# burchim/AVEC

Measured on AMD Instinct MI355X. Metric: AV utterances/sec fwd+bwd (audio T=400, video 100x88x88), higher is better.
Workload: dtype bf16

## Files before the change

avec_amd/csrc/norm.hip:

```cpp
#include "common.h"
#include "avec_hip.h"

#include "vec.h"

__global__ __launch_bounds__(256) void col_finalize_kernel(ColFin f) {
  __shared__ float red[16][17];
  const int cw = threadIdx.x & 15, sl = threadIdx.x >> 4;
  const int ncols = f.NV * f.W;
  const int o = blockIdx.x * 16 + cw;
  const unsigned cb = blockIdx.y;
  const int s0 = blockIdx.z * 128;
  float s = 0.f;
  if (o < ncols) {
    const float* p = f.partial + ((size_t)cb * f.nslots) * ncols + o;
#pragma unroll
    for (int k = 0; k < 8; ++k) {
      const int si = s0 + sl + 16 * k; const int sc = si < f.nslots ? si : f.nslots - 1;
      const float v = p[(size_t)sc * ncols];
      s += si < f.nslots ? v : 0.f;
    }
  }
  red[sl][cw] = s;
  __syncthreads();
  if (sl == 0 && o < ncols) {
// ... 241 lines not shown
  t1 = wave_sum(t1) / D; t2 = wave_sum(t2) / D;
#pragma unroll
  for (int i = 0; i < 2; ++i) {
    const int c = lane * 4 + i * 256; if (c >= D) break;
    float r[4];
#pragma unroll
    for (int e = 0; e < 4; ++e) r[e] = rs1 * (o[i][e] * gg1[i][e] - t1 - w1[i][e] * t2);
    st4<float>(dx1 + row * D + c, r);
    if (pr.out) {
      float q[4], ds[4]; drop4(dk, (unsigned long long)row * D + c, ds);
#pragma unroll
      for (int e = 0; e < 4; ++e) q[e] = r[e] * (pr.alpha * ds[e]);
      if (pr.f32) st4<float>((float*)pr.out + row * D + c, q); else st4<bf16>((bf16*)pr.out + row * D + c, q);
    }
  }
}
extern "C" int avec_layernorm_bwd2(int dtype, const void* dy2, const float* x2, const float* mean2, const float* rstd2, const float* gamma2, const float* dres2, float* dx2,
                                   const float* x1, const float* mean1, const float* rstd1, const float* gamma1, float* dx1,
                                   void* prep, float prep_alpha, float prep_drop_p, const unsigned long long* rng, unsigned rng_stream, long long M, int D, hipStream_t st) {
  AVEC_CHECK_ARG(dy2 && x2 && mean2 && rstd2 && gamma2 && dx2 && x1 && mean1 && rstd1 && gamma1 && dx1, "layernorm_bwd2: null pointer");
  AVEC_CHECK_ARG(M > 0 && D > 0 && D % 4 == 0 && D <= 512 && (!prep || prep_drop_p <= 0.f || rng), "layernorm_bwd2: D=%d must be a multiple of 4 in [4, 512]; dropout needs rng", D);
  LnPrep pr; pr.out = prep; pr.alpha = prep_alpha; pr.p = prep ? prep_drop_p : 0.f; pr.rng = rng; pr.stream = rng_stream; pr.f32 = dtype == AVEC_F32;
  dim3 grid((unsigned)((M + 3) / 4));
  if (dtype == AVEC_F32) hipLaunchKernelGGL(ln_bwd_rows2_kernel<float>, grid, dim3(256), 0, st, (const float*)dy2, x2, mean2, rstd2, gamma2, dres2, dx2, x1, mean1, rstd1, gamma1, dx1, M, D, pr);
  else hipLaunchKernelGGL(ln_bwd_rows2_kernel<bf16>, grid, dim3(256), 0, st, (const bf16*)dy2, x2, mean2, rstd2, gamma2, dres2, dx2, x1, mean1, rstd1, gamma1, dx1, M, D, pr);
  AVEC_LAUNCH_CHECK(); return 0;
}

struct LnItem { const void* dy; const float* x; const float* mean; const float* rstd; float* dg; float* db; int M, D, dy_f32, first; };
struct LnGroup { LnItem it[AVEC_LN_GROUP_MAX]; int n; };
static constexpr int LNG_ROWS = 128;
__global__ __launch_bounds__(256) void ln_param_grads_grouped_kernel(LnGroup grp) {
  __shared__ float red[2][256][4];
  const int w = blockIdx.x;
  int lo = 0, hi = grp.n - 1;
  while (lo < hi) { const int mid = (lo + hi + 1) >> 1; if (grp.it[mid].first <= w) lo = mid; else hi = mid - 1; }
  const LnItem& t = grp.it[lo];
  const int D = t.D, L = D >> 2, R = 256 / L;
  const int r = threadIdx.x / L, l = threadIdx.x - r * L;
  const int m0 = (w - t.first) * LNG_ROWS; int m1 = m0 + LNG_ROWS; if (m1 > t.M) m1 = t.M;
  float pg[4] = {0.f, 0.f, 0.f, 0.f}, pb[4] = {0.f, 0.f, 0.f, 0.f};
  if (r < R) {
    constexpr int U = 8;
    for (int m = m0 + r; m < m1; m += R * U) {
      float d[U][4], v[U][4], mu[U], rs[U];
#pragma unroll
      for (int u = 0; u < U; ++u) {
        const int mm = m + u * R; const bool ok = mm < m1; const long long mi = ok ? mm : m;
        if (t.dy_f32) ld4<float>((const float*)t.dy + mi * D + l * 4, d[u]); else ld4<bf16>((const bf16*)t.dy + mi * D + l * 4, d[u]);
        ld4<float>(t.x + mi * D + l * 4, v[u]); mu[u] = t.mean[mi]; rs[u] = ok ? t.rstd[mi] : 0.f;
        if (!ok) d[u][0] = d[u][1] = d[u][2] = d[u][3] = 0.f;
      }
#pragma unroll
      for (int u = 0; u < U; ++u)
#pragma unroll
        for (int e = 0; e < 4; ++e) { pg[e] += d[u][e] * (v[u][e] - mu[u]) * rs[u]; pb[e] += d[u][e]; }
    }
  }
#pragma unroll
  for (int e = 0; e < 4; ++e) { red[0][threadIdx.x][e] = pg[e]; red[1][threadIdx.x][e] = pb[e]; }
  __syncthreads();
  for (int o = threadIdx.x; o < 2 * D; o += 256) {
    const int which = o >= D, c = o - which * D; float s = 0.f;
    for (int rr = 0; rr < R; ++rr) s += red[which][rr * L + (c >> 2)][c & 3];
    atomicAdd((which ? t.db : t.dg) + c, s);
  }
}
extern "C" int avec_layernorm_param_grads_grouped(int dtype, const avec_ln_item_t* items, int n, hipStream_t st) {
  AVEC_CHECK_ARG(items && n > 0 && n <= AVEC_LN_GROUP_MAX, "layernorm_param_grads_grouped: need 1..%d items (got %d)", AVEC_LN_GROUP_MAX, n);
  LnGroup grp; grp.n = n; int first = 0;
  for (int k = 0; k < n; ++k) {
    const avec_ln_item_t& s = items[k];
    AVEC_CHECK_ARG(s.dy && s.x && s.mean && s.rstd && s.dgamma && s.dbeta && s.M > 0 && s.M < (1ll << 31) && s.D >= 4 && s.D % 4 == 0 && s.D <= 1024,
                   "layernorm_param_grads_grouped: item %d: null pointer or D=%d not a multiple of 4 in [4, 1024]", k, s.D);
    LnItem& t = grp.it[k];
    t.dy = s.dy; t.x = s.x; t.mean = s.mean; t.rstd = s.rstd; t.dg = s.dgamma; t.db = s.dbeta; t.M = (int)s.M; t.D = s.D;
    t.dy_f32 = (s.dy_f32 || dtype == AVEC_F32) ? 1 : 0; t.first = first;
    first += (int)((s.M + LNG_ROWS - 1) / LNG_ROWS);
  }
  hipLaunchKernelGGL(ln_param_grads_grouped_kernel, dim3((unsigned)first), dim3(256), 0, st, grp);
  AVEC_LAUNCH_CHECK(); return 0;
}

static int layernorm_bwd_impl(int dtype, const void* dy, int dy_f32, const float* x, const float* mean, const float* rstd, const float* gamma,
                              float* dx, const float* dres, float* dgamma, float* dbeta, long long M, int D, const LnPrep& pr, hipStream_t st) {
  AVEC_CHECK_ARG(dy && x && mean && rstd && gamma && dx && (!dgamma == !dbeta), "layernorm_bwd: null pointer");
  AVEC_CHECK_ARG(M > 0 && D > 0 && D % 4 == 0 && D <= 1536, "layernorm_bwd: D=%d must be a multiple of 4 and <= 1536", D);
  AVEC_CHECK_ARG(!pr.out || (!dgamma && (pr.p <= 0.f || pr.rng)), "layernorm_bwd_prep: the second output comes with the dx-only kernel (dgamma == NULL); dropout needs rng");
  if (!dgamma) {
    const dim3 grid((unsigned)((M + 3) / 4)); const bool f32in = dy_f32 || dtype == AVEC_F32;
#define AVEC_LN_ROWS(TG, NG) hipLaunchKernelGGL((ln_bwd_rows_kernel<TG, NG>), grid, dim3(256), 0, st, (const TG*)dy, x, mean, rstd, gamma, dx, dres, M, D, pr)
    if (D <= 512) { if (f32in) AVEC_LN_ROWS(float, 2); else AVEC_LN_ROWS(bf16, 2); }
    else { if (f32in) AVEC_LN_ROWS(float, 6); else AVEC_LN_ROWS(bf16, 6); }
#undef AVEC_LN_ROWS
    AVEC_LAUNCH_CHECK(); return 0;
  }
  long long nb = (M + 15) / 16; if (nb > 256) nb = 256; if (nb < 1) nb = 1;
  ColWs ws = avec_reduce_ws((size_t)nb * 2 * D, st);
  if (!ws.partial && nb > 128) nb = 128;
  const size_t lds = (size_t)2 * D * sizeof(float);
#define AVEC_LN_BWD(TG, NG) hipLaunchKernelGGL((ln_bwd_kernel<TG, NG>), dim3((unsigned)nb), dim3(256), lds, st, (const TG*)dy, x, mean, rstd, gamma, dx, dres, dgamma, dbeta, M, D, ws)
  const bool f32in = dy_f32 || dtype == AVEC_F32;
  if (D <= 512) { if (f32in) AVEC_LN_BWD(float, 2); else AVEC_LN_BWD(bf16, 2); }
  else { if (f32in) AVEC_LN_BWD(float, 6); else AVEC_LN_BWD(bf16, 6); }
#undef AVEC_LN_BWD
  AVEC_LAUNCH_CHECK();
  if (ws.partial) { float* const dst[2] = {dgamma, dbeta}; return col_finalize(ws, 1, (unsigned)nb, 2, D, dst, D, st); }
  return 0;
}
extern "C" int avec_layernorm_bwd(int dtype, const void* dy, int dy_f32, const float* x, const float* mean, const float* rstd, const float* gamma,
                                  float* dx, const float* dres, float* dgamma, float* dbeta, long long M, int D, hipStream_t st) {
  LnPrep pr; pr.out = nullptr; pr.alpha = 1.f; pr.p = 0.f; pr.rng = nullptr; pr.stream = 0; pr.f32 = 0;
  return layernorm_bwd_impl(dtype, dy, dy_f32, x, mean, rstd, gamma, dx, dres, dgamma, dbeta, M, D, pr, st);
}
extern "C" int avec_layernorm_bwd_prep(int dtype, const void* dy, int dy_f32, const float* x, const float* mean, const float* rstd, const float* gamma,
                                       float* dx, const float* dres, void* prep, float prep_alpha, float prep_drop_p, const unsigned long long* rng, unsigned rng_stream,
                                       long long M, int D, hipStream_t st) {
  AVEC_CHECK_ARG(prep, "layernorm_bwd_prep: null prep buffer");
  LnPrep pr; pr.out = prep; pr.alpha = prep_alpha; pr.p = prep_drop_p; pr.rng = rng; pr.stream = rng_stream; pr.f32 = dtype == AVEC_F32;
  return layernorm_bwd_impl(dtype, dy, dy_f32, x, mean, rstd, gamma, dx, dres, nullptr, nullptr, M, D, pr, st);
}

template <typename T>
__global__ __launch_bounds__(256) void grad_prep_kernel(const float* __restrict__ dout, long long ldd, T* __restrict__ dacc, float alpha, float p,
                                                        const unsigned long long* rng, unsigned stream, float* dbias, long long M, int N, ColWs ws) {
  const int tx = threadIdx.x & 31, ty = threadIdx.x >> 5;
  const int col = (blockIdx.x * 32 + tx) * 4;
  float part[1][4] = {{0.f, 0.f, 0.f, 0.f}};
  const DropKey dk = drop_key(rng, stream, p);
  if (col < N) {
    for (long long row = (long long)blockIdx.y * 8 + ty; row < M; row += (long long)gridDim.y * 8) {
      float v[4]; ld4<float>(dout + row * ldd + col, v);
      float ds[4]; drop4(dk, (unsigned long long)row * N + col, ds);
      for (int e = 0; e < 4; ++e) { v[e] *= alpha * ds[e]; part[0][e] += v[e]; }
      st4<T>(dacc + row * N + col, v);
    }
  }
  float* const dst[1] = {dbias};
  if (dbias) colreduce_atomic<1>(part, dst, col, N, ws);
}

template <typename T>
__global__ __launch_bounds__(256) void grad_prep_flat_kernel(const float* __restrict__ dout, long long ldd, T* __restrict__ dacc, float alpha, float p,
                                                             const unsigned long long* rng, unsigned stream, long long M, int N) {
  const int N4 = N >> 2; const long long n4 = M * N4;
  const DropKey dk = drop_key(rng, stream, p);
  for (long long i = (long long)blockIdx.x * 256 + threadIdx.x; i < n4; i += (long long)gridDim.x * 256) {
    const long long row = n4 < (1ll << 31) ? (long long)((unsigned)i / (unsigned)N4) : i / N4; const int col = (int)(i - row * N4) * 4;
    float v[4]; ld4<float>(dout + row * ldd + col, v);
    float ds[4]; drop4(dk, (unsigned long long)row * N + col, ds);
    for (int e = 0; e < 4; ++e) v[e] *= alpha * ds[e];
    st4<T>(dacc + row * N + col, v);
  }
}
extern "C" int avec_grad_prep(int dtype, const float* dout, long long ld, void* dacc, float alpha, float drop_p, const unsigned long long* rng,
                              unsigned rng_stream, float* dbias, long long M, int N, hipStream_t st) {
  AVEC_CHECK_ARG(dout && dacc && M > 0 && N > 0 && N % 4 == 0 && ld % 4 == 0, "grad_prep: bad arguments (N=%d ld=%lld)", N, ld);
  AVEC_CHECK_ARG(!(drop_p > 0.f) || rng, "grad_prep: dropout without rng");
  if (!dbias) {
    long long nb = (M * (N / 4) + 255) / 256; if (nb > 8192) nb = 8192;
    DISPATCH_T(dtype, hipLaunchKernelGGL(grad_prep_flat_kernel<T>, dim3((unsigned)nb), dim3(256), 0, st, dout, ld, (T*)dacc, alpha, drop_p, rng, rng_stream, M, N));
    AVEC_LAUNCH_CHECK(); return 0;
  }
  dim3 grid = col_grid(M, N); ColWs ws = dbias ? col_ws_if(grid, 1, N, st) : ColWs{nullptr};
  DISPATCH_T(dtype, hipLaunchKernelGGL(grad_prep_kernel<T>, grid, dim3(256), 0, st, dout, ld, (T*)dacc, alpha, drop_p, rng, rng_stream, dbias, M, N, ws));
  AVEC_LAUNCH_CHECK();
  if (ws.partial) { float* const dst[1] = {dbias}; return col_finalize(ws, grid.x, grid.y, 1, 128, dst, N, st); }
  return 0;
}

template <typename T>
__global__ __launch_bounds__(256) void colsum_kernel(const T* __restrict__ x, long long ld, float* out, long long M, int N, ColWs ws) {
  const int tx = threadIdx.x & 31, ty = threadIdx.x >> 5; const int col = (blockIdx.x * 32 + tx) * 4;
  float part[1][4] = {{0.f, 0.f, 0.f, 0.f}};
  if (col < N) for (long long row = (long long)blockIdx.y * 8 + ty; row < M; row += (long long)gridDim.y * 8) {
    float v[4]; ld4<T>(x + row * ld + col, v); for (int e = 0; e < 4; ++e) part[0][e] += v[e];
  }
  float* const dst[1] = {out};
  colreduce_atomic<1>(part, dst, col, N, ws);
}
extern "C" int avec_colsum(int dtype, const void* x, long long ld, float* out, long long M, int N, hipStream_t st) { return colsum_launch(dtype, x, ld, out, M, N, true, st); }
int colsum_launch(int dtype, const void* x, long long ld, float* out, long long M, int N, bool use_ws, hipStream_t st) {
  AVEC_CHECK_ARG(x && out && M > 0 && N > 0 && N % 4 == 0 && ld % 4 == 0, "colsum: bad arguments");
  dim3 grid = col_grid(M, N); if (!use_ws && grid.y > 16) grid.y = 16; ColWs ws = use_ws ? col_ws_if(grid, 1, N, st) : ColWs{nullptr};
  DISPATCH_T(dtype, hipLaunchKernelGGL(colsum_kernel<T>, grid, dim3(256), 0, st, (const T*)x, ld, out, M, N, ws));
  AVEC_LAUNCH_CHECK();
  if (ws.partial) { float* const dst[1] = {out}; return col_finalize(ws, grid.x, grid.y, 1, 128, dst, N, st); }
  return 0;
}

template <typename T>
__global__ __launch_bounds__(256) void bn_stats_kernel(const T* __restrict__ y, float* stats, long long M, int C, ColWs ws) {
  const int tx = threadIdx.x & 31, ty = threadIdx.x >> 5; const int col = (blockIdx.x * 32 + tx) * 4;
  float part[2][4] = {{0.f, 0.f, 0.f, 0.f}, {0.f, 0.f, 0.f, 0.f}};
  if (col < C) for (long long row = (long long)blockIdx.y * 8 + ty; row < M; row += (long long)gridDim.y * 8) {
    float v[4]; ld4<T>(y + row * C + col, v); for (int e = 0; e < 4; ++e) { part[0][e] += v[e]; part[1][e] += v[e] * v[e]; }
  }
  float* const dst[2] = {stats, stats + C};
  colreduce_atomic<2>(part, dst, col, C, ws);
}
extern "C" int avec_bn_stats(int dtype, const void* y, float* stats, long long M, int C, hipStream_t st) {
  AVEC_CHECK_ARG(y && stats && M > 0 && C > 0 && C % 4 == 0, "bn_stats: bad arguments");
  dim3 grid = col_grid(M, C); ColWs ws = col_ws_if(grid, 2, C, st);
  DISPATCH_T(dtype, hipLaunchKernelGGL(bn_stats_kernel<T>, grid, dim3(256), 0, st, (const T*)y, stats, M, C, ws));
  AVEC_LAUNCH_CHECK();
  if (ws.partial) { float* const dst[2] = {stats, stats + C}; return col_finalize(ws, grid.x, grid.y, 2, 128, dst, C, st); }
  return 0;
}

__global__ __launch_bounds__(256) void bn_finalize_kernel(const float* stats, int nrep, const float* count_ptr, float count, const float* gamma, const float* beta, float* rmean, float* rvar,
                                                          long long* nbt, float momentum, float eps, float* ss, int C, int training) {
  __shared__ float red[2][16][17];
  const int cl = threadIdx.x & 15, rl = threadIdx.x >> 4;
  const int c = blockIdx.x * 16 + cl;
  const bool lead = rl == 0 && c < C;
  float gm = 0.f, bt = 0.f, rm = 0.f, rv = 0.f, n = count;
  if (lead) { gm = gamma[c]; bt = beta[c]; if (rmean) { rm = rmean[c]; rv = rvar[c]; } if (training && count_ptr) n = *count_ptr; }
  float s1 = 0.f, s2 = 0.f;
  if (training && c < C) for (int r = rl; r < nrep; r += 16) { s1 += stats[(long long)r * 2 * C + c]; s2 += stats[(long long)r * 2 * C + C + c]; }
  red[0][rl][cl] = s1; red[1][rl][cl] = s2;
  __syncthreads();
  if (!lead) return;
  float mean, var;
  if (training) {
    s1 = 0.f; s2 = 0.f;
#pragma unroll
    for (int k = 0; k < 16; ++k) { s1 += red[0][k][cl]; s2 += red[1][k][cl]; }
    mean = s1 / n; var = fmaxf(s2 / n - mean * mean, 0.f);
    if (rmean && isfinite(mean) && isfinite(var)) {
      rmean[c] = (1.f - momentum) * rm + momentum * mean;
      rvar[c] = (1.f - momentum) * rv + momentum * var * (n / fmaxf(n - 1.f, 1.f));
      if (c == 0 && nbt) *nbt += 1;
    }
  } else { mean = rm; var = rv; }
  const float rs = rsqrtf(var + eps);
  ss[c] = gm * rs; ss[C + c] = bt - mean * gm * rs; ss[2 * C + c] = mean; ss[3 * C + c] = rs;
}
__global__ __launch_bounds__(256) void bn_collapse_kernel(const float* __restrict__ stats, int nrep, float count, float* __restrict__ out, int C2) {
  const int c = blockIdx.x * 256 + threadIdx.x;
  if (c < C2) { float s = 0.f; for (int r = 0; r < nrep; ++r) s += stats[(long long)r * C2 + c]; out[c] = s; }
  if (c == 0) out[C2] = count;
}
__global__ __launch_bounds__(256) void bn_affine_grads_kernel(const float* __restrict__ dstats, float* dgamma, float* dbeta, int C) {
  const int c = blockIdx.x * 256 + threadIdx.x;
  if (c < C) { dgamma[c] += dstats[C + c]; dbeta[c] += dstats[c]; }
}
extern "C" int avec_bn_collapse(const float* stats, int n_replicas, float count, float* out, int C, hipStream_t st) {
  AVEC_CHECK_ARG(stats && out && n_replicas > 0 && C > 0, "bn_collapse: bad arguments");
  hipLaunchKernelGGL(bn_collapse_kernel, dim3((2 * C + 255) / 256), dim3(256), 0, st, stats, n_replicas, count, out, 2 * C);
  AVEC_LAUNCH_CHECK(); return 0;
}
extern "C" int avec_bn_affine_grads(const float* dstats, float* dgamma, float* dbeta, int C, hipStream_t st) {
  AVEC_CHECK_ARG(dstats && dgamma && dbeta && C > 0, "bn_affine_grads: bad arguments");
  hipLaunchKernelGGL(bn_affine_grads_kernel, dim3((C + 255) / 256), dim3(256), 0, st, dstats, dgamma, dbeta, C);
  AVEC_LAUNCH_CHECK(); return 0;
}
extern "C" int avec_bn_finalize(const float* stats, int n_replicas, const float* count_ptr, float count, const float* gamma, const float* beta, float* running_mean,
                                float* running_var, long long* num_batches_tracked, float momentum, float eps, float* ss, int C, int training, hipStream_t st) {
  AVEC_CHECK_ARG(gamma && beta && ss && C > 0 && (training ? (stats != nullptr) : (running_mean && running_var)), "bn_finalize: bad arguments");
  hipLaunchKernelGGL(bn_finalize_kernel, dim3((C + 15) / 16), dim3(256), 0, st, stats, n_replicas > 0 ? n_replicas : 1, count_ptr, count, gamma, beta, running_mean, running_var,
                     num_batches_tracked, momentum, eps, ss, C, training);
  AVEC_LAUNCH_CHECK(); return 0;
}

__global__ void stamp_kernel(unsigned long long* out, int i) { if (threadIdx.x == 0) out[i] = wall_clock64(); }
extern "C" int avec_stamp(unsigned long long* out, int slot, hipStream_t st) {
  AVEC_CHECK_ARG(out && slot >= 0, "stamp: bad arguments");
  hipLaunchKernelGGL(stamp_kernel, dim3(1), dim3(64), 0, st, out, slot);
  AVEC_LAUNCH_CHECK(); return 0;
}

__global__ __launch_bounds__(256) void bn_bwd_finalize_kernel(const float* __restrict__ stats, int nrep, const float* __restrict__ ss, float* __restrict__ dstats, int C) {
  const int c = blockIdx.x * 256 + threadIdx.x;
  if (c >= C) return;
  float s1 = 0.f, sy = 0.f;
  for (int r = 0; r < nrep; ++r) { s1 += stats[(long long)r * 2 * C + c]; sy += stats[(long long)r * 2 * C + C + c]; }
  dstats[c] = s1; dstats[C + c] = ss[3 * C + c] * (sy - ss[2 * C + c] * s1);
}
extern "C" int avec_bn_bwd_finalize(const float* stats, int n_replicas, const float* ss, float* dstats, int C, hipStream_t st) {
  AVEC_CHECK_ARG(stats && ss && dstats && C > 0 && n_replicas > 0, "bn_bwd_finalize: bad arguments");
  hipLaunchKernelGGL(bn_bwd_finalize_kernel, dim3((C + 255) / 256), dim3(256), 0, st, stats, n_replicas, ss, dstats, C);
  AVEC_LAUNCH_CHECK(); return 0;
}

template <typename T>
__global__ __launch_bounds__(256) void bn_apply_kernel(const T* __restrict__ y, const float* __restrict__ ss, const T* __restrict__ res, int act,
                                                       T* __restrict__ out, long long n4, int C) {
  for (long long i = (long long)blockIdx.x * 256 + threadIdx.x; i < n4; i += (long long)gridDim.x * 256) {
    const long long off = i * 4; const int c = (int)(off % C);
    float v[4], sc[4], sh[4]; ld4<T>(y + off, v); ld4<float>(ss + c, sc); ld4<float>(ss + C + c, sh);
    for (int e = 0; e < 4; ++e) v[e] = v[e] * sc[e] + sh[e];
    if (res) { float r[4]; ld4<T>(res + off, r); for (int e = 0; e < 4; ++e) v[e] += r[e]; }
    if (act == 1) { for (int e = 0; e < 4; ++e) v[e] = swishf_(v[e]); } else if (act == 2) { for (int e = 0; e < 4; ++e) v[e] = fmaxf(v[e], 0.f); }
    st4<T>(out + off, v);
  }
}
static inline unsigned bn8_blocks(long long n8, int C, unsigned cap) {
  const unsigned C8 = (unsigned)C >> 3; unsigned g = C8, t = 256; while (t) { const unsigned r = g % t; g = t; t = r; }
  const unsigned q = C8 / g;
  long long nb = (n8 + 255) / 256; if (nb > cap) nb = cap;
  nb = nb / q * q; if (nb < q) nb = q;
  return (unsigned)nb;
}
constexpr int BN8_U = 2;
#ifndef AVEC_BN8_UR
#define AVEC_BN8_UR 1
#endif
constexpr int BN8_UR = AVEC_BN8_UR;
constexpr unsigned BN8_CAP_FWD = 8192, BN8_CAP_BWD = 3072;

template <typename T>
__global__ __launch_bounds__(256) void bn_apply8_kernel(const T* __restrict__ y, const float* __restrict__ ss, const T* __restrict__ res, int act,
                                                        T* __restrict__ out, unsigned n8, int C, unsigned char* __restrict__ mask = nullptr,
                                                        const float* __restrict__ res_ss = nullptr) {
  const unsigned C8 = (unsigned)C >> 3, stride = gridDim.x * 256, i0 = blockIdx.x * 256 + threadIdx.x;
  const int c = (int)(i0 % C8) * 8;
  float sc[8], sh[8]; ld8<float>(ss + c, sc); ld8<float>(ss + C + c, sh);
  float rsc[8], rsh[8];
  if (res_ss) { ld8<float>(res_ss + c, rsc); ld8<float>(res_ss + C + c, rsh);
#pragma unroll
    for (int e = 0; e < 8; ++e) sh[e] += rsh[e]; }
  for (unsigned i = i0; i < n8; i += stride * BN8_U) {
    Raw8<T> ry[BN8_U], rr[BN8_U];
#pragma unroll
    for (int u = 0; u < BN8_U; ++u) { const unsigned j = i + u * stride; if (j < n8) { ry[u].load(y + (long long)j * 8); if (res) rr[u].load(res + (long long)j * 8); } }
#pragma unroll
    for (int u = 0; u < BN8_U; ++u) {
      const unsigned j = i + u * stride; if (j >= n8) break;
      float v[8]; ry[u].get(v);
#pragma unroll
      for (int e = 0; e < 8; ++e) v[e] = v[e] * sc[e] + sh[e];
      if (res) { float r[8]; rr[u].get(r);
        if (res_ss) {
#pragma unroll
          for (int e = 0; e < 8; ++e) v[e] += r[e] * rsc[e];
        } else {
#pragma unroll
          for (int e = 0; e < 8; ++e) v[e] += r[e]; } }
      if (act == 1) {
#pragma unroll
        for (int e = 0; e < 8; ++e) v[e] = swishf_(v[e]);
      } else if (act == 2) {
        if (mask) {
          unsigned b = 0;
#pragma unroll
          for (int e = 0; e < 8; ++e) b |= (v[e] > 0.f ? 1u : 0u) << e;
          mask[j] = (unsigned char)b;
        }
#pragma unroll
        for (int e = 0; e < 8; ++e) v[e] = fmaxf(v[e], 0.f);
      }
      st8<T>(out + (long long)j * 8, v);
    }
  }
}
extern "C" int avec_bn_apply_fwd_mask(int dtype, const void* y, const float* ss, const void* residual, const float* residual_ss, void* out, unsigned char* mask, long long M, int C,
                                      hipStream_t st) {
  AVEC_CHECK_ARG(y && ss && out && mask && M > 0 && C > 0 && C % 8 == 0 && M * C / 8 < (1ll << 31) && (residual || !residual_ss), "bn_apply_fwd_mask: bad arguments (C %% 8 == 0, M*C < 2^34)");
  const long long n8 = M * C / 8; const unsigned nb8 = bn8_blocks(n8, C, BN8_CAP_FWD);
  DISPATCH_T(dtype, hipLaunchKernelGGL(bn_apply8_kernel<T>, dim3((unsigned)nb8), dim3(256), 0, st, (const T*)y, ss, (const T*)residual, 2, (T*)out, (unsigned)n8, C, mask, residual_ss));
  AVEC_LAUNCH_CHECK(); return 0;
}
extern "C" int avec_bn_apply_fwd(int dtype, const void* y, const float* ss, const void* residual, int act, void* out, long long M, int C, hipStream_t st) {
  AVEC_CHECK_ARG(y && ss && out && M > 0 && C > 0 && C % 4 == 0, "bn_apply_fwd: bad arguments");
  if (C % 8 == 0 && M * C / 8 < (1ll << 31)) {
    const long long n8 = M * C / 8; const unsigned nb8 = bn8_blocks(n8, C, BN8_CAP_FWD);
    DISPATCH_T(dtype, hipLaunchKernelGGL(bn_apply8_kernel<T>, dim3((unsigned)nb8), dim3(256), 0, st, (const T*)y, ss, (const T*)residual, act, (T*)out, (unsigned)n8, C));
    AVEC_LAUNCH_CHECK(); return 0;
  }
  long long n4 = M * C / 4; long long nb = (n4 + 255) / 256; if (nb > 4096) nb = 4096;
  DISPATCH_T(dtype, hipLaunchKernelGGL(bn_apply_kernel<T>, dim3((unsigned)nb), dim3(256), 0, st, (const T*)y, ss, (const T*)residual, act, (T*)out, n4, C));
  AVEC_LAUNCH_CHECK(); return 0;
}

template <typename T>
__device__ __forceinline__ void bn_dr(const T* dout, const T* y, const T* out, const float* ss, int act, long long off, int c, int C, float dr[4], float yh[4]) {
  float d[4], v[4], mu[4], rs[4]; ld4<T>(dout + off, d); ld4<T>(y + off, v); ld4<float>(ss + 2 * C + c, mu); ld4<float>(ss + 3 * C + c, rs);
  for (int e = 0; e < 4; ++e) yh[e] = (v[e] - mu[e]) * rs[e];
  if (act == 2) {
    if (out) { float o[4]; ld4<T>(out + off, o); for (int e = 0; e < 4; ++e) dr[e] = o[e] > 0.f ? d[e] : 0.f; }
    else { float sc[4], sh[4]; ld4<float>(ss + c, sc); ld4<float>(ss + C + c, sh); for (int e = 0; e < 4; ++e) dr[e] = (v[e] * sc[e] + sh[e]) > 0.f ? d[e] : 0.f; }
  }
  else if (act == 1) { float sc[4], sh[4]; ld4<float>(ss + c, sc); ld4<float>(ss + C + c, sh); for (int e = 0; e < 4; ++e) dr[e] = d[e] * dswishf_(v[e] * sc[e] + sh[e]); }
  else { for (int e = 0; e < 4; ++e) dr[e] = d[e]; }
}
template <typename T>
__global__ __launch_bounds__(256) void bn_bwd_reduce_kernel(const T* __restrict__ dout, const T* __restrict__ y, const T* __restrict__ out, const float* __restrict__ ss,
                                                            int act, float* dstats, long long M, int C, ColWs ws) {
  const int tx = threadIdx.x & 31, ty = threadIdx.x >> 5; const int col = (blockIdx.x * 32 + tx) * 4;
  float part[2][4] = {{0.f, 0.f, 0.f, 0.f}, {0.f, 0.f, 0.f, 0.f}};
  if (col < C) for (long long row = (long long)blockIdx.y * 8 + ty; row < M; row += (long long)gridDim.y * 8) {
    float dr[4], yh[4]; bn_dr<T>(dout, y, out, ss, act, row * C + col, col, C, dr, yh);
    for (int e = 0; e < 4; ++e) { part[0][e] += dr[e]; part[1][e] += dr[e] * yh[e]; }
  }
  float* const dst[2] = {dstats, dstats + C};
  colreduce_atomic<2>(part, dst, col, C, ws);
}
template <typename T>
__global__ __launch_bounds__(256) void bn_bwd_reduce8_kernel(const T* __restrict__ dout, const T* __restrict__ y, const T* __restrict__ out, const float* __restrict__ ss,
                                                             int act, float* dstats, long long M, int C, ColWs ws, const unsigned char* __restrict__ mask = nullptr) {
  const Col8 m = col8_map(C);
  float part[2][8];
#pragma unroll
  for (int e = 0; e < 8; ++e) part[0][e] = part[1][e] = 0.f;
  if (m.active) {
    const int c = m.l * 8;
    float mu[8], rs[8], sc[8], sh[8]; ld8<float>(ss + 2 * C + c, mu); ld8<float>(ss + 3 * C + c, rs);
    if (act == 1 || (act == 2 && !out && !mask)) { ld8<float>(ss + c, sc); ld8<float>(ss + C + c, sh); }
    const long long rstride = (long long)gridDim.x * m.R;
    for (long long row = (long long)blockIdx.x * m.R + m.r; row < M; row += rstride * BN8_UR) {
      Raw8<T> rd[BN8_UR], rv[BN8_UR], ro[BN8_UR]; unsigned mb[BN8_UR];
#pragma unroll
      for (int u = 0; u < BN8_UR; ++u) { const long long r = row + u * rstride; if (r < M) { const long long off = r * C + c; rd[u].load(dout + off); rv[u].load(y + off);
        if (mask) mb[u] = mask[off >> 3]; else if (act == 2 && out) ro[u].load(out + off); } }
#pragma unroll
      for (int u = 0; u < BN8_UR; ++u) {
        if (row + u * rstride >= M) break;
        float d[8], v[8]; rd[u].get(d); rv[u].get(v);
        if (mask) {
#pragma unroll
          for (int e = 0; e < 8; ++e) d[e] = (mb[u] >> e) & 1u ? d[e] : 0.f; }
        else if (act == 2 && out) { float o[8]; ro[u].get(o);
#pragma unroll
          for (int e = 0; e < 8; ++e) d[e] = o[e] > 0.f ? d[e] : 0.f; }
        else if (act == 2) {
#pragma unroll
          for (int e = 0; e < 8; ++e) d[e] = (v[e] * sc[e] + sh[e]) > 0.f ? d[e] : 0.f; }
        else if (act == 1) {
#pragma unroll
          for (int e = 0; e < 8; ++e) d[e] *= dswishf_(v[e] * sc[e] + sh[e]); }
#pragma unroll
        for (int e = 0; e < 8; ++e) { part[0][e] += d[e]; part[1][e] += d[e] * (v[e] - mu[e]) * rs[e]; }
      }
    }
  }
  float* const dst[2] = {dstats, dstats + C};
  colreduce8_atomic<2>(part, dst, m, ws);
}
extern "C" int avec_bn_bwd_reduce_mask(int dtype, const void* dout, const void* y, const unsigned char* mask, const float* ss, float* dstats, long long M, int C, hipStream_t st) {
  AVEC_CHECK_ARG(dout && y && mask && ss && dstats && M > 0 && col8_ok(C), "bn_bwd_reduce_mask: bad arguments");
  ColWs ws; const unsigned nb = col8_cfg(M, C, 2, &ws, st);
  DISPATCH_T(dtype, hipLaunchKernelGGL(bn_bwd_reduce8_kernel<T>, dim3(nb), dim3(256), 0, st, (const T*)dout, (const T*)y, (const T*)nullptr, ss, 2, dstats, M, C, ws, mask));
  AVEC_LAUNCH_CHECK();
  if (ws.partial) { float* const dst[2] = {dstats, dstats + C}; return col_finalize(ws, 1, nb, 2, C, dst, C, st); }
  return 0;
}
extern "C" int avec_bn_bwd_reduce(int dtype, const void* dout, const void* y, const void* out, const float* ss, int act, float* dstats, long long M, int C, hipStream_t st) {
  AVEC_CHECK_ARG(dout && y && ss && dstats && M > 0 && C % 4 == 0, "bn_bwd_reduce: bad arguments");
  if (col8_ok(C)) {
    ColWs ws; const unsigned nb = col8_cfg(M, C, 2, &ws, st);
    DISPATCH_T(dtype, hipLaunchKernelGGL(bn_bwd_reduce8_kernel<T>, dim3(nb), dim3(256), 0, st, (const T*)dout, (const T*)y, (const T*)out, ss, act, dstats, M, C, ws));
    AVEC_LAUNCH_CHECK();
    if (ws.partial) { float* const dst[2] = {dstats, dstats + C}; return col_finalize(ws, 1, nb, 2, C, dst, C, st); }
    return 0;
  }
  dim3 grid = col_grid(M, C); ColWs ws = col_ws_if(grid, 2, C, st);
  DISPATCH_T(dtype, hipLaunchKernelGGL(bn_bwd_reduce_kernel<T>, grid, dim3(256), 0, st, (const T*)dout, (const T*)y, (const T*)out, ss, act, dstats, M, C, ws));
  AVEC_LAUNCH_CHECK();
  if (ws.partial) { float* const dst[2] = {dstats, dstats + C}; return col_finalize(ws, grid.x, grid.y, 2, 128, dst, C, st); }
  return 0;
}
template <typename T>
__global__ __launch_bounds__(256) void bn_bwd_apply_kernel(const T* __restrict__ dout, const T* __restrict__ y, const T* __restrict__ out, const float* __restrict__ ss,
                                                           const float* __restrict__ gamma, const float* __restrict__ dstats, const float* count_ptr, float count, int act,
                                                           T* __restrict__ dy, T* __restrict__ dres, float* dgamma, float* dbeta, long long n4, int C) {
  const float inv_n = 1.f / (count_ptr ? *count_ptr : count);
  if (blockIdx.x == 0 && dgamma) for (int c = threadIdx.x; c < C; c += 256) { atomicAdd(dgamma + c, dstats[C + c]); atomicAdd(dbeta + c, dstats[c]); }
  for (long long i = (long long)blockIdx.x * 256 + threadIdx.x; i < n4; i += (long long)gridDim.x * 256) {
    const long long off = i * 4; const int c = (int)(off % C);
    float dr[4], yh[4], g[4], rs[4], s1[4], s2[4], o[4];
    bn_dr<T>(dout, y, out, ss, act, off, c, C, dr, yh);
    ld4<float>(gamma + c, g); ld4<float>(ss + 3 * C + c, rs); ld4<float>(dstats + c, s1); ld4<float>(dstats + C + c, s2);
    for (int e = 0; e < 4; ++e) o[e] = g[e] * rs[e] * (dr[e] - s1[e] * inv_n - yh[e] * s2[e] * inv_n);
    st4<T>(dy + off, o);
    if (dres) st4<T>(dres + off, dr);
  }
}
template <typename T>
__global__ __launch_bounds__(256) void bn_bwd_apply8_kernel(const T* __restrict__ dout, const T* __restrict__ y, const T* __restrict__ out, const float* __restrict__ ss,
                                                            const float* __restrict__ gamma, const float* __restrict__ dstats, const float* count_ptr, float count, int act,
                                                            T* __restrict__ dy, T* __restrict__ dres, float* dgamma, float* dbeta, unsigned n8, int C,
                                                            const unsigned char* __restrict__ mask = nullptr) {
  const float inv_n = 1.f / (count_ptr ? *count_ptr : count);
  if (blockIdx.x == 0 && dgamma) for (int c = threadIdx.x; c < C; c += 256) { atomicAdd(dgamma + c, dstats[C + c]); atomicAdd(dbeta + c, dstats[c]); }
  const unsigned C8 = (unsigned)C >> 3, stride = gridDim.x * 256, i0 = blockIdx.x * 256 + threadIdx.x;
  const int c = (int)(i0 % C8) * 8;
  float mu[8], rs[8], A[8], m1[8], m2[8], sc[8], sh[8];
  { float g[8], s1[8], s2[8]; ld8<float>(ss + 2 * C + c, mu); ld8<float>(ss + 3 * C + c, rs); ld8<float>(gamma + c, g); ld8<float>(dstats + c, s1); ld8<float>(dstats + C + c, s2);
#pragma unroll
    for (int e = 0; e < 8; ++e) { A[e] = g[e] * rs[e]; m1[e] = s1[e] * inv_n; m2[e] = s2[e] * inv_n; } }
  const bool recompute = act != 0 && !(act == 2 && (out || mask));
  if (recompute) { ld8<float>(ss + c, sc); ld8<float>(ss + C + c, sh); }
  for (unsigned i = i0; i < n8; i += stride * BN8_U) {
    Raw8<T> rd[BN8_U], rv[BN8_U], ro[BN8_U]; unsigned mb[BN8_U];
#pragma unroll
    for (int u = 0; u < BN8_U; ++u) { const unsigned j = i + u * stride; if (j < n8) { const long long off = (long long)j * 8; rd[u].load(dout + off); rv[u].load(y + off);
      if (mask) mb[u] = mask[j]; else if (act == 2 && out) ro[u].load(out + off); } }
#pragma unroll
    for (int u = 0; u < BN8_U; ++u) {
      const unsigned j = i + u * stride; if (j >= n8) break;
      const long long off = (long long)j * 8;
      float d[8], v[8], o[8]; rd[u].get(d); rv[u].get(v);
      if (mask) {
#pragma unroll
        for (int e = 0; e < 8; ++e) d[e] = (mb[u] >> e) & 1u ? d[e] : 0.f;
      } else if (act == 2 && out) { float q[8]; ro[u].get(q);
#pragma unroll
        for (int e = 0; e < 8; ++e) d[e] = q[e] > 0.f ? d[e] : 0.f;
      } else if (act != 0) {
#pragma unroll
        for (int e = 0; e < 8; ++e) { const float pre = v[e] * sc[e] + sh[e]; d[e] = act == 1 ? d[e] * dswishf_(pre) : (pre > 0.f ? d[e] : 0.f); }
      }
#pragma unroll
      for (int e = 0; e < 8; ++e) o[e] = A[e] * (d[e] - m1[e] - (v[e] - mu[e]) * rs[e] * m2[e]);
      st8<T>(dy + off, o);
      if (dres) st8<T>(dres + off, d);
    }
  }
}
extern "C" int avec_bn_bwd_apply_mask(int dtype, const void* dout, const void* y, const unsigned char* mask, const float* ss, const float* gamma, const float* dstats,
                                      const float* count_ptr, float count, void* dy, void* dres, float* dgamma, float* dbeta, long long M, int C, hipStream_t st) {
  AVEC_CHECK_ARG(dout && y && mask && ss && gamma && dstats && dy && M > 0 && C % 8 == 0 && M * C / 8 < (1ll << 31), "bn_bwd_apply_mask: bad arguments");
  const long long n8 = M * C / 8; const unsigned nb8 = bn8_blocks(n8, C, BN8_CAP_BWD);
  DISPATCH_T(dtype, hipLaunchKernelGGL(bn_bwd_apply8_kernel<T>, dim3((unsigned)nb8), dim3(256), 0, st, (const T*)dout, (const T*)y, (const T*)nullptr, ss, gamma, dstats,
                                       count_ptr, count, 2, (T*)dy, (T*)dres, dgamma, dbeta, (unsigned)n8, C, mask));
  AVEC_LAUNCH_CHECK(); return 0;
}
extern "C" int avec_bn_bwd_apply(int dtype, const void* dout, const void* y, const void* out, const float* ss, const float* gamma, const float* dstats,
                                 const float* count_ptr, float count, int act, void* dy, void* dres, float* dgamma, float* dbeta, long long M, int C, hipStream_t st) {
  AVEC_CHECK_ARG(dout && y && ss && gamma && dstats && dy && M > 0 && C % 4 == 0, "bn_bwd_apply: bad arguments");
  if (C % 8 == 0 && M * C / 8 < (1ll << 31)) {
    const long long n8 = M * C / 8; const unsigned nb8 = bn8_blocks(n8, C, BN8_CAP_BWD);
    DISPATCH_T(dtype, hipLaunchKernelGGL(bn_bwd_apply8_kernel<T>, dim3((unsigned)nb8), dim3(256), 0, st, (const T*)dout, (const T*)y, (const T*)out, ss, gamma, dstats,
                                         count_ptr, count, act, (T*)dy, (T*)dres, dgamma, dbeta, (unsigned)n8, C));
    AVEC_LAUNCH_CHECK(); return 0;
  }
  long long n4 = M * C / 4; long long nb = (n4 + 255) / 256; if (nb > 4096) nb = 4096;
  DISPATCH_T(dtype, hipLaunchKernelGGL(bn_bwd_apply_kernel<T>, dim3((unsigned)nb), dim3(256), 0, st, (const T*)dout, (const T*)y, (const T*)out, ss, gamma, dstats,
                                       count_ptr, count, act, (T*)dy, (T*)dres, dgamma, dbeta, n4, C));
  AVEC_LAUNCH_CHECK(); return 0;
}

template <typename T>
__global__ __launch_bounds__(256) void softmax_fwd_kernel(const float* __restrict__ x, T* __restrict__ p, long long M, int V) {
  const int lane = threadIdx.x & 63; const long long row = (long long)blockIdx.x * 4 + (threadIdx.x >> 6);
  if (row >= M) return;
  float mx = -INFINITY;
  for (int c = lane; c < V; c += 64) mx = fmaxf(mx, x[row * V + c]);
  mx = wave_max(mx);
  float s = 0.f;
  for (int c = lane; c < V; c += 64) s += __expf(x[row * V + c] - mx);
  s = 1.f / wave_sum(s);
  for (int c = lane; c < V; c += 64) stf(p + row * V + c, __expf(x[row * V + c] - mx) * s);
}
template <typename T>
__global__ __launch_bounds__(256) void softmax_bwd_kernel(const T* __restrict__ dp, const float* __restrict__ x, float* dx, const float* dadd, long long M, int V) {
  const int lane = threadIdx.x & 63; const long long row = (long long)blockIdx.x * 4 + (threadIdx.x >> 6);
  if (row >= M) return;
  float mx = -INFINITY;
  for (int c = lane; c < V; c += 64) mx = fmaxf(mx, x[row * V + c]);
  mx = wave_max(mx);
  float s = 0.f, dot = 0.f;
  for (int c = lane; c < V; c += 64) { float e = __expf(x[row * V + c] - mx); s += e; dot += e * ldf(dp + row * V + c); }
  s = wave_sum(s); dot = wave_sum(dot) / s;
  for (int c = lane; c < V; c += 64) {
    float pr = __expf(x[row * V + c] - mx) / s; float g = pr * (ldf(dp + row * V + c) - dot);
    dx[row * V + c] = dadd ? dadd[row * V + c] + g : g;
  }
}
extern "C" int avec_softmax_fwd(int dtype, const float* logits, void* probs, long long M, int V, hipStream_t st) {
  AVEC_CHECK_ARG(logits && probs && M > 0 && V > 0, "softmax_fwd: bad arguments");
  DISPATCH_T(dtype, hipLaunchKernelGGL(softmax_fwd_kernel<T>, dim3((unsigned)((M + 3) / 4)), dim3(256), 0, st, logits, (T*)probs, M, V));
  AVEC_LAUNCH_CHECK(); return 0;
}
extern "C" int avec_softmax_bwd(int dtype, const void* dprobs, const float* logits, float* dlogits, const float* dadd, long long M, int V, hipStream_t st) {
  AVEC_CHECK_ARG(dprobs && logits && dlogits && M > 0 && V > 0, "softmax_bwd: bad arguments");
  DISPATCH_T(dtype, hipLaunchKernelGGL(softmax_bwd_kernel<T>, dim3((unsigned)((M + 3) / 4)), dim3(256), 0, st, (const T*)dprobs, logits, dlogits, dadd, M, V));
  AVEC_LAUNCH_CHECK(); return 0;
}

template <typename T>
__global__ __launch_bounds__(256) void cast_rows_kernel(const float* __restrict__ src, long long lds_, T* __restrict__ dst, long long ldd, long long M, int N) {
  const long long n4 = M * (N / 4);
  for (long long i = (long long)blockIdx.x * 256 + threadIdx.x; i < n4; i += (long long)gridDim.x * 256) {
    const long long row = i / (N / 4); const int c = (int)(i % (N / 4)) * 4;
    float v[4]; ld4<float>(src + row * lds_ + c, v); st4<T>(dst + row * ldd + c, v);
  }
}
extern "C" int avec_cast_rows(int dtype, const float* src, long long ld_src, void* dst, long long ld_dst, long long M, int N, hipStream_t st) {
  AVEC_CHECK_ARG(src && dst && M > 0 && N > 0 && N % 4 == 0 && ld_src % 4 == 0 && ld_dst % 4 == 0, "cast_rows: bad arguments");
  long long nb = (M * (N / 4) + 255) / 256; if (nb > 4096) nb = 4096;
  DISPATCH_T(dtype, hipLaunchKernelGGL(cast_rows_kernel<T>, dim3((unsigned)nb), dim3(256), 0, st, src, ld_src, (T*)dst, ld_dst, M, N));
  AVEC_LAUNCH_CHECK(); return 0;
}
template <typename T>
__global__ __launch_bounds__(256) void to_f32_rows_kernel(const T* __restrict__ src, long long lds_, float* __restrict__ dst, long long ldd, long long M, int N, int accum) {
  const long long n4 = M * (N / 4);
  for (long long i = (long long)blockIdx.x * 256 + threadIdx.x; i < n4; i += (long long)gridDim.x * 256) {
    const long long row = i / (N / 4); const int c = (int)(i % (N / 4)) * 4;
    float v[4]; ld4<T>(src + row * lds_ + c, v);
    if (accum) { float o[4]; ld4<float>(dst + row * ldd + c, o); for (int e = 0; e < 4; ++e) v[e] += o[e]; }
    st4<float>(dst + row * ldd + c, v);
  }
}
extern "C" int avec_to_f32_rows(int dtype, const void* src, long long ld_src, float* dst, long long ld_dst, long long M, int N, int accum, hipStream_t st) {
  AVEC_CHECK_ARG(src && dst && M > 0 && N > 0 && N % 4 == 0 && ld_src % 4 == 0 && ld_dst % 4 == 0, "to_f32_rows: bad arguments");
  long long nb = (M * (N / 4) + 255) / 256; if (nb > 4096) nb = 4096;
  DISPATCH_T(dtype, hipLaunchKernelGGL(to_f32_rows_kernel<T>, dim3((unsigned)nb), dim3(256), 0, st, (const T*)src, ld_src, dst, ld_dst, M, N, accum));
  AVEC_LAUNCH_CHECK(); return 0;
}

__global__ __launch_bounds__(256) void dropout_f32_kernel(const float* __restrict__ x, float* __restrict__ y, float p, const unsigned long long* rng, unsigned stream, long long n) {
  const DropKey dk = drop_key(rng, stream, p);
  for (long long i = (long long)blockIdx.x * 256 + threadIdx.x; i < n; i += (long long)gridDim.x * 256) y[i] = x[i] * drop_one(dk, (unsigned long long)i);
}
extern "C" int avec_dropout_f32(const float* x, float* y, float p, const unsigned long long* rng, unsigned rng_stream, long long n, hipStream_t st) {
  AVEC_CHECK_ARG(x && y && n > 0 && rng, "dropout_f32: bad arguments");
  long long nb = (n + 255) / 256; if (nb > 4096) nb = 4096;
  hipLaunchKernelGGL(dropout_f32_kernel, dim3((unsigned)nb), dim3(256), 0, st, x, y, p, rng, rng_stream, n);
  AVEC_LAUNCH_CHECK(); return 0;
}

__global__ __launch_bounds__(256) void act_f32_kernel(const float* __restrict__ x, const float* __restrict__ dy, float* __restrict__ out, int act, long long rows, int C, int bwd) {
  const long long n = rows * C;
  for (long long i = (long long)blockIdx.x * 256 + threadIdx.x; i < n; i += (long long)gridDim.x * 256) {
    if (act == 3) {
      const long long r = i / C; const int c = (int)(i - r * C);
      const float a = x[r * 2 * C + c], b = x[r * 2 * C + C + c], sg = sigmoidf_(b);
      if (!bwd) out[i] = a * sg;
      else { const float g = dy[i]; out[r * 2 * C + c] = g * sg; out[r * 2 * C + C + c] = g * a * sg * (1.f - sg); }
    } else {
      const float v = x[i];
      if (!bwd) out[i] = act == 1 ? swishf_(v) : fmaxf(v, 0.f);
      else out[i] = dy[i] * (act == 1 ? dswishf_(v) : (v > 0.f ? 1.f : 0.f));
    }
  }
}
extern "C" int avec_act_f32(int act, const float* x, const float* dy, float* out, long long rows, int C, int backward, hipStream_t st) {
  AVEC_CHECK_ARG(x && out && rows > 0 && C > 0 && act >= 1 && act <= 3 && (!backward || dy), "act_f32: bad arguments (act=%d)", act);
  long long nb = (rows * C + 255) / 256; if (nb > 4096) nb = 4096;
  hipLaunchKernelGGL(act_f32_kernel, dim3((unsigned)nb), dim3(256), 0, st, x, dy, out, act, rows, C, backward);
  AVEC_LAUNCH_CHECK(); return 0;
}

template <typename T>
__global__ __launch_bounds__(256) void patch_pool_fwd_kernel(const T* __restrict__ x, T* __restrict__ y, int B, int Tn, int D, int P, int Tp) {
  const long long n4 = (long long)B * Tp * (D / 4);
  for (long long i = (long long)blockIdx.x * 256 + threadIdx.x; i < n4; i += (long long)gridDim.x * 256) {
    const int c = (int)(i % (D / 4)) * 4; const long long r = i / (D / 4); const int tp = (int)(r % Tp); const int b = (int)(r / Tp);
    float a[4] = {0.f, 0.f, 0.f, 0.f};
    for (int k = 0; k < P; ++k) { int t = tp * P + k; if (t < Tn) { float v[4]; ld4<T>(x + ((long long)b * Tn + t) * D + c, v); for (int e = 0; e < 4; ++e) a[e] += v[e]; } }
    for (int e = 0; e < 4; ++e) a[e] /= P;
    st4<T>(y + r * D + c, a);
  }
}
template <typename T>
__global__ __launch_bounds__(256) void patch_pool_bwd_kernel(const T* __restrict__ dy, T* __restrict__ dx, int B, int Tn, int D, int P, int Tp) {
  const long long n4 = (long long)B * Tn * (D / 4);
  for (long long i = (long long)blockIdx.x * 256 + threadIdx.x; i < n4; i += (long long)gridDim.x * 256) {
    const int c = (int)(i % (D / 4)) * 4; const long long r = i / (D / 4); const int t = (int)(r % Tn); const int b = (int)(r / Tn);
    float v[4]; ld4<T>(dy + ((long long)b * Tp + t / P) * D + c, v); for (int e = 0; e < 4; ++e) v[e] /= P;
    st4<T>(dx + r * D + c, v);
  }
}
template <typename T>
__global__ __launch_bounds__(256) void patch_unpool_add_kernel(const T* __restrict__ o, const float* __restrict__ res, float* __restrict__ out, float p,
                                                               const unsigned long long* rng, unsigned stream, int B, int Tn, int D, int P, int Tp) {
  const long long n4 = (long long)B * Tn * (D / 4);
  const DropKey dk = drop_key(rng, stream, p);
  for (long long i = (long long)blockIdx.x * 256 + threadIdx.x; i < n4; i += (long long)gridDim.x * 256) {
    const int c = (int)(i % (D / 4)) * 4; const long long r = i / (D / 4); const int t = (int)(r % Tn); const int b = (int)(r / Tn);
    float v[4], q[4]; ld4<T>(o + ((long long)b * Tp + t / P) * D + c, v); ld4<float>(res + r * D + c, q);
    float ds[4]; drop4(dk, (unsigned long long)r * D + c, ds);
    for (int e = 0; e < 4; ++e) q[e] += v[e] * ds[e];
    st4<float>(out + r * D + c, q);
  }
}
template <typename T>
__global__ __launch_bounds__(256) void patch_unpool_bwd_kernel(const float* __restrict__ dout, T* __restrict__ dob, float p, const unsigned long long* rng, unsigned stream,
                                                               int B, int Tn, int D, int P, int Tp) {
  const long long n4 = (long long)B * Tp * (D / 4);
  const DropKey dk = drop_key(rng, stream, p);
  for (long long i = (long long)blockIdx.x * 256 + threadIdx.x; i < n4; i += (long long)gridDim.x * 256) {
    const int c = (int)(i % (D / 4)) * 4; const long long r = i / (D / 4); const int tp = (int)(r % Tp); const int b = (int)(r / Tp);
    float a[4] = {0.f, 0.f, 0.f, 0.f};
    for (int k = 0; k < P; ++k) {
      int t = tp * P + k; if (t >= Tn) break;
      const long long rr = (long long)b * Tn + t; float v[4]; ld4<float>(dout + rr * D + c, v);
      float ds[4]; drop4(dk, (unsigned long long)rr * D + c, ds);
      for (int e = 0; e < 4; ++e) a[e] += v[e] * ds[e];
    }
    st4<T>(dob + r * D + c, a);
  }
}
#define PATCH_LAUNCH(kern, total, ...) do { long long nb = ((total) + 255) / 256; if (nb > 4096) nb = 4096; if (nb < 1) nb = 1; \
  DISPATCH_T(dtype, hipLaunchKernelGGL(kern<T>, dim3((unsigned)nb), dim3(256), 0, st, __VA_ARGS__)); AVEC_LAUNCH_CHECK(); return 0; } while (0)
extern "C" int avec_patch_pool_fwd(int dtype, const void* x, void* y, int B, int T_, int D, int P, hipStream_t st) {
  AVEC_CHECK_ARG(x && y && B > 0 && T_ > 0 && D % 4 == 0 && P > 0, "patch_pool_fwd: bad arguments"); const int Tp = (T_ + P - 1) / P;
  PATCH_LAUNCH(patch_pool_fwd_kernel, (long long)B * Tp * (D / 4), (const T*)x, (T*)y, B, T_, D, P, Tp);
}
extern "C" int avec_patch_pool_bwd(int dtype, const void* dy, void* dx, int B, int T_, int D, int P, hipStream_t st) {
  AVEC_CHECK_ARG(dy && dx && B > 0 && T_ > 0 && D % 4 == 0 && P > 0, "patch_pool_bwd: bad arguments"); const int Tp = (T_ + P - 1) / P;
  PATCH_LAUNCH(patch_pool_bwd_kernel, (long long)B * T_ * (D / 4), (const T*)dy, (T*)dx, B, T_, D, P, Tp);
}
extern "C" int avec_patch_unpool_add(int dtype, const void* o, const float* res, float* out, float drop_p, const unsigned long long* rng, unsigned rng_stream,
                                     int B, int T_, int D, int P, hipStream_t st) {
  AVEC_CHECK_ARG(o && res && out && B > 0 && T_ > 0 && D % 4 == 0 && P > 0 && (drop_p <= 0.f || rng), "patch_unpool_add: bad arguments"); const int Tp = (T_ + P - 1) / P;
  PATCH_LAUNCH(patch_unpool_add_kernel, (long long)B * T_ * (D / 4), (const T*)o, res, out, drop_p, rng, rng_stream, B, T_, D, P, Tp);
}
extern "C" int avec_patch_unpool_bwd(int dtype, const float* dout, void* dob, float drop_p, const unsigned long long* rng, unsigned rng_stream,
                                     int B, int T_, int D, int P, hipStream_t st) {
  AVEC_CHECK_ARG(dout && dob && B > 0 && T_ > 0 && D % 4 == 0 && P > 0 && (drop_p <= 0.f || rng), "patch_unpool_bwd: bad arguments"); const int Tp = (T_ + P - 1) / P;
  PATCH_LAUNCH(patch_unpool_bwd_kernel, (long long)B * Tp * (D / 4), dout, (T*)dob, drop_p, rng, rng_stream, B, T_, D, P, Tp);
}

template <typename T>
__global__ __launch_bounds__(256) void avgpool_fwd_kernel(const T* __restrict__ x, T* __restrict__ y, long long N, int HW, int C) {
  const long long n4 = N * (C / 4);
  for (long long i = (long long)blockIdx.x * 256 + threadIdx.x; i < n4; i += (long long)gridDim.x * 256) {
    const int c = (int)(i % (C / 4)) * 4; const long long n = i / (C / 4);
    float a[4] = {0.f, 0.f, 0.f, 0.f};
    for (int s = 0; s < HW; ++s) { float v[4]; ld4<T>(x + (n * HW + s) * C + c, v); for (int e = 0; e < 4; ++e) a[e] += v[e]; }
    for (int e = 0; e < 4; ++e) a[e] /= HW;
    st4<T>(y + n * C + c, a);
  }
}
template <typename T>
__global__ __launch_bounds__(256) void avgpool_bwd_kernel(const T* __restrict__ dy, T* __restrict__ dx, long long N, int HW, int C) {
  const long long n4 = N * HW * (C / 4);
  for (long long i = (long long)blockIdx.x * 256 + threadIdx.x; i < n4; i += (long long)gridDim.x * 256) {
    const int c = (int)(i % (C / 4)) * 4; const long long r = i / (C / 4); const long long n = r / HW;
    float v[4]; ld4<T>(dy + n * C + c, v); for (int e = 0; e < 4; ++e) v[e] /= HW;
    st4<T>(dx + r * C + c, v);
  }
}
extern "C" int avec_avgpool_fwd(int dtype, const void* x, void* y, long long N, int HW, int C, hipStream_t st) {
  AVEC_CHECK_ARG(x && y && N > 0 && HW > 0 && C % 4 == 0, "avgpool_fwd: bad arguments");
  PATCH_LAUNCH(avgpool_fwd_kernel, N * (C / 4), (const T*)x, (T*)y, N, HW, C);
}
extern "C" int avec_avgpool_bwd(int dtype, const void* dy, void* dx, long long N, int HW, int C, hipStream_t st) {
  AVEC_CHECK_ARG(dy && dx && N > 0 && HW > 0 && C % 4 == 0, "avgpool_bwd: bad arguments");
  PATCH_LAUNCH(avgpool_bwd_kernel, N * HW * (C / 4), (const T*)dy, (T*)dx, N, HW, C);
}

__global__ __launch_bounds__(256) void strided_rows_add_kernel(float* __restrict__ dx, const float* __restrict__ src, int B, int Tn, int To, int D, int step) {
  const long long n4 = (long long)B * To * (D / 4);
  for (long long i = (long long)blockIdx.x * 256 + threadIdx.x; i < n4; i += (long long)gridDim.x * 256) {
    const int c = (int)(i % (D / 4)) * 4; const long long r = i / (D / 4); const int to = (int)(r % To); const long long b = r / To;
    float v[4], o[4]; ld4<float>(src + r * D + c, v); float* dst = dx + (b * Tn + (long long)to * step) * D + c; ld4<float>(dst, o);
    for (int e = 0; e < 4; ++e) o[e] += v[e];
    st4<float>(dst, o);
  }
}
extern "C" int avec_strided_rows_add(float* dx, const float* src, int B, int T_, int To, int D, int step, hipStream_t st) {
  AVEC_CHECK_ARG(dx && src && B > 0 && T_ > 0 && To > 0 && D % 4 == 0 && step > 0 && (long long)(To - 1) * step < T_, "strided_rows_add: bad arguments");
  long long n4 = (long long)B * To * (D / 4); long long nb = (n4 + 255) / 256; if (nb > 4096) nb = 4096;
  hipLaunchKernelGGL(strided_rows_add_kernel, dim3((unsigned)nb), dim3(256), 0, st, dx, src, B, T_, To, D, step);
  AVEC_LAUNCH_CHECK(); return 0;
}
```

avec_amd/ops.py:

```python
import ctypes
import os

import torch

from . import fp8
from . import runtime as rt
from .lib import (ACT_GELU, ACT_NONE, ACT_RELU, ACT_SWISH, BF16, LN_GROUP_MAX, ROWS_CONV_BWD, ROWS_CONV_FWD, ROWS_PLAIN, ROWS_STEM3D, TN_GROUP_MAX, WGRAD_GROUP_MAX, Attn, Epilogue, LnItem, Rows, TnBatched, TnItem,
                  WgradItem, lib)

_byref = ctypes.byref


class KernelTimer:
    NAMES = {(0, ROWS_CONV_FWD): "gemm_nt<conv_fwd>", (0, ROWS_CONV_BWD): "gemm_nt<conv_bwd_data>", (0, ROWS_STEM3D): "gemm_nt<stem3d>",
             (0, ROWS_PLAIN): "gemm_nt<plain>", (1, ROWS_CONV_FWD): "gemm_tn<conv_wgrad>", (1, ROWS_STEM3D): "gemm_tn<stem3d_wgrad>",
             (1, ROWS_PLAIN): "gemm_tn<plain>", (2, 0): "conv3x3_slab<fwd>", (2, 1): "conv3x3_slab<bwd_data>", (2, 2): "conv3x3_slab<wgrad>"}

    def __init__(self):
        self.enabled = False
        self.records = []

    def reset(self, enabled):
        self.enabled, self.records = enabled, []

# ... 694 lines not shown
    if entry.remaining > 0:
        return
    grp = rt.fused_group(wp)
    R, W = 2 * entry.Tp - 1, entry.L * entry.D
    dea = empty((R, W), rt.act_dtype(), entry.de_all)
    lib.cast_rows(rt.dt(), entry.de_all.data_ptr(), W, dea.data_ptr(), W, R, W, rt.stream())
    gemm_tn(dea, entry.pe, grp.wgrad, R, W, entry.D, p_colsum=grp.bgrad, side=True)
    entry.de_all, entry.remaining = None, entry.L


class AttentionModuleFn(torch.autograd.Function):
    @staticmethod
    def forward(ctx, x, lens, mask, ln_w, ln_b, wq, bq, wk, bk, wv, bv, wo, bo, wp, bp, H, patch, eps, drop_p, sid, residual):
        rt.require_gpu(x)
        B, T, D = x.shape
        M, d, adt = B * T, D // H, rt.act_dtype()
        grp = rt.fused_group(wq)
        grp_ok = grp is not None and grp.weights[1] is wk and grp.weights[2] is wv and bq is not None
        x2 = _f32c(x.reshape(-1, D))
        if ln_w is not None:
            h, mean, rstd = layernorm_fwd(x2, ln_w, ln_b, M, D, False, eps)
        else:
            mean = rstd = None
            h = empty((M, D), adt, x2)
            lib.cast_rows(rt.dt(), x2.data_ptr(), D, h.data_ptr(), D, M, D, rt.stream())
        if patch > 1:
            Tp = (T + patch - 1) // patch
            hp = empty((B * Tp, D), adt, x2)
            lib.patch_pool_fwd(rt.dt(), h.data_ptr(), hp.data_ptr(), B, T, D, patch, rt.stream())
        else:
            Tp, hp = T, h
        Mp = B * Tp
        if mask is not None:
            mask = mask.reshape(mask.shape[0], T, T) if patch == 1 else _pool_mask(mask, T, patch)
            mask = mask.float().contiguous()
        if grp_ok:
            qkv = empty((Mp, 3 * D), adt, x2)
            ent = fp8.entry(wq, D)
            if ent is not None and ent.N == 3 * D:
                gemm_nt_fp8(hp, ent, qkv, Mp, 3 * D, D, bias=grp.bias)
            else:
                gemm_nt(hp, grp.fwd, qkv, Mp, 3 * D, D, bias=grp.bias)
        else:
            qkv = empty((Mp, 3 * D), adt, x2)
            for i, (w, b) in enumerate(((wq, bq), (wk, bk), (wv, bv))):
                sh = rt.shadow(w)
                gemm_nt(hp, sh.fwd, qkv[:, i * D:], Mp, D, D, bias=b, ldo=3 * D)
        pg, pgi = _pos_group_entry(wp, Tp, D, x.device)
        if pg is not None:
            pe, e = pg.pe, pg.e_all[:, pgi * D:(pgi + 1) * D]
        else:
            pe = rel_pos_table(Tp, D, x.device)
            e = linear_fwd(pe, wp, bp, 2 * Tp - 1, in_f32=False, out_f32=False)
        o = empty((Mp, D), adt, x2)
        lse = empty((B * H, Tp, 2), torch.float32, x2)
        q_full = T // patch if (patch > 1 and mask is None) else 0
        a = _attn_args(qkv, e, lens, patch, mask, o, lse, B, H, Tp, d, D, q_full)
        lib.relpos_attention_fwd(rt.dt(), _byref(a), rt.stream())
        res = x2 if residual else None
        if patch > 1:
            oo = linear_fwd(o, wo, bo, Mp, in_f32=False, out_f32=False)
            base = x2 if residual else torch.zeros_like(x2)
            y = empty((M, D), torch.float32, x2)
            rng = rt.rng_state(x.device).data_ptr() if drop_p > 0 else None
            lib.patch_unpool_add(rt.dt(), oo.data_ptr(), base.data_ptr(), y.data_ptr(), drop_p, rng, sid, B, T, D, patch, rt.stream())
        else:
            y = linear_fwd(o, wo, bo, M, in_f32=False, out_f32=True, drop_p=drop_p, sid=sid, res=res, alpha=1.0)
        ctx.saved = (x2, mean, rstd, h, hp, qkv, pe, e, o, lse, lens, mask, ln_w, ln_b, wq, bq, wk, bk, wv, bv, wo, bo, wp, bp,
                     H, patch, drop_p, sid, residual, B, T, Tp, D)
        ctx.pos_group = (pg, pgi)
        ctx.prep_req = _prep_request(x)
        return _tag_prep(y.view(B, T, D), 1.0, drop_p, sid) if patch == 1 else y.view(B, T, D)

    @staticmethod
    def backward(ctx, dy):
        (x2, mean, rstd, h, hp, qkv, pe, e, o, lse, lens, mask, ln_w, ln_b, wq, bq, wk, bk, wv, bv, wo, bo, wp, bp,
         H, patch, drop_p, sid, residual, B, T, Tp, D) = ctx.saved
        M, Mp, d, adt = B * T, B * Tp, D // H, rt.act_dtype()
        dy = _f32c(dy.reshape(M, D))
        if patch > 1:
            doo = empty((Mp, D), adt, dy)
            rng = rt.rng_state(dy.device).data_ptr() if drop_p > 0 else None
            lib.patch_unpool_bwd(rt.dt(), dy.data_ptr(), doo.data_ptr(), drop_p, rng, sid, B, T, D, patch, rt.stream())
        else:
            doo = _take_prep(dy, M, D, 1.0, drop_p, sid)
            if doo is None:
                doo = grad_prep(dy, M, D, drop_p=drop_p, sid=sid)
        linear_bwd_weight(doo, o, wo, Mp, bias=bo)
        do = torch.empty(Mp * D + 8, dtype=adt, device=dy.device)[:Mp * D].view(Mp, D)
        do = linear_bwd_input(doo, wo, Mp, out_f32=False, out=do)
        dqkv = empty((Mp, 3 * D), adt, dy)
        pg, pgi = ctx.pos_group
        if pg is not None:
            if pg.de_all is None:
                pg.de_all = rt.zeros_scratch((2 * Tp - 1) * pg.L * D, dy.device).view(2 * Tp - 1, pg.L * D)
            de = pg.de_all[:, pgi * D:(pgi + 1) * D]
        else:
            de = rt.zeros_scratch((2 * Tp - 1) * D, dy.device).view(2 * Tp - 1, D)
        a = _attn_args(qkv, e, lens, patch, mask, o, lse, B, H, Tp, d, D, T // patch if (patch > 1 and mask is None) else 0)
        a.dout = do.data_ptr()
        esz = dqkv.element_size()
        a.dq, a.lddq = dqkv.data_ptr(), 3 * D
        a.dk, a.dv, a.ldd = dqkv.data_ptr() + D * esz, dqkv.data_ptr() + 2 * D * esz, 3 * D
        a.de, a.ldde = de.data_ptr(), de.stride(0)
        Tld, Rld = (Tp + 7) // 8 * 8, (2 * Tp - 1 + 7) // 8 * 8
        scratch = empty((2, B * H, Tp, Tld), adt, dy)
        a.pbuf, a.dsbuf, a.ldt = scratch.data_ptr(), scratch.data_ptr() + scratch[0].numel() * esz, Tld
        use_mfma = d % 2 == 0 or not ATTN_ODD_VALU
        if use_mfma:
            n_rel = H * B * Tp * Rld
            if adt == torch.bfloat16:
                dsrel = rt.zeros_scratch((n_rel + 1) // 2, dy.device).view(torch.bfloat16)[:n_rel].view(H, B * Tp, Rld)
            else:
                dsrel = rt.zeros_scratch(n_rel, dy.device).view(H, B * Tp, Rld)
            a.dsrel, a.ldr = dsrel.data_ptr(), Rld
        lib.relpos_attention_bwd(rt.dt(), _byref(a), rt.stream())
        if use_mfma:
            L6 = ctypes.c_longlong * 6
            sK, sV, sE = L6(H * Tp * Tld, Tp * Tld, Tp * 3 * D, d, Tp * 3 * D, d), L6(H * Tp * Tld, Tp * Tld, Tp * D, d, Tp * 3 * D, d), L6(0, B * Tp * Rld, 0, d, 0, d)
            if TN_MULTI:
                it = (TnBatched * 3)()
                it[0].P, it[0].ldp, it[0].Q, it[0].ldq, it[0].O_act, it[0].ldo = a.dsbuf, Tld, qkv.data_ptr(), 3 * D, dqkv.data_ptr() + D * esz, 3 * D
                it[0].M, it[0].I, it[0].J, it[0].nb_outer, it[0].nb_inner, it[0].strides6 = Tp, Tp, d, B, H, sK
                it[1].P, it[1].ldp, it[1].Q, it[1].ldq, it[1].O_act, it[1].ldo = a.pbuf, Tld, do.data_ptr(), D, dqkv.data_ptr() + 2 * D * esz, 3 * D
                it[1].M, it[1].I, it[1].J, it[1].nb_outer, it[1].nb_inner, it[1].strides6 = Tp, Tp, d, B, H, sV
                it[2].P, it[2].ldp, it[2].Q, it[2].ldq, it[2].O, it[2].ldo = dsrel.data_ptr(), Rld, qkv.data_ptr(), 3 * D, de.data_ptr(), de.stride(0)
                it[2].M, it[2].I, it[2].J, it[2].nb_outer, it[2].nb_inner, it[2].strides6 = B * Tp, 2 * Tp - 1, d, 1, H, sE
                lib.gemm_tn_batched_multi(rt.dt(), it, 3, rt.stream())
            else:
                lib.gemm_tn_batched_store(rt.dt(), a.dsbuf, Tld, qkv.data_ptr(), 3 * D, dqkv.data_ptr() + D * esz, 3 * D, Tp, Tp, d, B, H, sK, rt.stream())
                lib.gemm_tn_batched_store(rt.dt(), a.pbuf, Tld, do.data_ptr(), D, dqkv.data_ptr() + 2 * D * esz, 3 * D, Tp, Tp, d, B, H, sV, rt.stream())
                lib.gemm_tn_batched(rt.dt(), dsrel.data_ptr(), Rld, qkv.data_ptr(), 3 * D, de.data_ptr(), de.stride(0), B * Tp, 2 * Tp - 1, d, 1, H, sE, rt.stream())
        dhp = None
        grp = rt.fused_group(wq)
        if grp is not None and grp.weights[1] is wk and grp.weights[2] is wv and bq is not None:
            gemm_tn(dqkv, hp, grp.wgrad, Mp, 3 * D, D, p_colsum=grp.bgrad, side=True)
            dhp = empty((Mp, D), adt, dy)
            gemm_nt(dqkv, grp.bwd, dhp, Mp, D, 3 * D)
        else:
            for i, (w, b) in enumerate(((wq, bq), (wk, bk), (wv, bv))):
                g = dqkv[:, i * D:]
                linear_bwd_weight(g, hp, w, Mp, ldp=3 * D, bias=b)
                dhp = linear_bwd_input(g, w, Mp, out_f32=False, lda=3 * D, res=dhp, res_act=True, out=dhp)
        if pg is not None:
            _pos_group_backward(pg, wp)
        else:
            dea = empty((2 * Tp - 1, D), adt, dy)
            lib.cast_rows(rt.dt(), de.data_ptr(), D, dea.data_ptr(), D, 2 * Tp - 1, D, rt.stream())
            linear_bwd_weight(dea, pe, wp, 2 * Tp - 1, bias=bp)
        if patch > 1:
            dh = empty((M, D), adt, dy)
            lib.patch_pool_bwd(rt.dt(), dhp.data_ptr(), dh.data_ptr(), B, T, D, patch, rt.stream())
        else:
            dh = dhp
        if ln_w is not None:
            dx = layernorm_bwd(dh, False, x2, mean, rstd, ln_w, ln_b, M, D, dres=dy if residual else None, prep=ctx.prep_req)
        else:
            dx = dy.clone() if residual else torch.zeros_like(dy)
            lib.to_f32_rows(rt.dt(), dh.data_ptr(), D, dx.data_ptr(), D, M, D, 1, rt.stream())
        return (dx.view(B, T, D),) + (None,) * 20


class RelPosCoreFn(torch.autograd.Function):

    @staticmethod
    def forward(ctx, qkv, e, lens, len_div, mask, B, H, T, d, scale):
        rt.require_gpu(qkv)
        D, adt = H * d, rt.act_dtype()
        assert qkv.dtype == adt and e.dtype == adt and qkv.is_contiguous() and e.is_contiguous() and qkv.shape == (B * T, 3 * D) and e.shape == (2 * T - 1, D)
        assert d % 2 == 0, "the batched-GEMM backward needs an even head width (pad the operands)"
        if mask is not None:
            mask = mask.reshape(mask.shape[0], T, T).float().contiguous()
        o = empty((B * T, D), adt, qkv)
        lse = empty((B * H, T, 2), torch.float32, qkv)
        a = _attn_args(qkv, e, lens, len_div, mask, o, lse, B, H, T, d, D)
        a.scale = scale
        lib.relpos_attention_fwd(rt.dt(), _byref(a), rt.stream())
        ctx.saved = (qkv, e, o, lse, lens, len_div, mask, B, H, T, d, scale)
        return o

    @staticmethod
    def backward(ctx, do):
        qkv, e, o, lse, lens, len_div, mask, B, H, T, d, scale = ctx.saved
        D, adt = H * d, rt.act_dtype()
        do = do.to(adt).contiguous()
        dqkv = empty((B * T, 3 * D), adt, do)
        de = torch.zeros((2 * T - 1, D), dtype=torch.float32, device=do.device)
        a = _attn_args(qkv, e, lens, len_div, mask, o, lse, B, H, T, d, D)
        a.scale = scale
        a.dout = do.data_ptr()
        esz = dqkv.element_size()
        a.dq, a.lddq = dqkv.data_ptr(), 3 * D
        a.dk, a.dv, a.ldd = dqkv.data_ptr() + D * esz, dqkv.data_ptr() + 2 * D * esz, 3 * D
        a.de, a.ldde = de.data_ptr(), D
        Tld, Rld = (T + 7) // 8 * 8, (2 * T - 1 + 7) // 8 * 8
        scratch = empty((2, B * H, T, Tld), adt, do)
        a.pbuf, a.dsbuf, a.ldt = scratch.data_ptr(), scratch.data_ptr() + scratch[0].numel() * esz, Tld
        dsrel = torch.zeros((H, B * T, Rld), dtype=adt, device=do.device)
        a.dsrel, a.ldr = dsrel.data_ptr(), Rld
        lib.relpos_attention_bwd(rt.dt(), _byref(a), rt.stream())
        L6 = ctypes.c_longlong * 6
        lib.gemm_tn_batched_store(rt.dt(), a.dsbuf, Tld, qkv.data_ptr(), 3 * D, dqkv.data_ptr() + D * esz, 3 * D, T, T, d, B, H,
                                  L6(H * T * Tld, T * Tld, T * 3 * D, d, T * 3 * D, d), rt.stream())
        lib.gemm_tn_batched_store(rt.dt(), a.pbuf, Tld, do.data_ptr(), D, dqkv.data_ptr() + 2 * D * esz, 3 * D, T, T, d, B, H,
                                  L6(H * T * Tld, T * Tld, T * D, d, T * 3 * D, d), rt.stream())
        lib.gemm_tn_batched(rt.dt(), dsrel.data_ptr(), Rld, qkv.data_ptr(), 3 * D, de.data_ptr(), D, B * T, 2 * T - 1, d, 1, H,
                            L6(0, B * T * Rld, 0, d, 0, d), rt.stream())
        return dqkv, de.to(adt), None, None, None, None, None, None, None, None


def relpos_core_infer(q, k, v, e, lens, mask, B, H, T, Tk, d, scale, want_probs=False):
    rt.require_gpu(q)
    D, adt = H * d, rt.act_dtype()
    for t in (q, k, v, e):
        assert t.dtype == adt and t.is_contiguous()
    assert q.shape == (B * T, D) and k.shape == (B * Tk, D) and v.shape == (B * Tk, D) and e.shape == (Tk + T - 1, D)
    if mask is not None:
        mask = mask.reshape(mask.shape[0], T, Tk).float().contiguous()
    o = empty((B * T, D), adt, q)
    lse = empty((B * H, T, 2), torch.float32, q)
    a = Attn()
    a.q, a.k, a.v, a.ld = q.data_ptr(), k.data_ptr(), v.data_ptr(), D
    a.e, a.lde = e.data_ptr(), D
    a.lens, a.len_div = _p(lens), 1
    if mask is not None:
        a.mask, a.mask_bstride = mask.data_ptr(), (T * Tk if mask.shape[0] > 1 else 0)
    a.o, a.ldo, a.lse = o.data_ptr(), D, lse.data_ptr()
    a.B, a.H, a.T, a.d, a.scale, a.Tk = B, H, T, d, scale, Tk
    lib.relpos_attention_fwd(rt.dt(), _byref(a), rt.stream())
    if not want_probs:
        return o, None
    Tld = (Tk + 7) // 8 * 8
    scratch = empty((2, B * H, T, Tld), adt, q)
    dq = empty((B * T, D), adt, q)
    zero = torch.zeros((B * T, D), dtype=adt, device=q.device)
    dsrel = torch.zeros((H, B * T, (Tk + T - 1 + 7) // 8 * 8), dtype=adt, device=q.device)
    a.dout, a.dq, a.lddq = zero.data_ptr(), dq.data_ptr(), D
    a.pbuf, a.dsbuf, a.ldt = scratch.data_ptr(), scratch.data_ptr() + scratch[0].numel() * scratch.element_size(), Tld
    a.dsrel, a.ldr = dsrel.data_ptr(), dsrel.shape[2]
    lib.relpos_attention_bwd(rt.dt(), _byref(a), rt.stream())
    return o, scratch[0].view(B, H, T, Tld)[..., :Tk].float()


def _pool_mask(mask, T, P):
    pad = (P - T % P) % P
    m = torch.nn.functional.pad(mask.reshape(mask.shape[0], 1, T, T).float(), (0, pad, 0, pad), value=0.0)
    Tp = (T + pad) // P
    return m.reshape(m.shape[0], Tp, P, Tp, P).amin(dim=(2, 4))


class BNState:

    NREP = 64

    def __init__(self, C, ref):
        self.stats = rt.zeros_scratch(self.NREP * 2 * C, ref.device)
        self.red = None
        self.ss = torch.empty(4 * C, dtype=torch.float32, device=ref.device)
        self.C = C


RELU_BITMASK = True
def bn_finalize(bn, st, count, training):
    C = st.C
    cptr = None
    sptr, nrep = st.stats.data_ptr(), st.NREP
    if training and rt.sync_batchnorm():
        st.red = rt.sync_bn_stats(st.stats, st.NREP, C, count, key=(id(bn), "f"))
        sptr, nrep, cptr = st.red.data_ptr(), 1, st.red.data_ptr() + 2 * C * 4
    mom = bn.momentum if bn.momentum is not None else 0.1
    track = bn.track_running_stats and bn.running_mean is not None
    lib.bn_finalize(sptr, nrep, cptr, float(count), bn.weight.data_ptr(), bn.bias.data_ptr(),
                    bn.running_mean.data_ptr() if track else None, bn.running_var.data_ptr() if track else None,
                    bn.num_batches_tracked.data_ptr() if (track and training) else None, mom, bn.eps, st.ss.data_ptr(), C, int(training), rt.stream())
    return cptr


def bn_backward(bn, st, cptr, count, dout, y, out, act, M, want_dres=False, pre=None, mask=None):
    C = st.C
    adt = rt.act_dtype()
    dstats = rt.zeros_scratch(2 * C, dout.device)
    if pre is not None:
        lib.bn_bwd_finalize(pre.stats.data_ptr(), BNState.NREP, st.ss.data_ptr(), dstats.data_ptr(), C, rt.stream())
        act, out, want_dres, mask = ACT_NONE, None, False, None
    elif mask is not None:
        lib.bn_bwd_reduce_mask(rt.dt(), dout.data_ptr(), y.data_ptr(), mask.data_ptr(), st.ss.data_ptr(), dstats.data_ptr(), M, C, rt.stream())
    else:
        lib.bn_bwd_reduce(rt.dt(), dout.data_ptr(), y.data_ptr(), _p(out), st.ss.data_ptr(), act, dstats.data_ptr(), M, C, rt.stream())
    gw, gb = grad_of(bn.weight), grad_of(bn.bias)
    dstats, synced = _add_local_affine_grads(dstats, gw, gb, C, (id(bn), "b"))
    if synced:
        gw = gb = None
    dy = empty((M, C), adt, dout)
    dres = empty((M, C), adt, dout) if want_dres else None
    if mask is not None:
        lib.bn_bwd_apply_mask(rt.dt(), dout.data_ptr(), y.data_ptr(), mask.data_ptr(), st.ss.data_ptr(), bn.weight.data_ptr(), dstats.data_ptr(), cptr, float(count),
                              dy.data_ptr(), _p(dres), _p(gw), _p(gb), M, C, rt.stream())
    else:
        lib.bn_bwd_apply(rt.dt(), dout.data_ptr(), y.data_ptr(), _p(out), st.ss.data_ptr(), bn.weight.data_ptr(), dstats.data_ptr(), cptr, float(count), act,
                         dy.data_ptr(), _p(dres), _p(gw), _p(gb), M, C, rt.stream())
    return dy, (dout if pre is not None else dres)


def _add_local_affine_grads(dstats, gw, gb, C, key):
    if not rt.sync_batchnorm():
        return dstats, False
    from . import peer
    px = peer.active()
    if px is not None and dstats.is_cuda and dstats.is_contiguous() :
        return px.all_reduce_sum_fused(dstats, 1, 2 * C, None, key, dgamma=gw, dbeta=gb, C=C), True
    lib.bn_affine_grads(dstats.data_ptr(), gw.data_ptr(), gb.data_ptr(), C, rt.stream())
    return rt.all_reduce_small(dstats, key), True



def dw_pad_left(conv):
    K = conv.kernel_size[0]
    kind = getattr(conv, "padding_type", "same")
    if kind == "causal":
        return K - 1
    assert kind == "same", "the fused convolution module supports 'same' and 'causal' padding, got %r" % (kind,)
    return K // 2

CONVMOD_BN_FUSE = True


class ConvModuleFn(torch.autograd.Function):
    @staticmethod
    def forward(ctx, x, _anchor, mod, res_conv, drop_p, sid, training):
        rt.require_gpu(x)
        B, T, D = x.shape
        ln, pw1, dw, bn, pw2 = mod.layers[0], mod.layers[1], mod.layers[3], mod.layers[4], mod.layers[6]
        Dp, K, stride = dw.weight.shape[0], dw.weight.shape[2], dw.stride[0]
        To = (T - 1) // stride + 1
        M, Mo, adt = B * T, B * To, rt.act_dtype()
        x2 = _f32c(x.reshape(M, D))
        h, mean, rstd = layernorm_fwd(x2, ln.weight, ln.bias, M, D, False, ln.eps)
        u = linear_fwd(h, pw1.weight, pw1.bias, M, in_f32=False, out_f32=False)
        c = empty((Mo, Dp), adt, x2)
        st = BNState(Dp, x2)
        use_batch = training and not getattr(bn, "frozen", False)
        if use_batch and not rt.sync_batchnorm() and CONVMOD_BN_FUSE:
            track = bn.track_running_stats and bn.running_mean is not None
            lib.glu_dwconv_fwd_bn(rt.dt(), u.data_ptr(), dw.weight.data_ptr(), _p(dw.bias), c.data_ptr(), st.stats.data_ptr(), B, T, Dp, K, stride, dw_pad_left(dw),
                                  bn.weight.data_ptr(), bn.bias.data_ptr(), bn.running_mean.data_ptr() if track else None, bn.running_var.data_ptr() if track else None,
                                  bn.num_batches_tracked.data_ptr() if track else None, bn.momentum if bn.momentum is not None else 0.1, bn.eps, st.ss.data_ptr(), rt.stream())
            cptr = None
        else:
            lib.glu_dwconv_fwd(rt.dt(), u.data_ptr(), dw.weight.data_ptr(), _p(dw.bias), c.data_ptr(), st.stats.data_ptr() if use_batch else None,
                               B, T, Dp, K, stride, dw_pad_left(dw), rt.stream())
            cptr = bn_finalize(bn, st, Mo, use_batch)
        a = empty((Mo, Dp), adt, x2)
        lib.bn_apply_fwd(rt.dt(), c.data_ptr(), st.ss.data_ptr(), None, ACT_SWISH, a.data_ptr(), Mo, Dp, rt.stream())
        if res_conv is not None:
            rs = res_conv.stride[0]
            R = linear_fwd(x2, res_conv.weight, res_conv.bias, Mo, in_f32=(adt != torch.float32), out_f32=True,
                           rows=rows_plain(D, To, T, rs) if rs > 1 else None)
        else:
            R = x2
        y = linear_fwd(a, pw2.weight, pw2.bias, Mo, in_f32=False, out_f32=True, drop_p=drop_p, sid=sid, res=R, alpha=1.0)
        ctx.saved = (x2, mean, rstd, h, u, c, a, st, cptr, use_batch, mod, res_conv, drop_p, sid, B, T, To, D, Dp, K, stride)
        ctx.prep_req = _prep_request(x)
        return _tag_prep(y.view(B, To, Dp), 1.0, drop_p, sid)

    @staticmethod
    def backward(ctx, dy):
        x2, mean, rstd, h, u, c, a, st, cptr, use_batch, mod, res_conv, drop_p, sid, B, T, To, D, Dp, K, stride = ctx.saved
        ln, pw1, dw, bn, pw2 = mod.layers[0], mod.layers[1], mod.layers[3], mod.layers[4], mod.layers[6]
        M, Mo, adt = B * T, B * To, rt.act_dtype()
        dy = _f32c(dy.reshape(Mo, Dp))
        dacc = _take_prep(dy, Mo, Dp, 1.0, drop_p, sid)
        if dacc is None:
            dacc = grad_prep(dy, Mo, Dp, drop_p=drop_p, sid=sid)
        linear_bwd_weight(dacc, a, pw2.weight, Mo, bias=pw2.bias)
        da = linear_bwd_input(dacc, pw2.weight, Mo, out_f32=False)
        du = empty((M, 2 * Dp), adt, dy)
        if use_batch and CONVMOD_BN_FUSE and stride == 1 and not rt.sync_batchnorm():
            dstats = rt.zeros_scratch(2 * Dp, da.device)
            lib.bn_bwd_reduce(rt.dt(), da.data_ptr(), c.data_ptr(), None, st.ss.data_ptr(), ACT_SWISH, dstats.data_ptr(), Mo, Dp, rt.stream())
            lib.dwconv_glu_bwd_bn(rt.dt(), da.data_ptr(), c.data_ptr(), st.ss.data_ptr(), bn.weight.data_ptr(), dstats.data_ptr(), float(Mo), u.data_ptr(), dw.weight.data_ptr(),
                                  du.data_ptr(), grad_of(dw.weight).data_ptr(), None if dw.bias is None else grad_of(dw.bias).data_ptr(),
                                  grad_of(bn.weight).data_ptr(), grad_of(bn.bias).data_ptr(), B, T, Dp, K, dw_pad_left(dw), rt.stream())
        else:
            if use_batch:
                dc, _ = bn_backward(bn, st, cptr, Mo, da, c, None, ACT_SWISH, Mo)
            else:
                dc = _bn_eval_backward(bn, st, da, c, ACT_SWISH, Mo)
            lib.dwconv_glu_bwd(rt.dt(), dc.data_ptr(), u.data_ptr(), dw.weight.data_ptr(), du.data_ptr(), grad_of(dw.weight).data_ptr(),
                               None if dw.bias is None else grad_of(dw.bias).data_ptr(), B, T, Dp, K, stride, dw_pad_left(dw), rt.stream())
        linear_bwd_weight(du, h, pw1.weight, M, bias=pw1.bias)
        dh = linear_bwd_input(du, pw1.weight, M, out_f32=False)
        if res_conv is None:
            dx = layernorm_bwd(dh, False, x2, mean, rstd, ln.weight, ln.bias, M, D, dres=dy, prep=ctx.prep_req)
        else:
            rs = res_conv.stride[0]
            dx = layernorm_bwd(dh, False, x2, mean, rstd, ln.weight, ln.bias, M, D)
            dracc = grad_prep(dy, Mo, Dp)
            linear_bwd_weight(dracc, x2, res_conv.weight, Mo, q_f32=(adt != torch.float32), q_rows=rows_plain(D, To, T, rs) if rs > 1 else None, bias=res_conv.bias)
            dxr = linear_bwd_input(dracc, res_conv.weight, Mo, out_f32=True)
            lib.strided_rows_add(dx.data_ptr(), dxr.data_ptr(), B, T, To, D, rs, rt.stream())
        return dx.view(B, T, D), None, None, None, None, None, None


def _bn_eval_backward(bn, st, dout, y, act, M, out=None):
    C = st.C
    dstats = torch.zeros(2 * C, dtype=torch.float32, device=dout.device)
    dstats2 = torch.zeros(2 * C, dtype=torch.float32, device=dout.device)
    lib.bn_bwd_reduce(rt.dt(), dout.data_ptr(), y.data_ptr(), _p(out), st.ss.data_ptr(), act, dstats2.data_ptr(), M, C, rt.stream())
    dy = empty((M, C), rt.act_dtype(), dout)
    lib.bn_bwd_apply(rt.dt(), dout.data_ptr(), y.data_ptr(), _p(out), st.ss.data_ptr(), bn.weight.data_ptr(), dstats.data_ptr(), None, 1.0, act,
                     dy.data_ptr(), None, None, None, M, C, rt.stream())
    grad_of(bn.weight).add_(dstats2[C:])
    grad_of(bn.bias).add_(dstats2[:C])
    return dy


class InterCTCFn(torch.autograd.Function):
    @staticmethod
    def forward(ctx, x, w1, b1, w2, b2):
        rt.require_gpu(x)
        B, T, D = x.shape
        M, V = B * T, w1.shape[0]
        x2 = _f32c(x.reshape(M, D))
        conv = rt.act_dtype() != torch.float32
        logits = linear_fwd(x2, w1, b1, M, in_f32=conv, out_f32=True)
        probs = empty((M, V), rt.act_dtype(), x2)
        lib.softmax_fwd(rt.dt(), logits.data_ptr(), probs.data_ptr(), M, V, rt.stream())
        y = linear_fwd(probs, w2, b2, M, in_f32=False, out_f32=True, res=x2, alpha=1.0)
        ctx.saved = (x2, logits, probs, w1, b1, w2, b2, B, T, D, V, conv)
        return y.view(B, T, D), logits.view(B, T, V)

    @staticmethod
    def backward(ctx, dy, dlogits_ext):
        x2, logits, probs, w1, b1, w2, b2, B, T, D, V, conv = ctx.saved
        M = B * T
        dy = _f32c(dy.reshape(M, D))
        dacc = grad_prep(dy, M, D)
        linear_bwd_weight(dacc, probs, w2, M, bias=b2)
        dprobs = linear_bwd_input(dacc, w2, M, out_f32=False)
        dl = empty((M, V), torch.float32, dy)
        dext = None if dlogits_ext is None else _f32c(dlogits_ext.reshape(M, V))
        lib.softmax_bwd(rt.dt(), dprobs.data_ptr(), logits.data_ptr(), dl.data_ptr(), _p(dext), M, V, rt.stream())
        dla = grad_prep(dl, M, V)
        linear_bwd_weight(dla, x2, w1, M, q_f32=conv, bias=b1)
        dx = linear_bwd_input(dla, w1, M, out_f32=True, res=dy)
        return dx.view(B, T, D), None, None, None, None


class FusionFn(torch.autograd.Function):
    @staticmethod
    def forward(ctx, a, v, w1, b1, w2, b2):
        rt.require_gpu(a)
        B, T, Da = a.shape
        Dv = v.shape[-1]
        M, F, adt = B * T, w1.shape[0], rt.act_dtype()
        a2, v2 = _f32c(a.reshape(M, Da)), _f32c(v.reshape(M, Dv))
        xc = empty((M, Da + Dv), adt, a2)
        lib.cast_rows(rt.dt(), a2.data_ptr(), Da, xc.data_ptr(), Da + Dv, M, Da, rt.stream())
        lib.cast_rows(rt.dt(), v2.data_ptr(), Dv, xc.data_ptr() + Da * xc.element_size(), Da + Dv, M, Dv, rt.stream())
        z = empty((M, F), adt, a2)
        h = linear_fwd(xc, w1, b1, M, in_f32=False, out_f32=False, act=ACT_SWISH, out_pre=z)
        y = linear_fwd(h, w2, b2, M, in_f32=False, out_f32=True)
        ctx.saved = (xc, z, h, w1, b1, w2, b2, B, T, Da, Dv, F)
        return y.view(B, T, -1)

    @staticmethod
    def backward(ctx, dy):
        xc, z, h, w1, b1, w2, b2, B, T, Da, Dv, F = ctx.saved
        M, N = B * T, w2.shape[0]
        dy = _f32c(dy.reshape(M, N))
        dacc = grad_prep(dy, M, N)
        linear_bwd_weight(dacc, h, w2, M, bias=b2)
        dz = linear_bwd_input(dacc, w2, M, out_f32=False, dact_z=z, dact=ACT_SWISH)
        linear_bwd_weight(dz, xc, w1, M, bias=b1)
        sh = rt.shadow(w1)
        da = empty((M, Da), torch.float32, dy)
        dv = empty((M, Dv), torch.float32, dy)
        gemm_nt(dz, sh.bwd, da, M, Da, F, out_f32=True)
        gemm_nt(dz, sh.bwd[Da * F:], dv, M, Dv, F, out_f32=True)
        return da.view(B, T, Da), dv.view(B, T, Dv), None, None, None, None


class CTCLossFn(torch.autograd.Function):
    @staticmethod
    def forward(ctx, logits, logit_len, targets, target_len, blank, zero_infinity):
        rt.require_gpu(logits)
        B, T, V = logits.shape
        lg = _f32c(logits)
        tg = targets.to(device=lg.device, dtype=torch.int64).contiguous()
        if tg.dim() == 1:
            tg = tg.view(B, -1)
        Lmax = tg.shape[1]
        il = logit_len.to(device=lg.device, dtype=torch.int64).contiguous()
        tl = target_len.to(device=lg.device, dtype=torch.int64).contiguous()
        nll = empty((B,), torch.float32, lg)
        mean = torch.zeros((), dtype=torch.float32, device=lg.device)
        need_grad = ctx.needs_input_grad[0]
        grad = empty((B, T, V), torch.float32, lg) if need_grad else None
        ws = empty((lib.raw("avec_ctc_workspace_floats")(B, T, max(Lmax, 1)),), torch.float32, lg)
        lib.ctc_loss(lg.data_ptr(), il.data_ptr(), tg.data_ptr(), tl.data_ptr(), nll.data_ptr(), mean.data_ptr(), _p(grad), ws.data_ptr(),
                     B, T, V, Lmax, blank, int(zero_infinity), rt.stream())
        ctx.saved = (grad, B)
        ctx.nll = nll
        return mean

    @staticmethod
    def backward(ctx, dloss):
        grad, B = ctx.saved
        out = torch.empty_like(grad)
        dl = dloss.float().contiguous()
        lib.scale_by_scalar(grad.data_ptr(), dl.data_ptr(), 1.0 / B, out.data_ptr(), grad.numel(), rt.stream())
        return out, None, None, None, None, None


class CTCLossMultiFn(torch.autograd.Function):

    @staticmethod
    def forward(ctx, blank, zero_infinity, targets, target_len, weights, *flat):
        n = len(flat) // 2
        logits, lens = [_f32c(t) for t in flat[0::2]], flat[1::2]
        rt.require_gpu(logits[0])
        B, _, V = logits[0].shape
        dev = logits[0].device
        tg = targets.to(device=dev, dtype=torch.int64).contiguous()
        if tg.dim() == 1:
            tg = tg.view(B, -1)
        Lmax = tg.shape[1]
        tl = target_len.to(device=dev, dtype=torch.int64).contiguous()
        ils = [l.to(device=dev, dtype=torch.int64).contiguous() for l in lens]
        nll = torch.empty((n, B), dtype=torch.float32, device=dev)
        means = rt.zeros_scratch(n + 1, dev)
        grads = [empty(tuple(lg.shape), torch.float32, lg) if ctx.needs_input_grad[5 + 2 * i] else None for i, lg in enumerate(logits)]
        arr_p = lambda ptrs: (ctypes.c_void_p * n)(*ptrs)
        Ts = (ctypes.c_int * n)(*[lg.shape[1] for lg in logits])
        lib.ctc_loss_multi(n, arr_p([lg.data_ptr() for lg in logits]), arr_p([l.data_ptr() for l in ils]), Ts, arr_p([nll[i].data_ptr() for i in range(n)]),
                           arr_p([means[i:].data_ptr() for i in range(n)]), arr_p([g.data_ptr() if g is not None else None for g in grads]),
                           tg.data_ptr(), tl.data_ptr(), (ctypes.c_float * n)(*[float(x) for x in weights]), means[n:].data_ptr(), B, V, Lmax, blank, int(zero_infinity), rt.stream())
        total = means[n]
        ctx.set_materialize_grads(False)
        ctx.saved = (grads, B, n, [float(x) for x in weights])
        ctx.keep = (logits, ils, tg, tl, nll)
        outs = tuple(means[i] for i in range(n))
        ctx.mark_non_differentiable(*outs)
        return (total,) + outs

    @staticmethod
    def backward(ctx, dtotal, *_unused):
        grads, B, n, weights = ctx.saved
        out = [None, None, None, None, None]
        if dtotal is None:
            return tuple(out + [None, None] * n)
        dt = dtotal.float().contiguous()
        live = [i for i in range(n) if grads[i] is not None]
        outs = {i: torch.empty_like(grads[i]) for i in live}
        if live:
            k = len(live)
            lib.scale_by_scalar_multi(k, (ctypes.c_void_p * k)(*[grads[i].data_ptr() for i in live]), (ctypes.c_void_p * k)(*[outs[i].data_ptr() for i in live]),
                                      (ctypes.c_longlong * k)(*[grads[i].numel() for i in live]), (ctypes.c_float * k)(*[weights[i] / B for i in live]), dt.data_ptr(), rt.stream())
        for i in range(n):
            out += [outs.get(i), None]
        return tuple(out)


_WCACHE = {}


def ctc_multi_fits(T, V, Lmax):
    return bool(lib.raw("avec_ctc_loss_multi_fits")(int(T), int(V), int(Lmax)))


class TimeMeanFn(torch.autograd.Function):

    @staticmethod
    def forward(ctx, x):
        from .lib import F32
        rt.require_gpu(x)
        B, T, V = x.shape
        x = _f32c(x)
        y = empty((B, V), torch.float32, x)
        lib.avgpool_fwd(F32, x.data_ptr(), y.data_ptr(), B, T, V, rt.stream())
        ctx.saved = (B, T, V)
        return y

    @staticmethod
    def backward(ctx, dy):
        from .lib import F32
        B, T, V = ctx.saved
        dy = _f32c(dy)
        dx = empty((B, T, V), torch.float32, dy)
        lib.avgpool_bwd(F32, dy.data_ptr(), dx.data_ptr(), B, T, V, rt.stream())
        return dx


class SoftmaxCEFn(torch.autograd.Function):

    @staticmethod
    def forward(ctx, logits, targets, ignore_index):
        rt.require_gpu(logits)
        M, V = logits.shape
        lg = _f32c(logits)
        tg = targets.to(device=lg.device, dtype=torch.int64).contiguous()
        loss = empty((M,), torch.float32, lg)
        mean = torch.zeros((), dtype=torch.float32, device=lg.device)
        grad = empty((M, V), torch.float32, lg) if ctx.needs_input_grad[0] else None
        lib.softmax_ce(lg.data_ptr(), tg.data_ptr(), int(ignore_index), loss.data_ptr(), mean.data_ptr(), _p(grad), M, V, rt.stream())
        ctx.saved = (grad, M)
        return mean

    @staticmethod
    def backward(ctx, dloss):
        grad, M = ctx.saved
        out = torch.empty_like(grad)
        lib.scale_by_scalar(grad.data_ptr(), dloss.float().contiguous().data_ptr(), 1.0 / M, out.data_ptr(), grad.numel(), rt.stream())
        return out, None, None


def conv2d_fwd(x, weight, N, H, W, Cin, stride, stats=None):
    Cout, KH, KW = weight.shape[0], weight.shape[2], weight.shape[3]
    pad = (KH - 1) // 2
    OH, OW = (H - 1) // stride + 1, (W - 1) // stride + 1
    M = N * OH * OW
    sh = rt.shadow(weight)
    y = empty((M, Cout), rt.act_dtype(), x)
    if _slab_conv(H, W, Cin, Cout, KH, KW, stride):
        ev = KERNEL_TIMER.start() if KERNEL_TIMER.enabled else None
        lib.conv3x3_c64(x.data_ptr(), sh.fwd.data_ptr(), y.data_ptr(), None, _p(stats), N, H, W, 0, rt.stream())
        if ev is not None:
            KERNEL_TIMER.stop(ev, (2, 0), 2.0 * M * Cout * KH * KW * Cin, 2.0 * (N * H * W * Cin + Cout * KH * KW * Cin + M * Cout))
        return y, OH, OW
    gemm_nt(x, sh.fwd, y, M, Cout, KH * KW * Cin, rows=rows_conv(H, W, Cin, KH, KW, stride, pad, OH, OW), mode=ROWS_CONV_FWD, stats=stats,
            abytes=2.0 * (N * H * W * Cin + Cout * KH * KW * Cin + M * Cout))
    return y, OH, OW


SLAB_CONV = True
SLAB_WGRAD128 = True
SHORTCUT_SUBGRID = True
GROUP_WGRAD128 = True


def _slab_conv(H, W, Cin, Cout, KH, KW, stride):
    return SLAB_CONV and rt.act_dtype() == torch.bfloat16 and bool(lib.raw("avec_conv3x3_c64_supported")(H, W, Cin, Cout, KH, KW, stride))


class BnbFuse:
    __slots__ = ("y", "ss", "mask_z", "stats", "done")

    def __init__(self, y, ss, mask_z, C):
        self.y, self.ss, self.mask_z, self.done = y, ss, mask_z, False
        self.stats = rt.zeros_scratch(BNState.NREP * 2 * C, y.device)


BNB_FUSE = False


def conv2d_bwd(dy, x, weight, N, H, W, Cin, stride, OH, OW, need_dx=True, dx_res=None, bnb=None, dx_res_cls0=False, dx_res_mask=None):
    Cout, KH, KW = weight.shape[0], weight.shape[2], weight.shape[3]
    pad = (KH - 1) // 2
    M = N * OH * OW
    sh = rt.shadow(weight)
    if _slab_conv(H, W, Cin, Cout, KH, KW, stride) and H * (W + 1) <= 512:
        if GROUP_WGRAD128 and _in_backward():
            it = WgradItem()
            it.x, it.dy, it.dw, it.images, it.C, it.H, it.W = x.data_ptr(), dy.data_ptr(), grad_of(weight).data_ptr(), N, Cin, H, W
            q = _pending()
            q.cw64.append(it)
            q.keep += [x, dy]
            q.cw64_flops += 2.0 * M * Cout * KH * KW * Cin
        else:
            ev = KERNEL_TIMER.start() if KERNEL_TIMER.enabled else None
            lib.wgrad3x3_c64(x.data_ptr(), dy.data_ptr(), grad_of(weight).data_ptr(), N, H, W, rt.stream())
            if ev is not None:
                KERNEL_TIMER.stop(ev, (2, 2), 2.0 * M * Cout * KH * KW * Cin)
    elif SLAB_CONV and SLAB_WGRAD128 and rt.act_dtype() == torch.bfloat16 and bool(lib.raw("avec_wgrad3x3_c128_supported")(H, W, Cin, Cout, KH, KW, stride)):
        if GROUP_WGRAD128 and _in_backward():
            it = WgradItem()
            it.x, it.dy, it.dw, it.images, it.C, it.H, it.W = x.data_ptr(), dy.data_ptr(), grad_of(weight).data_ptr(), N, Cin, H, W
            q = _pending()
            q.cw.append(it)
            q.keep += [x, dy]
            q.cw_flops += 2.0 * M * Cout * KH * KW * Cin
        else:
            ev = KERNEL_TIMER.start() if KERNEL_TIMER.enabled else None
            lib.wgrad3x3_c128(x.data_ptr(), dy.data_ptr(), grad_of(weight).data_ptr(), N, Cin, H, W, rt.stream())
            if ev is not None:
                KERNEL_TIMER.stop(ev, (2, 2), 2.0 * M * Cout * KH * KW * Cin)
    else:
        gemm_tn(dy, x, grad_of(weight), M, Cout, KH * KW * Cin, q_rows=rows_conv(H, W, Cin, KH, KW, stride, pad, OH, OW), q_mode=ROWS_CONV_FWD, side=True)
    if not need_dx:
        return None
    dx = empty((N * H * W, Cin), rt.act_dtype(), dy)
    if _slab_conv(H, W, Cin, Cout, KH, KW, stride):
        ev = KERNEL_TIMER.start() if KERNEL_TIMER.enabled else None
        if dx_res_mask is not None:
            lib.conv3x3_c64_res_masked(dy.data_ptr(), sh.bwd.data_ptr(), dx.data_ptr(), dx_res.data_ptr(), dx_res_mask.data_ptr(), N, H, W, 1, rt.stream())
        else:
            lib.conv3x3_c64(dy.data_ptr(), sh.bwd.data_ptr(), dx.data_ptr(), _p(dx_res), None, N, H, W, 1, rt.stream())
        if ev is not None:
            KERNEL_TIMER.stop(ev, (2, 1), 2.0 * N * H * W * Cin * KH * KW * Cout, 2.0 * (2 * N * H * W * Cin + Cout * KH * KW * Cin + M * Cout))
        return dx
    fuse = bnb if (bnb is not None and BNB_FUSE and rt.act_dtype() == torch.bfloat16 and Cin % 4 == 0) else None
    gemm_nt(dy, sh.bwd, dx, N * H * W, Cin, KH * KW * Cout, rows=rows_conv(H, W, Cout, KH, KW, stride, pad, OH, OW), mode=ROWS_CONV_BWD,
            res=dx_res, res_act=True, flops=2.0 * N * OH * OW * Cout * KH * KW * Cin, bnb=fuse, res_cls0=dx_res_cls0, res_mask=dx_res_mask,
            abytes=2.0 * (N * H * W * Cin * (2 if dx_res is not None else 1) + Cout * KH * KW * Cin + M * Cout))
    if fuse is not None:
        fuse.done = True
    return dx


RES_MASK = True


def res_mask_ok(H, W, Cin, Cout, stride):
    if rt.act_dtype() != torch.bfloat16 or stride != 1 or Cin != Cout:
        return False
    return _slab_conv(H, W, Cin, Cout, 3, 3, 1) or (Cin >= 128 and Cin % 32 == 0 and W <= 31)


class ResNetBlockFn(torch.autograd.Function):

    _CHAIN, _READY = {}, {}

    @staticmethod
    def forward(ctx, x, _anchor, blk, training, chain=False):
        rt.require_gpu(x)
        N, H, W, Cin = x.shape
        conv1, bn1, conv2, bn2 = blk.layers[0], blk.layers[1], blk.layers[3], blk.layers[4]
        stride = conv1.stride[0]
        Cout = conv1.weight.shape[0]
        adt = rt.act_dtype()
        x = x.contiguous()
        st1, st2 = BNState(Cout, x), BNState(Cout, x)
        y1, OH, OW = conv2d_fwd(x, conv1.weight, N, H, W, Cin, stride, stats=st1.stats if training else None)
        Mo = N * OH * OW
        c1 = bn_finalize(bn1, st1, Mo, training)
        a1 = empty((Mo, Cout), adt, x)
        lib.bn_apply_fwd(rt.dt(), y1.data_ptr(), st1.ss.data_ptr(), None, ACT_RELU, a1.data_ptr(), Mo, Cout, rt.stream())
        y2, _, _ = conv2d_fwd(a1, conv2.weight, N, OH, OW, Cout, 1, stats=st2.stats if training else None)
        c2 = bn_finalize(bn2, st2, Mo, training)
        has_proj = not isinstance(blk.residual, torch.nn.Identity)
        yr = str_ = cr = None
        if has_proj:
            convr, bnr = blk.residual[0], blk.residual[1]
            str_ = BNState(Cout, x)
            yr, _, _ = conv2d_fwd(x, convr.weight, N, H, W, Cin, stride, stats=str_.stats if training else None)
            cr = bn_finalize(bnr, str_, Mo, training)
        use_mask = RELU_BITMASK and training and Cout % 8 == 0 and Cout <= 2048 and Mo * Cout // 8 < (1 << 31)
        if has_proj and not use_mask:
            r = empty((Mo, Cout), adt, x)
            lib.bn_apply_fwd(rt.dt(), yr.data_ptr(), str_.ss.data_ptr(), None, ACT_NONE, r.data_ptr(), Mo, Cout, rt.stream())
        elif not has_proj:
            r = x
        out = empty((Mo, Cout), adt, x)
        ctx.relu_mask = None
        if use_mask:
            ctx.relu_mask = torch.empty(Mo * Cout // 8, dtype=torch.uint8, device=x.device)
            lib.bn_apply_fwd_mask(rt.dt(), y2.data_ptr(), st2.ss.data_ptr(), (yr if has_proj else r).data_ptr(), str_.ss.data_ptr() if has_proj else None, out.data_ptr(),
                                  ctx.relu_mask.data_ptr(), Mo, Cout, rt.stream())
        else:
            lib.bn_apply_fwd(rt.dt(), y2.data_ptr(), st2.ss.data_ptr(), r.data_ptr(), ACT_RELU, out.data_ptr(), Mo, Cout, rt.stream())
        ctx.saved = (x, y1, a1, y2, yr, out, st1, st2, str_, c1, c2, cr, blk, training, N, H, W, Cin, Cout, OH, OW, stride, has_proj)
        ctx.chain = bool(chain and training and BNB_FUSE and rt.act_dtype() == torch.bfloat16)
        if ctx.chain:
            if len(ResNetBlockFn._CHAIN) > 64:
                ResNetBlockFn._CHAIN.clear()
            ResNetBlockFn._CHAIN[out.data_ptr()] = (y2, out, st2, Cout)
        return out.view(N, OH, OW, Cout)

    @staticmethod
    def backward(ctx, dout):
        x, y1, a1, y2, yr, out, st1, st2, str_, c1, c2, cr, blk, training, N, H, W, Cin, Cout, OH, OW, stride, has_proj = ctx.saved
        conv1, bn1, conv2, bn2 = blk.layers[0], blk.layers[1], blk.layers[3], blk.layers[4]
        Mo = N * OH * OW
        dout = dout.reshape(Mo, Cout).to(rt.act_dtype()).contiguous()
        assert training, "ResNetBlock backward is implemented for training-mode BatchNorm"
        ResNetBlockFn._CHAIN.pop(out.data_ptr(), None)
        pre2 = ResNetBlockFn._READY.pop(dout.data_ptr(), None) if ctx.chain else None
        if pre2 is not None and pre2.y is not y2:
            raise RuntimeError("ResNetBlock backward: a fused BatchNorm-backward request does not belong to this block (the block output has another consumer?)")
        lazy_dres = (RES_MASK and not BNB_FUSE and ctx.relu_mask is not None and pre2 is None and
                     (has_proj or (conv1.weight.shape[2] == 3 and res_mask_ok(H, W, Cin, Cout, stride) and not KERNEL_TIMER.enabled)))
        dy2, dres = bn_backward(bn2, st2, c2, Mo, dout, y2, out, ACT_RELU, Mo, want_dres=not lazy_dres, pre=pre2, mask=ctx.relu_mask)
        f1 = BnbFuse(y1, st1.ss, None, Cout)
        da1 = conv2d_bwd(dy2, a1, conv2.weight, N, OH, OW, Cout, 1, OH, OW, bnb=f1)
        dy1, _ = bn_backward(bn1, st1, c1, Mo, da1, y1, None, ACT_RELU, Mo, pre=f1 if f1.done else None)
        need_dx = ctx.needs_input_grad[0]
        prev = ResNetBlockFn._CHAIN.get(x.data_ptr()) if need_dx else None
        fx = BnbFuse(prev[0], prev[2].ss, prev[1], prev[3]) if prev is not None else None
        if has_proj:
            convr, bnr = blk.residual[0], blk.residual[1]
            if lazy_dres:
                dyr, _ = bn_backward(bnr, str_, cr, Mo, dout, yr, None, ACT_NONE, Mo, mask=ctx.relu_mask)
            else:
                dyr, _ = bn_backward(bnr, str_, cr, Mo, dres, yr, None, ACT_NONE, Mo)
            kr = convr.weight.shape[2]
            if (SHORTCUT_SUBGRID and need_dx and stride == 2 and kr == 1 and rt.act_dtype() == torch.bfloat16 and Cin % 64 == 0 and Cout % 64 == 0
                    and conv1.weight.shape[2] == 3 and not _slab_conv(H, W, Cin, Cout, 3, 3, stride)):
                conv2d_bwd(dyr, x, convr.weight, N, H, W, Cin, stride, OH, OW, need_dx=False)
                dxs = empty((Mo, Cin), rt.act_dtype(), dyr)
                gemm_nt(dyr, rt.shadow(convr.weight).bwd, dxs, Mo, Cin, Cout)
                dx = conv2d_bwd(dy1, x, conv1.weight, N, H, W, Cin, stride, OH, OW, need_dx=True, dx_res=dxs, bnb=fx, dx_res_cls0=True)
            else:
                dx = conv2d_bwd(dyr, x, convr.weight, N, H, W, Cin, stride, OH, OW, need_dx=need_dx)
                dx = conv2d_bwd(dy1, x, conv1.weight, N, H, W, Cin, stride, OH, OW, need_dx=need_dx, dx_res=dx, bnb=fx)
        else:
            if lazy_dres:
                dx = conv2d_bwd(dy1, x, conv1.weight, N, H, W, Cin, stride, OH, OW, need_dx=need_dx, dx_res=dout, dx_res_mask=ctx.relu_mask, bnb=fx)
            else:
                dx = conv2d_bwd(dy1, x, conv1.weight, N, H, W, Cin, stride, OH, OW, need_dx=need_dx, dx_res=dres, bnb=fx)
        if fx is not None and fx.done:
            if len(ResNetBlockFn._READY) > 64:
                ResNetBlockFn._READY.clear()
            ResNetBlockFn._READY[dx.data_ptr()] = fx
        return (dx.view(N, H, W, Cin) if dx is not None else None), None, None, None, None


STEM3D_DIRECT = True
STEM3P_FUSED_WGRAD = True
STEM_GRAD_CLONE = False
STEM3P = True


class VideoStemFn(torch.autograd.Function):

    @staticmethod
    def forward(ctx, video, _anchor, conv, bn, training):
        rt.require_gpu(video)
        B, T, H, W = video.shape
        C = conv.weight.shape[0]
        v = _f32c(video)
        OH, OW = (H - 1) // 2 + 1, (W - 1) // 2 + 1
        M = B * T * OH * OW
        sh = rt.shadow(conv.weight)
        st = BNState(C, v)
        K, Kp = sh.Tm * sh.C, sh.Cp
        y = empty((M, C), rt.act_dtype(), v)
        if (STEM3P and STEM3D_DIRECT and rt.compute_dtype() == "bf16" and C == 64 and K == 245 and lib.raw("avec_stem3p_supported")(B, T, H, W)
                and lib.raw("avec_stem3d_supported")(B, T, H, W)):
            w8 = torch.zeros((C, 36, 8), dtype=sh.fwd.dtype, device=v.device)
            w8[:, :35, 1:] = sh.fwd.view(C, Kp)[:, :K].view(C, 35, 7)
            vb = v.to(torch.bfloat16)
            PH, PW = (OH - 1) // 2 + 1, (OW - 1) // 2 + 1
            zp = torch.empty((B * T, PH, PW, C), dtype=torch.bfloat16, device=v.device)
            idx = torch.empty((B * T, PH, PW, C), dtype=torch.uint8, device=v.device)
            lib.stem3p_fwd(vb.data_ptr(), w8.data_ptr(), _p(conv.bias), bn.weight.data_ptr(), zp.data_ptr(), idx.data_ptr(), st.stats.data_ptr() if training else None,
                           B, T, H, W, rt.stream())
            cp = bn_finalize(bn, st, M, training)
            out = torch.empty_like(zp)
            lib.bn_apply_fwd(rt.dt(), zp.data_ptr(), st.ss.data_ptr(), None, ACT_RELU, out.data_ptr(), B * T * PH * PW, C, rt.stream())
            ctx.saved = (v, None, idx, st, cp, conv, bn, ("p", vb, w8, zp, PH, PW), B, T, OH, OW, C, M, K, training, None)
            return out
        if STEM3D_DIRECT and rt.compute_dtype() == "bf16" and C == 64 and K == 245 and lib.raw("avec_stem3d_supported")(B, T, H, W):
            w8 = torch.zeros((C, 36, 8), dtype=sh.fwd.dtype, device=v.device)
            w8[:, :35, :7] = sh.fwd.view(C, Kp)[:, :K].view(C, 35, 7)
            lib.stem3d_fwd(v.data_ptr(), w8.data_ptr(), 288, _p(conv.bias), y.data_ptr(), st.stats.data_ptr() if training else None, B, T, H, W, rt.stream())
            r = None
        else:
            A = empty((M, Kp), rt.act_dtype(), v)
            lib.stem_im2col(rt.dt(), v.data_ptr(), A.data_ptr(), B, T, H, W, Kp, rt.stream())
            gemm_nt(A, sh.fwd, y, M, C, Kp, bias=conv.bias, stats=st.stats if training else None)
            r = A
        cp = bn_finalize(bn, st, M, training)
        PH, PW = (OH - 1) // 2 + 1, (OW - 1) // 2 + 1
        out = empty((B * T, PH, PW, C), rt.act_dtype(), v)
        idx = torch.empty((B * T, PH, PW, C), dtype=torch.uint8, device=v.device)
        ymax = torch.empty_like(out) if (training and C % 8 == 0) else None
        lib.stem_pool_fwd(rt.dt(), y.data_ptr(), st.ss.data_ptr(), out.data_ptr(), idx.data_ptr(), _p(ymax), B * T, OH, OW, C, rt.stream())
        ctx.saved = (v, y, idx, st, cp, conv, bn, r, B, T, OH, OW, C, M, K, training, ymax)
        return out

    @staticmethod
    def backward(ctx, dpool):
        v, y, idx, st, cp, conv, bn, r, B, T, OH, OW, C, M, K, training, ymax = ctx.saved
        assert training, "VideoStem backward is implemented for training-mode BatchNorm"
        dpool_in = dpool
        dpool = dpool.to(rt.act_dtype()).contiguous()
        if isinstance(r, tuple) and dpool.data_ptr() == dpool_in.data_ptr() and STEM_GRAD_CLONE:
            dpool = dpool.clone()
        if isinstance(r, tuple):
            _, vb, w8, zp, PH, PW = r
            H, W = v.shape[2], v.shape[3]
            dstats = torch.zeros(2 * C, dtype=torch.float32, device=v.device)
            lib.stem3p_reduce(dpool.data_ptr(), zp.data_ptr(), st.ss.data_ptr(), dstats.data_ptr(), B * T, PH, PW, rt.stream())
            gw, gb = grad_of(bn.weight), grad_of(bn.bias)
            dstats, synced = _add_local_affine_grads(dstats, gw, gb, C, (id(bn), "b"))
            if synced:
                gw = gb = None
            if STEM3P_FUSED_WGRAD and lib.raw("avec_stem3p_wgrad_supported")(B, T, H, W):
                lib.stem3p_wgrad(vb.data_ptr(), w8.data_ptr(), _p(conv.bias), dpool.data_ptr(), idx.data_ptr(), st.ss.data_ptr(), bn.weight.data_ptr(), dstats.data_ptr(), cp, float(M),
                                 grad_of(conv.weight).data_ptr(), _p(gw), _p(gb), B, T, H, W, rt.stream())
            else:
                dy = empty((M, C), rt.act_dtype(), v)
                lib.stem3p_dz(vb.data_ptr(), w8.data_ptr(), _p(conv.bias), dpool.data_ptr(), idx.data_ptr(), st.ss.data_ptr(), bn.weight.data_ptr(), dstats.data_ptr(), cp, float(M),
                              dy.data_ptr(), _p(gw), _p(gb), B, T, H, W, rt.stream())
                lib.stem3d_wgrad(v.data_ptr(), dy.data_ptr(), grad_of(conv.weight).data_ptr(), B, T, H, W, rt.stream())
            if conv.bias is not None:
                grad_of(conv.bias)
            stamp("v_stem_end:b")
            return None, None, None, None, None
        dstats = torch.zeros(2 * C, dtype=torch.float32, device=v.device)
        args = (dpool.data_ptr(), idx.data_ptr(), y.data_ptr(), st.ss.data_ptr(), bn.weight.data_ptr(), dstats.data_ptr(), cp, float(M))
        if ymax is not None:
            lib.stem_pool_bwd_reduce_pooled(rt.dt(), dpool.data_ptr(), idx.data_ptr(), ymax.data_ptr(), st.ss.data_ptr(), dstats.data_ptr(), B * T, OH, OW, C, rt.stream())
        else:
            lib.stem_pool_bwd(rt.dt(), *args, 0, None, None, None, B * T, OH, OW, C, rt.stream())
        gw, gb = grad_of(bn.weight), grad_of(bn.bias)
        dstats, synced = _add_local_affine_grads(dstats, gw, gb, C, (id(bn), "b"))
        if synced:
            gw = gb = None
            args = args[:5] + (dstats.data_ptr(),) + args[6:]
        dy = empty((M, C), rt.act_dtype(), v)
        lib.stem_pool_bwd(rt.dt(), *args, 1, dy.data_ptr(), _p(gw), _p(gb), B * T, OH, OW, C, rt.stream())
        if r is None:
            H, W = v.shape[2], v.shape[3]
            lib.stem3d_wgrad(v.data_ptr(), dy.data_ptr(), grad_of(conv.weight).data_ptr(), B, T, H, W, rt.stream())
        else:
            gemm_tn(dy, r, grad_of(conv.weight), M, C, K, q_rows=rows_plain(r.shape[1]), side=True)
        if conv.bias is not None:
            grad_of(conv.bias)
        return None, None, None, None, None


class AvgPoolFn(torch.autograd.Function):

    @staticmethod
    def forward(ctx, x):
        N, H, W, C = x.shape
        x = x.contiguous()
        y = empty((N, C), x.dtype, x)
        lib.avgpool_fwd(rt.dt(), x.data_ptr(), y.data_ptr(), N, H * W, C, rt.stream())
        ctx.saved = (N, H, W, C)
        return y

    @staticmethod
    def backward(ctx, dy):
        N, H, W, C = ctx.saved
        dy = dy.to(rt.act_dtype()).contiguous()
        dx = empty((N, H, W, C), dy.dtype, dy)
        lib.avgpool_bwd(rt.dt(), dy.data_ptr(), dx.data_ptr(), N, H * W, C, rt.stream())
        return dx


class AudioStemFn(torch.autograd.Function):

    @staticmethod
    def forward(ctx, mel, _anchor, conv, bn, training):
        rt.require_gpu(mel)
        B, NM, F = mel.shape
        C = conv.weight.shape[0]
        mel = _f32c(mel)
        Fo, To = (NM - 1) // 2 + 1, (F - 1) // 2 + 1
        adt = rt.act_dtype()
        y = empty((B * To, C * Fo), adt, mel)
        st = BNState(C, mel)
        lib.audio_stem_conv_fwd(rt.dt(), mel.data_ptr(), conv.weight.data_ptr(), _p(conv.bias), y.data_ptr(), st.stats.data_ptr() if training else None,
                                B, NM, F, C, rt.stream())
        count = B * To * Fo
        cp = bn_finalize(bn, st, count, training)
        a = empty((B, To, C * Fo), adt, mel)
        lib.audio_stem_act_fwd(rt.dt(), y.data_ptr(), st.ss.data_ptr(), a.data_ptr(), B, NM, F, C, rt.stream())
        ctx.saved = (mel, y, st, cp, count, conv, bn, B, NM, F, C, training)
        return a

    @staticmethod
    def backward(ctx, da):
        mel, y, st, cp, count, conv, bn, B, NM, F, C, training = ctx.saved
        assert training, "AudioStem backward is implemented for training-mode BatchNorm"
        flush_param_grads()
        da = da.to(rt.act_dtype()).contiguous()
        dstats = torch.zeros(2 * C, dtype=torch.float32, device=mel.device)
        base = (da.data_ptr(), y.data_ptr(), mel.data_ptr(), st.ss.data_ptr(), bn.weight.data_ptr(), dstats.data_ptr(), cp, float(count))
        lib.audio_stem_bwd(rt.dt(), *base, 0, None, None, None, None, B, NM, F, C, rt.stream())
        gw, gb = grad_of(bn.weight), grad_of(bn.bias)
        dstats, synced = _add_local_affine_grads(dstats, gw, gb, C, (id(bn), "b"))
        if synced:
            gw = gb = None
            base = base[:5] + (dstats.data_ptr(),) + base[6:]
        lib.audio_stem_bwd(rt.dt(), *base, 1, grad_of(conv.weight).data_ptr(), None if conv.bias is None else grad_of(conv.bias).data_ptr(),
                           _p(gw), _p(gb), B, NM, F, C, rt.stream())
        stamp("a_stem_end:b")
        arena = rt.arena_of(bn)
        if arena is not None and getattr(arena, "_early_armed", False) and getattr(arena, "_audio_range", None):
            lo, hi = arena._audio_range
            arena._audio_range = None
            arena.early_all_reduce(lo, hi)
        return None, None, None, None, None


def mel_spectrogram(audio, window, dft, fb, n_fft, win, hop, n_mels):
    rt.require_gpu(audio)
    from .lib import F32
    B, L = audio.shape
    audio = _f32c(audio)
    F = L // hop + 1
    nb = n_fft // 2 + 1
    frames = empty((B * F, win), torch.float32, audio)
    lib.mel_frames(audio.data_ptr(), window.data_ptr(), frames.data_ptr(), B, L, n_fft, win, hop, rt.stream())
    spec = empty((B * F, 2 * nb), torch.float32, audio)
    gemm_nt(frames, dft, spec, B * F, 2 * nb, win, out_f32=True, dtype=F32)
    out = empty((B, n_mels, F), torch.float32, audio)
    lib.mel_power_log(spec.data_ptr(), fb.data_ptr(), out.data_ptr(), B, F, nb, n_mels, rt.stream())
    return out


def spec_augment_(mel, lens, mF, Fp, mT, pS, sid):
    B, NM, F = mel.shape
    lens_ = None if lens is None else lens.to(device=mel.device, dtype=torch.int64).contiguous()
    lib.specaugment(mel.data_ptr(), _p(lens_), B, NM, F, mF, Fp, mT, pS, rt.rng_state(mel.device).data_ptr(), sid, rt.stream())
    return mel


def len_affine(lengths, sub, div, add):
    if torch.is_tensor(lengths) and lengths.is_cuda and lengths.dtype == torch.int64 and lengths.is_contiguous() and lengths.numel() > 0:
        out = torch.empty_like(lengths)
        lib.len_affine(lengths.data_ptr(), out.data_ptr(), lengths.numel(), sub, div, add, rt.stream())
        return out
    return torch.div(lengths - sub, div, rounding_mode="floor") + add


def argmax_rows(logits):
    lead, V = logits.shape[:-1], logits.shape[-1]
    lg = _f32c(logits)
    out = torch.empty(lead, dtype=torch.int64, device=lg.device)
    lib.argmax_rows(lg.data_ptr(), out.data_ptr(), out.numel(), V, rt.stream())
    return out


def ctc_beam_search(logits, lengths, beam, tmp=1.0, lm=None, alpha=0.6, beta=1.0):
    B, T, V = logits.shape
    lg = _f32c(logits)
    dev = lg.device
    lens = lengths.to(device=dev, dtype=torch.int64).contiguous()
    st = rt.stream()
    ws = torch.empty(lib.raw("avec_ctc_beam_workspace_bytes")(B, T, beam), dtype=torch.uint8, device=dev)
    tokens = torch.empty(B, beam, T, dtype=torch.int32, device=dev)
    out_len = torch.empty(B, beam, dtype=torch.int32, device=dev)
    score = torch.empty(B, beam, dtype=torch.float32, device=dev)
    ctc_logp = torch.empty(B, beam, dtype=torch.float32, device=dev)
    use_lm = lm is not None and lm.usable
    lm_arg = _byref(lm.device_struct(dev)) if use_lm else None
    oov = lm.oov_logprob if use_lm else 0.0
    lib.ctc_beam_search(lg.data_ptr(), lens.data_ptr(), B, T, V, beam, 1.0 / tmp, lm_arg, alpha if use_lm else 0.0, beta if use_lm else 0.0, oov,
                        ws.data_ptr(), ws.numel(), tokens.data_ptr(), out_len.data_ptr(), score.data_ptr(), ctc_logp.data_ptr(), st)
    return tokens, out_len, score, ctc_logp


def ngram_rows(lm, contexts):
    dev = torch.device("cuda", torch.cuda.current_device())
    n, L = len(contexts), max(1, max((len(c) for c in contexts), default=1))
    ctx = torch.zeros(n, L, dtype=torch.int32)
    for i, c in enumerate(contexts):
        if len(c):
            ctx[i, :len(c)] = torch.tensor(list(c), dtype=torch.int32)
    ctx, clen = ctx.to(dev), torch.tensor([len(c) for c in contexts], dtype=torch.int32, device=dev)
    rows = torch.empty(n, lm.V, dtype=torch.float32, device=dev)
    lib.ngram_rows(_byref(lm.device_struct(dev)), ctx.data_ptr(), clen.data_ptr(), n, L, lm.oov_logprob, rows.data_ptr(), rt.stream())
    return rows


CAUSAL_HEAD_DIM = 64


def _inference_only(what, *tensors):
    if torch.is_grad_enabled() and any(t is not None and t.requires_grad for t in tensors):
        raise RuntimeError("%s is an inference path (it has no backward kernels): call it under torch.no_grad(), or with inputs and parameters that do not "
                           "require grad -- a graph-less result would silently train nothing" % what)


def embed_pos(ids, weight, pos, out_f32=True):
    _inference_only("ops.embed_pos", weight, pos)
    rt.require_gpu(weight)
    N, L = ids.shape
    V, D = weight.shape
    pos = pos.reshape(-1, D)
    if pos.shape[0] < L:
        raise ValueError("ops.embed_pos: %d positions for sequences of %d tokens (max_pos_encoding)" % (pos.shape[0], L))
    ids = ids.to(device=weight.device, dtype=torch.int64).contiguous()
    w, p = _f32c(weight.detach()), _f32c(pos.detach())
    out = torch.empty(N, L, D, dtype=torch.float32 if out_f32 else rt.act_dtype(), device=weight.device)
    lib.embed_pos(rt.dt(), ids.data_ptr(), w.data_ptr(), p.data_ptr(), out.data_ptr(), int(out_f32), N, L, V, D, rt.stream())
    return out


def causal_attention(qkv, N, H, L, lens=None):
    _inference_only("ops.causal_attention", qkv)
    rt.require_gpu(qkv)
    M, W3 = qkv.shape
    d = W3 // (3 * H)
    if d != CAUSAL_HEAD_DIM or 3 * H * d != W3:
        raise NotImplementedError("ops.causal_attention: head width %d (row of %d over %d heads); the causal attention kernel supports d = %d only" % (d, W3, H, CAUSAL_HEAD_DIM))
    assert qkv.dtype == rt.act_dtype() and qkv.is_contiguous() and M == N * L, (qkv.dtype, qkv.shape, N, L)
    o = empty((M, H * d), rt.act_dtype(), qkv)
    lens_t = None if lens is None else lens.to(device=qkv.device, dtype=torch.int64).contiguous()
    lib.causal_attention(rt.dt(), qkv.data_ptr(), W3, _p(lens_t), o.data_ptr(), H * d, N, H, L, d, 1.0 / d ** 0.5, rt.stream())
# ... 70 lines not shown
```

include/avec_hip.h:

```cpp
#ifndef AVEC_HIP_H
#define AVEC_HIP_H
#include <stdint.h>
#ifdef __HIPCC__
#include <hip/hip_runtime.h>
#else
typedef struct ihipStream_t* hipStream_t;
#endif
#ifdef __cplusplus
extern "C" {
#endif

#define AVEC_F32 0
#define AVEC_BF16 1
#define AVEC_ABI_VERSION 4
#define AVEC_STAT_REPLICAS 64

int avec_version(void);
int avec_struct_size(int which);
const char* avec_last_error(void);
const char* avec_last_kernel(void);
int avec_set_reduce_workspace(void* base, long long bytes);
int avec_set_reduce_workspace_stream(void* base, long long bytes, hipStream_t stream);

enum { AVEC_ROWS_PLAIN = 0, AVEC_ROWS_CONV_FWD = 1, AVEC_ROWS_CONV_BWD = 2 };
typedef struct avec_rows {
  long long ld;
  int rows_out, rows_in, step;
  int H, W, C, KH, KW, stride, pad, OH, OW;
  int T3;
} avec_rows_t;

typedef struct avec_epilogue {
  void* out; long long ldo; int out_f32;
  void* out_pre; long long ldpre;
  const float* bias;
  int act;
  float drop_p; const unsigned long long* rng; unsigned rng_stream;
  const void* res; long long ldres; float alpha; int res_act;
  const void* dact_z; long long ldz; int dact;
  float* colsum;
  float* stats;
  const void* bnb_y; long long ldby; const float* bnb_ss; int bnb_mask;
  int res_cls0;
  const unsigned char* res_mask;
} avec_epilogue_t;

int avec_gemm_nt(int dtype, const void* A, const avec_rows_t* a_rows, int a_mode, int a_f32,
                 const void* W, long long ldw, long long M, int N, int K,
                 const avec_epilogue_t* ep, hipStream_t stream);

typedef struct { const float* src; void* dst; long long n; int slot; int K, Kp; int reserved; } avec_fp8_item_t;
int avec_fp8_quantize(int src_dtype, const void* x, long long ldx, void* q, long long ldq, long long M, int K, float* amax, int compute_amax, hipStream_t stream);
int avec_fp8_weights_refresh(const avec_fp8_item_t* table, int n_items, int blocks_per_item, float* amax, hipStream_t stream);
int avec_gemm_nt_fp8(const void* A, long long lda, const void* W, long long ldw, long long M, int N, int K,
                     const float* amax_a, const float* amax_w, const avec_epilogue_t* ep, hipStream_t stream);


int avec_gemm_tn(int dtype, const void* P, long long ldp, const void* Q, const avec_rows_t* q_rows, int q_mode, int q_f32,
                 float* O, long long ldo, long long M, int I, int J, hipStream_t stream);
int avec_gemm_tn_bias(int dtype, const void* P, long long ldp, const void* Q, const avec_rows_t* q_rows, int q_mode, int q_f32,
                      float* O, long long ldo, float* p_colsum, long long M, int I, int J, hipStream_t stream);
#define AVEC_TN_GROUP_MAX 32
typedef struct avec_tn_item {
  const void* P; const void* Q; float* O; float* p_colsum;
  long long ldp, ldq, ldo, M;
  int I, J;
  int q_rows_out, q_rows_in, q_step;
  int reserved;
} avec_tn_item_t;
int avec_gemm_tn_grouped_ok(int dtype, const avec_tn_item_t* item);
int avec_gemm_tn_grouped(int dtype, const avec_tn_item_t* items, int n, hipStream_t stream);
int avec_gemm_tn_batched(int dtype, const void* P, long long ldp, const void* Q, long long ldq, float* O, long long ldo, long long M, int I, int J,
                         int nb_outer, int nb_inner, const long long* strides6, hipStream_t stream);
int avec_gemm_tn_batched_store(int dtype, const void* P, long long ldp, const void* Q, long long ldq, void* O_act, long long ldo, long long M, int I, int J,
                               int nb_outer, int nb_inner, const long long* strides6, hipStream_t stream);

typedef struct {
  const void* P; long long ldp; const void* Q; long long ldq;
  float* O; void* O_act; long long ldo;
  long long M; int I, J, nb_outer, nb_inner;
  const long long* strides6;
} avec_tn_batched_t;
int avec_gemm_tn_batched_multi(int dtype, const avec_tn_batched_t* items, int n, hipStream_t stream);

#define AVEC_PEER_MAX_WORLD 8
int avec_peer_exchange_sum(const float* in, float* out, int n, void* const* pages, long long page_stride_granules, int rank, int world,
                           unsigned* epoch, int* err_flag, int timeout_ms, hipStream_t stream);
int avec_peer_exchange_sum_fused(const float* in, int n_replicas, int n_in, int has_tail, float tail, float* dgamma, float* dbeta, int C, float* out,
                                 void* const* pages, long long page_stride_granules, int rank, int world, unsigned* epoch, int* err_flag, int timeout_ms,
                                 hipStream_t stream);
int avec_enable_peer_access(int peer_device);
int avec_peer_buffer_alloc(void** ptr, long long bytes, void* ipc_handle_64b);
int avec_peer_buffer_open(const void* ipc_handle_64b, void** ptr);
int avec_peer_buffer_close(void* ptr);
int avec_peer_buffer_free(void* ptr);

int avec_layernorm_fwd(int dtype, const float* x, const float* gamma, const float* beta, void* y, int y_f32,
                       float* mean, float* rstd, long long M, int D, float eps, hipStream_t stream);
int avec_layernorm_bwd(int dtype, const void* dy, int dy_f32, const float* x, const float* mean, const float* rstd, const float* gamma,
                       float* dx, const float* dres, float* dgamma, float* dbeta, long long M, int D, hipStream_t stream);
int avec_layernorm_bwd_prep(int dtype, const void* dy, int dy_f32, const float* x, const float* mean, const float* rstd, const float* gamma,
                            float* dx, const float* dres, void* prep, float prep_alpha, float prep_drop_p, const unsigned long long* rng, unsigned rng_stream,
                            long long M, int D, hipStream_t stream);
int avec_layernorm_fwd2(int dtype, const float* x, const float* gamma1, const float* beta1, float eps1, float* y1, float* mean1, float* rstd1,
                        const float* gamma2, const float* beta2, float eps2, void* h2, float* mean2, float* rstd2, long long M, int D, hipStream_t stream);
int avec_layernorm_bwd2(int dtype, const void* dy2, const float* x2, const float* mean2, const float* rstd2, const float* gamma2, const float* dres2, float* dx2,
                        const float* x1, const float* mean1, const float* rstd1, const float* gamma1, float* dx1,
                        void* prep, float prep_alpha, float prep_drop_p, const unsigned long long* rng, unsigned rng_stream, long long M, int D, hipStream_t stream);
#define AVEC_LN_GROUP_MAX 40
typedef struct avec_ln_item {
  const void* dy; const float* x; const float* mean; const float* rstd; float* dgamma; float* dbeta;
  long long M; int D; int dy_f32;
} avec_ln_item_t;
int avec_layernorm_param_grads_grouped(int dtype, const avec_ln_item_t* items, int n, hipStream_t stream);
int avec_grad_prep(int dtype, const float* dout, long long ld, void* dacc, float alpha, float drop_p, const unsigned long long* rng,
                   unsigned rng_stream, float* dbias, long long M, int N, hipStream_t stream);
int avec_colsum(int dtype, const void* x, long long ld, float* out, long long M, int N, hipStream_t stream);
int avec_strided_rows_add(float* dx, const float* src, int B, int T, int To, int D, int step, hipStream_t stream);
int avec_bn_stats(int dtype, const void* y, float* stats, long long M, int C, hipStream_t stream);
int avec_bn_collapse(const float* stats, int n_replicas, float count, float* out, int C, hipStream_t stream);
int avec_bn_affine_grads(const float* dstats, float* dgamma, float* dbeta, int C, hipStream_t stream);
int avec_bn_finalize(const float* stats, int n_replicas, const float* count_ptr, float count, const float* gamma, const float* beta, float* running_mean,
                     float* running_var, long long* num_batches_tracked, float momentum, float eps, float* ss, int C, int training, hipStream_t stream);
int avec_stamp(unsigned long long* out, int slot, hipStream_t stream);
int avec_bn_bwd_finalize(const float* stats, int n_replicas, const float* ss, float* dstats, int C, hipStream_t stream);
int avec_bn_apply_fwd(int dtype, const void* y, const float* ss, const void* residual, int act, void* out, long long M, int C, hipStream_t stream);
int avec_bn_bwd_reduce(int dtype, const void* dout, const void* y, const void* out, const float* ss, int act, float* dstats, long long M, int C, hipStream_t stream);
int avec_bn_bwd_apply(int dtype, const void* dout, const void* y, const void* out, const float* ss, const float* gamma, const float* dstats,
                      const float* count_ptr, float count, int act, void* dy, void* dres, float* dgamma, float* dbeta, long long M, int C, hipStream_t stream);
int avec_bn_apply_fwd_mask(int dtype, const void* y, const float* ss, const void* residual, const float* residual_ss, void* out, unsigned char* mask, long long M, int C,
                           hipStream_t stream);
int avec_bn_bwd_reduce_mask(int dtype, const void* dout, const void* y, const unsigned char* mask, const float* ss, float* dstats, long long M, int C, hipStream_t stream);
int avec_bn_bwd_apply_mask(int dtype, const void* dout, const void* y, const unsigned char* mask, const float* ss, const float* gamma, const float* dstats,
                           const float* count_ptr, float count, void* dy, void* dres, float* dgamma, float* dbeta, long long M, int C, hipStream_t stream);
int avec_softmax_fwd(int dtype, const float* logits, void* probs, long long M, int V, hipStream_t stream);
int avec_softmax_bwd(int dtype, const void* dprobs, const float* logits, float* dlogits, const float* dadd, long long M, int V, hipStream_t stream);
int avec_cast_rows(int dtype, const float* src, long long ld_src, void* dst, long long ld_dst, long long M, int N, hipStream_t stream);
int avec_to_f32_rows(int dtype, const void* src, long long ld_src, float* dst, long long ld_dst, long long M, int N, int accum, hipStream_t stream);
int avec_act_f32(int act, const float* x, const float* dy, float* out, long long rows, int C, int backward, hipStream_t stream);
int avec_dropout_f32(const float* x, float* y, float p, const unsigned long long* rng, unsigned rng_stream, long long n, hipStream_t stream);
int avec_maxpool_hw_fwd(int dtype, const void* x, void* out, unsigned char* idx, long long frames, int H, int W, int C, int KH, int KW, int SH, int SW,
                        int pad0_h, int pad0_w, int pad1_h, int pad1_w, hipStream_t stream);
int avec_maxpool_hw_bwd(int dtype, const void* dy, const unsigned char* idx, void* dx, long long frames, int H, int W, int C, int KH, int KW, int SH, int SW,
                        int pad0_h, int pad0_w, int pad1_h, int pad1_w, hipStream_t stream);
int avec_upsample_rows(int dtype, const void* src, void* dst, long long B, int T, int D, int P, int backward, hipStream_t stream);
int avec_patch_pool_fwd(int dtype, const void* x, void* y, int B, int T, int D, int P, hipStream_t stream);
int avec_patch_pool_bwd(int dtype, const void* dy, void* dx, int B, int T, int D, int P, hipStream_t stream);
int avec_patch_unpool_add(int dtype, const void* o, const float* res, float* out, float drop_p, const unsigned long long* rng, unsigned rng_stream,
                          int B, int T, int D, int P, hipStream_t stream);
int avec_patch_unpool_bwd(int dtype, const float* dout, void* dob, float drop_p, const unsigned long long* rng, unsigned rng_stream,
                          int B, int T, int D, int P, hipStream_t stream);
int avec_avgpool_fwd(int dtype, const void* x, void* y, long long N, int HW, int C, hipStream_t stream);
int avec_avgpool_bwd(int dtype, const void* dy, void* dx, long long N, int HW, int C, hipStream_t stream);

int avec_glu_dwconv_fwd(int dtype, const void* u, const float* w, const float* bias, void* out, float* stats,
                        int B, int T, int C, int K, int stride, int pad_left, hipStream_t stream);
int avec_glu_dwconv_fwd_bn(int dtype, const void* u, const float* w, const float* bias, void* out, float* stats, int B, int T, int C, int K, int stride, int pad_left,
                           const float* gamma, const float* beta, float* running_mean, float* running_var, long long* num_batches_tracked, float momentum, float eps,
                           float* ss, hipStream_t stream);
int avec_dwconv_glu_bwd(int dtype, const void* dc, const void* u, const float* w, void* du, float* dw, float* dbias,
                        int B, int T, int C, int K, int stride, int pad_left, hipStream_t stream);
int avec_dwconv_glu_bwd_bn(int dtype, const void* da, const void* c, const float* ss, const float* gamma, const float* dstats, float count, const void* u, const float* w,
                           void* du, float* dw, float* dbias, float* dgamma, float* dbeta, int B, int T, int C, int K, int pad_left, hipStream_t stream);

typedef struct avec_attn {
  const void *q, *k, *v; long long ld;
  const void* e; long long lde;
  const long long* lens; int len_div;
  int q_full;
  const float* mask; long long mask_bstride;
  void* o; long long ldo; float* lse;
  const void* dout;
  void *dq, *dk, *dv; long long lddq, ldd;
  float* de; long long ldde;
  void *pbuf, *dsbuf; long long ldt;
  void* dsrel; long long ldr;
  int B, H, T, d; float scale;
  int Tk;
} avec_attn_t;
int avec_relpos_attention_fwd(int dtype, const avec_attn_t* args, hipStream_t stream);
int avec_relpos_attention_bwd(int dtype, const avec_attn_t* args, hipStream_t stream);

int avec_mel_frames(const float* audio, const float* window, float* frames, int B, long long L, int n_fft, int win, int hop, hipStream_t stream);
int avec_mel_power_log(const float* spec, const float* fb, float* out, int B, int F, int n_bins, int n_mels, hipStream_t stream);
int avec_specaugment(float* mel, const long long* lens, int B, int n_mels, int F, int mF, int Fparam, int mT, float pS,
                     const unsigned long long* rng, unsigned rng_stream, hipStream_t stream);
int avec_debug_rng_uniform(const unsigned long long* rng, unsigned rng_stream, const long long* ids, int n, float* out, hipStream_t stream);
int avec_audio_stem_conv_fwd(int dtype, const float* mel, const float* w, const float* bias, void* y, float* stats, int B, int n_mels, int F, int C, hipStream_t stream);
int avec_audio_stem_act_fwd(int dtype, const void* y, const float* ss, void* a, int B, int n_mels, int F, int C, hipStream_t stream);
int avec_audio_stem_bwd(int dtype, const void* da, const void* y, const float* mel, const float* ss, const float* gamma, float* dstats,
                        const float* count_ptr, float count, int phase, float* dw, float* dbias, float* dgamma, float* dbeta,
                        int B, int n_mels, int F, int C, hipStream_t stream);
int avec_stem_im2col(int dtype, const float* video, void* A, long long clips, int T, int H, int W, int ldk, hipStream_t stream);
int avec_stem3d_supported(long long clips, int T, int H, int W);
int avec_stem3d_fwd(const float* video, const void* w_shadow, int ldw, const float* bias, void* y, float* stats, long long clips, int T, int H, int W, hipStream_t stream);
int avec_stem3d_wgrad(const float* video, const void* dy, float* dw, long long clips, int T, int H, int W, hipStream_t stream);
int avec_stem3p_supported(long long clips, int T, int H, int W);
int avec_stem3p_fwd(const void* video_bf16, const void* w_shadow, const float* bias, const float* gamma, void* zp, unsigned char* idx, float* stats,
                    long long clips, int T, int H, int W, hipStream_t stream);
int avec_stem3p_reduce(void* dpool, const void* zp, const float* ss, float* dstats, long long frames, int PH, int PW, hipStream_t stream);
int avec_stem3p_wgrad_supported(long long clips, int T, int H, int W);
int avec_stem3p_wgrad(const void* video_bf16, const void* w_shadow, const float* bias, const void* dpool_masked, const unsigned char* idx, const float* ss,
                      const float* gamma, const float* dstats, const float* count_ptr, float count, float* dw, float* dgamma, float* dbeta,
                      long long clips, int T, int H, int W, hipStream_t stream);
int avec_stem3p_dz(const void* video_bf16, const void* w_shadow, const float* bias, const void* dpool_masked, const unsigned char* idx, const float* ss,
                   const float* gamma, const float* dstats, const float* count_ptr, float count, void* dz, float* dgamma, float* dbeta,
                   long long clips, int T, int H, int W, hipStream_t stream);
int avec_stem_pool_fwd(int dtype, const void* y, const float* ss, void* out, unsigned char* idx, void* ymax, long long frames, int H, int W, int C, hipStream_t stream);
int avec_stem_pool_bwd_reduce_pooled(int dtype, const void* dpool, const unsigned char* idx, const void* ymax, const float* ss, float* dstats,
                                     long long frames, int H, int W, int C, hipStream_t stream);
int avec_stem_pool_bwd(int dtype, const void* dpool, const unsigned char* idx, const void* y, const float* ss, const float* gamma, float* dstats,
                       const float* count_ptr, float count, int phase, void* dy, float* dgamma, float* dbeta, long long frames, int H, int W, int C, hipStream_t stream);

int avec_conv3x3_c64_supported(int H, int W, int Cin, int Cout, int KH, int KW, int stride);
int avec_conv3x3_c64(const void* x, const void* w, void* y, const void* res, float* stats, long long images, int H, int W, int flip, hipStream_t stream);
int avec_conv3x3_c64_res_masked(const void* x, const void* w, void* y, const void* res, const unsigned char* res_mask, long long images, int H, int W, int flip, hipStream_t stream);
int avec_wgrad3x3_c64(const void* x, const void* dy, float* dw, long long images, int H, int W, hipStream_t stream);
int avec_wgrad3x3_c128_supported(int H, int W, int Cin, int Cout, int KH, int KW, int stride);
int avec_wgrad3x3_c128(const void* x, const void* dy, float* dw, long long images, int C, int H, int W, hipStream_t stream);
#define AVEC_WGRAD_GROUP_MAX 16
typedef struct { const void* x; const void* dy; float* dw; long long images; int C, H, W, reserved; } avec_wgrad3x3_item_t;
int avec_wgrad3x3_c128_grouped(const avec_wgrad3x3_item_t* items, int n, hipStream_t stream);
int avec_wgrad3x3_c64_grouped(const avec_wgrad3x3_item_t* items, int n, hipStream_t stream);

int avec_video_input(const unsigned char* clips, const long long* clip_off, const int* geom, const int* masks, int max_masks, int channels, const float* lut, float mean, float stdv,
                     int mean_frame, float* out, float* frame_ws, int B, int Tout, int OH, int OW, hipStream_t stream);

long long avec_ctc_workspace_floats(int B, int T, int Lmax);
int avec_ctc_loss(const float* logits, const long long* in_lens, const long long* targets, const long long* tgt_lens, float* nll, float* mean_out,
                  float* grad, float* workspace, int B, int T, int V, int Lmax, int blank, int zero_infinity, hipStream_t stream);
int avec_ctc_loss_multi_fits(int T, int V, int Lmax);
int avec_ctc_loss_multi(int n_heads, const float* const* logits, const long long* const* in_lens, const int* T, float* const* nll, float* const* mean_out, float* const* grad,
                        const long long* targets, const long long* tgt_lens, const float* weights, float* total, int B, int V, int Lmax, int blank, int zero_infinity, hipStream_t stream);
int avec_scale_by_scalar(const float* g, const float* scalar_dev, float mul, float* out, long long n, hipStream_t stream);
int avec_scale_by_scalar_multi(int n_tensors, const float* const* g, float* const* out, const long long* numel, const float* mul, const float* scalar_dev, hipStream_t stream);
int avec_softmax_ce(const float* logits, const long long* targets, long long ignore_index, float* loss, float* mean_out, float* grad, long long M, int V, hipStream_t stream);
int avec_len_affine(const long long* in, long long* out, int n, long long sub, long long div, long long add, hipStream_t stream);
int avec_argmax_rows(const float* x, long long* out, long long M, int V, hipStream_t stream);

typedef struct avec_ngram {
  int order;
  int V;
  const float* unigram;
  long long ctx_cap;
  const unsigned long long* ctx_key;
  const float* ctx_bo;
  const int* ctx_off;
  const int* ctx_cnt;
  const int* cont_tok;
  const float* cont_lp;
} avec_ngram_t;
long long avec_ctc_beam_workspace_bytes(int B, int T, int W);
int avec_ctc_beam_search(const float* logits, const long long* lengths, int B, int T, int V, int W, float inv_tmp, const avec_ngram_t* lm, float alpha, float beta,
                         float oov_logprob, void* workspace, long long workspace_bytes, int* tokens, int* out_len, float* score, float* ctc_logp, hipStream_t stream);
int avec_ngram_rows(const avec_ngram_t* lm, const int* ctx, const int* ctx_len, int n, int max_len, float oov_logprob, float* rows, hipStream_t stream);
int avec_embed_pos(int dtype, const long long* ids, const float* E, const float* P, void* out, int out_f32, long long N, int L, int V, int D, hipStream_t stream);
int avec_causal_attention_supported(int d);
int avec_causal_attention(int dtype, const void* qkv, long long ld, const long long* lens, void* o, long long ldo, int N, int H, int L, int d, float scale, hipStream_t stream);
long long avec_lm_head_nll_workspace_bytes(long long R, int V, int D);
int avec_lm_head_nll(int dtype, const void* h, long long ldh, const void* W, long long ldw, const float* bias, const long long* tgt, float* nll, long long R, int V, int D,
                     void* workspace, long long workspace_bytes, hipStream_t stream);
int avec_lm_segment_sum(const float* nll, const long long* lens, long long S, int L, float* out, hipStream_t stream);
int avec_lm_rescore_select(const float* neural, const long long* lens, const float* beam_score, float alpha, float beta, int B, int K, float* total, long long* best,
                           hipStream_t stream);
int avec_adam_step(float* params, float* grads, float* exp_avg, float* exp_avg_sq, const float* state_dev, float beta1, float beta2, float eps,
                   float weight_decay, float grad_scale, int zero_grad, long long n, hipStream_t stream);
int avec_adam_step_guarded(float* params, float* grads, float* exp_avg, float* exp_avg_sq, const float* state_dev, float beta1, float beta2, float eps,
                           float weight_decay, float grad_scale, int zero_grad, long long n, const int* skip_flag, hipStream_t stream);
int avec_shadow_refresh(int dtype, const float* master, void* shadow, const long long* table_dev, int n_entries, long long total_blocks, hipStream_t stream);
int avec_shadow_refresh_range(int dtype, const float* master, void* shadow, const long long* table_dev, int n_entries, long long first_block, long long n_blocks, hipStream_t stream);

#ifdef __cplusplus
}
#endif
#endif
```

Measured before the change: 1903.

## Template-specialize BN8 kernels with software-pipelined streaming and add paired residual BN backward

Rewrites the 8-wide BatchNorm apply, backward-reduce and backward-apply kernels so the activation, residual and mask variants are compile-time template parameters. It also adds a double-buffered streaming helper that issues the next trip's loads before using the current ones, and sets the unroll factors to 1. It adds fused pair kernels that compute the main and projection-residual BN backward in one pass over dout and the mask, but the Python switch BN_PAIR is off by default. The aim is to cut runtime branching and hide memory latency in these bandwidth-bound passes, at the cost of more kernel instantiations and extra register pressure from the double buffer.

```diff
diff --git a/avec_amd/csrc/norm.hip b/avec_amd/csrc/norm.hip
--- a/avec_amd/csrc/norm.hip
+++ b/avec_amd/csrc/norm.hip
@@ -567,70 +567,110 @@
   nb = nb / q * q; if (nb < q) nb = q;
   return (unsigned)nb;
 }
-constexpr int BN8_U = 2;
-#ifndef AVEC_BN8_UR
-#define AVEC_BN8_UR 1
-#endif
-constexpr int BN8_UR = AVEC_BN8_UR;
+constexpr int BN8_U = 1;
+constexpr int BN8_UR = 1;
 constexpr unsigned BN8_CAP_FWD = 8192, BN8_CAP_BWD = 3072;
 
-template <typename T>
-__global__ __launch_bounds__(256) void bn_apply8_kernel(const T* __restrict__ y, const float* __restrict__ ss, const T* __restrict__ res, int act,
-                                                        T* __restrict__ out, unsigned n8, int C, unsigned char* __restrict__ mask = nullptr,
-                                                        const float* __restrict__ res_ss = nullptr) {
+template <typename I> __device__ __forceinline__ I bn_min(I a, I b) { return a < b ? a : b; }
+template <int U, typename Set, typename I, typename LD, typename USE>
+__device__ __forceinline__ void bn8_stream(I i, const I stride, const I n, LD ld, USE use) {
+  const I step = stride * U, last = n - 1;
+  Set a[U], b[U];
+#pragma unroll
+  for (int u = 0; u < U; ++u) ld(a[u], bn_min(i + u * stride, last));
+  auto ragged = [&](Set (&cur)[U], Set (&nxt)[U]) {
+    const bool more = i + step < n;
+    if (more) {
+#pragma unroll
+      for (int u = 0; u < U; ++u) ld(nxt[u], bn_min(i + step + u * stride, last)); }
+#pragma unroll
+    for (int u = 0; u < U; ++u) if (i + u * stride < n) use(cur[u], i + u * stride);
+    if (more) {
+#pragma unroll
+      for (int u = 0; u < U; ++u) if (i + step + u * stride < n) use(nxt[u], i + step + u * stride); }
+  };
+  auto trip = [&](Set (&cur)[U], Set (&nxt)[U]) {
+#pragma unroll
+    for (int u = 0; u < U; ++u) ld(nxt[u], i + step + u * stride);
+    __builtin_amdgcn_sched_barrier(0);
+#pragma unroll
+    for (int u = 0; u < U; ++u) use(cur[u], i + u * stride);
+    i += step;
+  };
+  for (;;) {
+    if (!(i + step + (U - 1) * stride < n)) { ragged(a, b); break; }
+    trip(a, b);
+    if (!(i + step + (U - 1) * stride < n)) { ragged(b, a); break; }
+    trip(b, a);
+  }
+}
+enum { BN_RES_NONE = 0, BN_RES_PLAIN = 1, BN_RES_SS = 2 };
+template <typename T, int RES> struct BnFwdIn {
+  Raw8<T> y, r;
+  __device__ __forceinline__ void load(const T* __restrict__ yp, const T* __restrict__ rp, unsigned j) {
+    y.load(yp + (long long)j * 8); if constexpr (RES != BN_RES_NONE) r.load(rp + (long long)j * 8); }
+};
+template <typename T, int ACT, int RES, bool MASK>
+__global__ __launch_bounds__(256) void bn_apply8_kernel(const T* __restrict__ y, const float* __restrict__ ss, const T* __restrict__ res,
+                                                        T* __restrict__ out, unsigned n8, int C, unsigned char* __restrict__ mask,
+                                                        const float* __restrict__ res_ss) {
   const unsigned C8 = (unsigned)C >> 3, stride = gridDim.x * 256, i0 = blockIdx.x * 256 + threadIdx.x;
+  if (i0 >= n8) return;
   const int c = (int)(i0 % C8) * 8;
   float sc[8], sh[8]; ld8<float>(ss + c, sc); ld8<float>(ss + C + c, sh);
   float rsc[8], rsh[8];
-  if (res_ss) { ld8<float>(res_ss + c, rsc); ld8<float>(res_ss + C + c, rsh);
+  if constexpr (RES == BN_RES_SS) { ld8<float>(res_ss + c, rsc); ld8<float>(res_ss + C + c, rsh);
 #pragma unroll
     for (int e = 0; e < 8; ++e) sh[e] += rsh[e]; }
-  for (unsigned i = i0; i < n8; i += stride * BN8_U) {
-    Raw8<T> ry[BN8_U], rr[BN8_U];
-#pragma unroll
-    for (int u = 0; u < BN8_U; ++u) { const unsigned j = i + u * stride; if (j < n8) { ry[u].load(y + (long long)j * 8); if (res) rr[u].load(res + (long long)j * 8); } }
-#pragma unroll
-    for (int u = 0; u < BN8_U; ++u) {
-      const unsigned j = i + u * stride; if (j >= n8) break;
-      float v[8]; ry[u].get(v);
-#pragma unroll
-      for (int e = 0; e < 8; ++e) v[e] = v[e] * sc[e] + sh[e];
-      if (res) { float r[8]; rr[u].get(r);
-        if (res_ss) {
-#pragma unroll
-          for (int e = 0; e < 8; ++e) v[e] += r[e] * rsc[e];
-        } else {
-#pragma unroll
-          for (int e = 0; e < 8; ++e) v[e] += r[e]; } }
-      if (act == 1) {
-#pragma unroll
-        for (int e = 0; e < 8; ++e) v[e] = swishf_(v[e]);
-      } else if (act == 2) {
-        if (mask) {
-          unsigned b = 0;
-#pragma unroll
-          for (int e = 0; e < 8; ++e) b |= (v[e] > 0.f ? 1u : 0u) << e;
-          mask[j] = (unsigned char)b;
-        }
-#pragma unroll
-        for (int e = 0; e < 8; ++e) v[e] = fmaxf(v[e], 0.f);
+  auto emit = [&](const BnFwdIn<T, RES>& in, unsigned j) {
+    float v[8]; in.y.get(v);
+#pragma unroll
+    for (int e = 0; e < 8; ++e) v[e] = fmaf(v[e], sc[e], sh[e]);
+    if constexpr (RES != BN_RES_NONE) { float r[8]; in.r.get(r);
+#pragma unroll
+      for (int e = 0; e < 8; ++e) { if constexpr (RES == BN_RES_SS) v[e] = fmaf(r[e], rsc[e], v[e]); else v[e] += r[e]; } }
+    if constexpr (ACT == 1) {
+#pragma unroll
+      for (int e = 0; e < 8; ++e) v[e] = swishf_(v[e]);
+    } else if constexpr (ACT == 2) {
+      if constexpr (MASK) {
+        unsigned b = 0;
+#pragma unroll
+        for (int e = 0; e < 8; ++e) b |= (v[e] > 0.f ? 1u : 0u) << e;
+        mask[j] = (unsigned char)b;
       }
-      st8<T>(out + (long long)j * 8, v);
-    }
-  }
+#pragma unroll
+      for (int e = 0; e < 8; ++e) v[e] = fmaxf(v[e], 0.f);
+    }
+    st8<T>(out + (long long)j * 8, v);
+  };
+  bn8_stream<BN8_U, BnFwdIn<T, RES>, unsigned>(i0, stride, n8, [&](BnFwdIn<T, RES>& in, unsigned j) { in.load(y, res, j); }, emit);
+}
+template <typename T, int ACT, int RES, bool MASK>
+static void bn_apply8_launch(const void* y, const float* ss, const void* res, void* out, long long n8, int C, unsigned char* mask, const float* res_ss, hipStream_t st) {
+  hipLaunchKernelGGL((bn_apply8_kernel<T, ACT, RES, MASK>), dim3(bn8_blocks(n8, C, BN8_CAP_FWD)), dim3(256), 0, st, (const T*)y, ss, (const T*)res, (T*)out, (unsigned)n8, C, mask, res_ss);
 }
 extern "C" int avec_bn_apply_fwd_mask(int dtype, const void* y, const float* ss, const void* residual, const float* residual_ss, void* out, unsigned char* mask, long long M, int C,
                                       hipStream_t st) {
   AVEC_CHECK_ARG(y && ss && out && mask && M > 0 && C > 0 && C % 8 == 0 && M * C / 8 < (1ll << 31) && (residual || !residual_ss), "bn_apply_fwd_mask: bad arguments (C %% 8 == 0, M*C < 2^34)");
-  const long long n8 = M * C / 8; const unsigned nb8 = bn8_blocks(n8, C, BN8_CAP_FWD);
-  DISPATCH_T(dtype, hipLaunchKernelGGL(bn_apply8_kernel<T>, dim3((unsigned)nb8), dim3(256), 0, st, (const T*)y, ss, (const T*)residual, 2, (T*)out, (unsigned)n8, C, mask, residual_ss));
-  AVEC_LAUNCH_CHECK(); return 0;
+  const long long n8 = M * C / 8;
+  if (residual_ss) DISPATCH_T(dtype, bn_apply8_launch<T, 2, BN_RES_SS, true>(y, ss, residual, out, n8, C, mask, residual_ss, st));
+  else if (residual) DISPATCH_T(dtype, bn_apply8_launch<T, 2, BN_RES_PLAIN, true>(y, ss, residual, out, n8, C, mask, nullptr, st));
+  else DISPATCH_T(dtype, bn_apply8_launch<T, 2, BN_RES_NONE, true>(y, ss, nullptr, out, n8, C, mask, nullptr, st));
+  AVEC_LAUNCH_CHECK(); return 0;
+}
+template <typename T, int RES>
+static void bn_apply8_launch_act(int act, const void* y, const float* ss, const void* res, void* out, long long n8, int C, hipStream_t st) {
+  if (act == 1) bn_apply8_launch<T, 1, RES, false>(y, ss, res, out, n8, C, nullptr, nullptr, st);
+  else if (act == 2) bn_apply8_launch<T, 2, RES, false>(y, ss, res, out, n8, C, nullptr, nullptr, st);
+  else bn_apply8_launch<T, 0, RES, false>(y, ss, res, out, n8, C, nullptr, nullptr, st);
 }
 extern "C" int avec_bn_apply_fwd(int dtype, const void* y, const float* ss, const void* residual, int act, void* out, long long M, int C, hipStream_t st) {
   AVEC_CHECK_ARG(y && ss && out && M > 0 && C > 0 && C % 4 == 0, "bn_apply_fwd: bad arguments");
   if (C % 8 == 0 && M * C / 8 < (1ll << 31)) {
-    const long long n8 = M * C / 8; const unsigned nb8 = bn8_blocks(n8, C, BN8_CAP_FWD);
-    DISPATCH_T(dtype, hipLaunchKernelGGL(bn_apply8_kernel<T>, dim3((unsigned)nb8), dim3(256), 0, st, (const T*)y, ss, (const T*)residual, act, (T*)out, (unsigned)n8, C));
+    const long long n8 = M * C / 8;
+    if (residual) DISPATCH_T(dtype, bn_apply8_launch_act<T, BN_RES_PLAIN>(act, y, ss, residual, out, n8, C, st));
+    else DISPATCH_T(dtype, bn_apply8_launch_act<T, BN_RES_NONE>(act, y, ss, nullptr, out, n8, C, st));
     AVEC_LAUNCH_CHECK(); return 0;
   }
   long long n4 = M * C / 4; long long nb = (n4 + 255) / 256; if (nb > 4096) nb = 4096;
@@ -661,51 +701,82 @@
   float* const dst[2] = {dstats, dstats + C};
   colreduce_atomic<2>(part, dst, col, C, ws);
 }
-template <typename T>
+enum { BN_SRC_NONE = 0,
+       BN_SRC_SWISH = 1,
+       BN_SRC_RECOMP = 2,
+       BN_SRC_OUT = 3,
+       BN_SRC_BITS = 4 };
+static inline int bn_src_reduce(int act, const void* out) { return act == 2 ? (out ? BN_SRC_OUT : BN_SRC_RECOMP) : act == 1 ? BN_SRC_SWISH : BN_SRC_NONE; }
+static inline int bn_src_apply(int act, const void* out) { return act == 0 ? BN_SRC_NONE : act == 1 ? BN_SRC_SWISH : (act == 2 && out) ? BN_SRC_OUT : BN_SRC_RECOMP; }
+__device__ __forceinline__ float bn_mul_rounded(float a, float b) {
+#pragma clang fp contract(off)
+  return a * b;
+}
+constexpr bool bn_src_needs_ss(int SRC) { return SRC == BN_SRC_SWISH || SRC == BN_SRC_RECOMP; }
+template <typename T, int SRC> struct BnBwdIn {
+  Raw8<T> d, v, o; unsigned char mb;
+  __device__ __forceinline__ void load(const T* __restrict__ dout, const T* __restrict__ y, const T* __restrict__ out, const unsigned char* __restrict__ mask, long long j) {
+    d.load(dout + j * 8); v.load(y + j * 8);
+    if constexpr (SRC == BN_SRC_BITS) mb = mask[j];
+    if constexpr (SRC == BN_SRC_OUT) o.load(out + j * 8);
+  }
+  __device__ __forceinline__ void get(float (&dd)[8], float (&vv)[8], const float (&sc)[8], const float (&sh)[8]) const {
+    d.get(dd); v.get(vv);
+    if constexpr (SRC == BN_SRC_BITS) {
+#pragma unroll
+      for (int e = 0; e < 8; ++e) dd[e] = (mb >> e) & 1 ? dd[e] : 0.f;
+    } else if constexpr (SRC == BN_SRC_OUT) { float q[8]; o.get(q);
+#pragma unroll
+      for (int e = 0; e < 8; ++e) dd[e] = q[e] > 0.f ? dd[e] : 0.f;
+    } else if constexpr (SRC == BN_SRC_RECOMP) {
+#pragma unroll
+      for (int e = 0; e < 8; ++e) dd[e] = fmaf(vv[e], sc[e], sh[e]) > 0.f ? dd[e] : 0.f;
+    } else if constexpr (SRC == BN_SRC_SWISH) {
+#pragma unroll
+      for (int e = 0; e < 8; ++e) dd[e] = bn_mul_rounded(dd[e], dswishf_(fmaf(vv[e], sc[e], sh[e])));
+    }
+  }
+};
+template <typename T, int SRC>
 __global__ __launch_bounds__(256) void bn_bwd_reduce8_kernel(const T* __restrict__ dout, const T* __restrict__ y, const T* __restrict__ out, const float* __restrict__ ss,
-                                                             int act, float* dstats, long long M, int C, ColWs ws, const unsigned char* __restrict__ mask = nullptr) {
+                                                             float* dstats, long long M, int C, ColWs ws, const unsigned char* __restrict__ mask) {
   const Col8 m = col8_map(C);
   float part[2][8];
 #pragma unroll
   for (int e = 0; e < 8; ++e) part[0][e] = part[1][e] = 0.f;
-  if (m.active) {
+  const long long row = (long long)blockIdx.x * m.R + m.r;
+  if (m.active && row < M) {
     const int c = m.l * 8;
     float mu[8], rs[8], sc[8], sh[8]; ld8<float>(ss + 2 * C + c, mu); ld8<float>(ss + 3 * C + c, rs);
-    if (act == 1 || (act == 2 && !out && !mask)) { ld8<float>(ss + c, sc); ld8<float>(ss + C + c, sh); }
-    const long long rstride = (long long)gridDim.x * m.R;
-    for (long long row = (long long)blockIdx.x * m.R + m.r; row < M; row += rstride * BN8_UR) {
-      Raw8<T> rd[BN8_UR], rv[BN8_UR], ro[BN8_UR]; unsigned mb[BN8_UR];
-#pragma unroll
-      for (int u = 0; u < BN8_UR; ++u) { const long long r = row + u * rstride; if (r < M) { const long long off = r * C + c; rd[u].load(dout + off); rv[u].load(y + off);
-        if (mask) mb[u] = mask[off >> 3]; else if (act == 2 && out) ro[u].load(out + off); } }
-#pragma unroll
-      for (int u = 0; u < BN8_UR; ++u) {
-        if (row + u * rstride >= M) break;
-        float d[8], v[8]; rd[u].get(d); rv[u].get(v);
-        if (mask) {
-#pragma unroll
-          for (int e = 0; e < 8; ++e) d[e] = (mb[u] >> e) & 1u ? d[e] : 0.f; }
-        else if (act == 2 && out) { float o[8]; ro[u].get(o);
-#pragma unroll
-          for (int e = 0; e < 8; ++e) d[e] = o[e] > 0.f ? d[e] : 0.f; }
-        else if (act == 2) {
-#pragma unroll
-          for (int e = 0; e < 8; ++e) d[e] = (v[e] * sc[e] + sh[e]) > 0.f ? d[e] : 0.f; }
-        else if (act == 1) {
-#pragma unroll
-          for (int e = 0; e < 8; ++e) d[e] *= dswishf_(v[e] * sc[e] + sh[e]); }
-#pragma unroll
-        for (int e = 0; e < 8; ++e) { part[0][e] += d[e]; part[1][e] += d[e] * (v[e] - mu[e]) * rs[e]; }
-      }
-    }
+    if constexpr (bn_src_needs_ss(SRC)) { ld8<float>(ss + c, sc); ld8<float>(ss + C + c, sh); }
+    auto acc = [&](const BnBwdIn<T, SRC>& in, long long) {
+      float d[8], v[8]; in.get(d, v, sc, sh);
+#pragma unroll
+      for (int e = 0; e < 8; ++e) { part[0][e] += d[e]; part[1][e] += d[e] * (v[e] - mu[e]) * rs[e]; }
+    };
+    const long long L = m.L, l = m.l;
+    bn8_stream<BN8_UR, BnBwdIn<T, SRC>, long long>(row, (long long)gridDim.x * m.R, M, [&](BnBwdIn<T, SRC>& in, long long r) { in.load(dout, y, out, mask, r * L + l); }, acc);
   }
   float* const dst[2] = {dstats, dstats + C};
   colreduce8_atomic<2>(part, dst, m, ws);
+}
+template <typename T>
+static void bn_bwd_reduce8_launch(int src, unsigned nb, const void* dout, const void* y, const void* out, const float* ss, float* dstats, long long M, int C, ColWs ws,
+                                  const unsigned char* mask, hipStream_t st) {
+#define BN_RED8(SRC) hipLaunchKernelGGL((bn_bwd_reduce8_kernel<T, SRC>), dim3(nb), dim3(256), 0, st, (const T*)dout, (const T*)y, (const T*)out, ss, dstats, M, C, ws, mask)
+  switch (src) {
+    case BN_SRC_SWISH: BN_RED8(BN_SRC_SWISH); break;
+    case BN_SRC_RECOMP: BN_RED8(BN_SRC_RECOMP); break;
+    case BN_SRC_OUT: BN_RED8(BN_SRC_OUT); break;
+    case BN_SRC_BITS: BN_RED8(BN_SRC_BITS); break;
+    default: BN_RED8(BN_SRC_NONE); break;
+  }
+#undef BN_RED8
 }
 extern "C" int avec_bn_bwd_reduce_mask(int dtype, const void* dout, const void* y, const unsigned char* mask, const float* ss, float* dstats, long long M, int C, hipStream_t st) {
   AVEC_CHECK_ARG(dout && y && mask && ss && dstats && M > 0 && col8_ok(C), "bn_bwd_reduce_mask: bad arguments");
   ColWs ws; const unsigned nb = col8_cfg(M, C, 2, &ws, st);
-  DISPATCH_T(dtype, hipLaunchKernelGGL(bn_bwd_reduce8_kernel<T>, dim3(nb), dim3(256), 0, st, (const T*)dout, (const T*)y, (const T*)nullptr, ss, 2, dstats, M, C, ws, mask));
+  DISPATCH_T(dtype, bn_bwd_reduce8_launch<T>(BN_SRC_BITS, nb, dout, y, nullptr, ss, dstats, M, C, ws, mask, st));
   AVEC_LAUNCH_CHECK();
   if (ws.partial) { float* const dst[2] = {dstats, dstats + C}; return col_finalize(ws, 1, nb, 2, C, dst, C, st); }
   return 0;
@@ -714,7 +785,7 @@
   AVEC_CHECK_ARG(dout && y && ss && dstats && M > 0 && C % 4 == 0, "bn_bwd_reduce: bad arguments");
   if (col8_ok(C)) {
     ColWs ws; const unsigned nb = col8_cfg(M, C, 2, &ws, st);
-    DISPATCH_T(dtype, hipLaunchKernelGGL(bn_bwd_reduce8_kernel<T>, dim3(nb), dim3(256), 0, st, (const T*)dout, (const T*)y, (const T*)out, ss, act, dstats, M, C, ws));
+    DISPATCH_T(dtype, bn_bwd_reduce8_launch<T>(bn_src_reduce(act, out), nb, dout, y, out, ss, dstats, M, C, ws, nullptr, st));
     AVEC_LAUNCH_CHECK();
     if (ws.partial) { float* const dst[2] = {dstats, dstats + C}; return col_finalize(ws, 1, nb, 2, C, dst, C, st); }
     return 0;
@@ -741,69 +812,159 @@
     if (dres) st4<T>(dres + off, dr);
   }
 }
-template <typename T>
+template <typename T, int SRC, bool DRES>
 __global__ __launch_bounds__(256) void bn_bwd_apply8_kernel(const T* __restrict__ dout, const T* __restrict__ y, const T* __restrict__ out, const float* __restrict__ ss,
-                                                            const float* __restrict__ gamma, const float* __restrict__ dstats, const float* count_ptr, float count, int act,
+                                                            const float* __restrict__ gamma, const float* __restrict__ dstats, const float* count_ptr, float count,
                                                             T* __restrict__ dy, T* __restrict__ dres, float* dgamma, float* dbeta, unsigned n8, int C,
-                                                            const unsigned char* __restrict__ mask = nullptr) {
+                                                            const unsigned char* __restrict__ mask) {
   const float inv_n = 1.f / (count_ptr ? *count_ptr : count);
   if (blockIdx.x == 0 && dgamma) for (int c = threadIdx.x; c < C; c += 256) { atomicAdd(dgamma + c, dstats[C + c]); atomicAdd(dbeta + c, dstats[c]); }
   const unsigned C8 = (unsigned)C >> 3, stride = gridDim.x * 256, i0 = blockIdx.x * 256 + threadIdx.x;
+  if (i0 >= n8) return;
   const int c = (int)(i0 % C8) * 8;
   float mu[8], rs[8], A[8], m1[8], m2[8], sc[8], sh[8];
   { float g[8], s1[8], s2[8]; ld8<float>(ss + 2 * C + c, mu); ld8<float>(ss + 3 * C + c, rs); ld8<float>(gamma + c, g); ld8<float>(dstats + c, s1); ld8<float>(dstats + C + c, s2);
 #pragma unroll
     for (int e = 0; e < 8; ++e) { A[e] = g[e] * rs[e]; m1[e] = s1[e] * inv_n; m2[e] = s2[e] * inv_n; } }
-  const bool recompute = act != 0 && !(act == 2 && (out || mask));
-  if (recompute) { ld8<float>(ss + c, sc); ld8<float>(ss + C + c, sh); }
-  for (unsigned i = i0; i < n8; i += stride * BN8_U) {
-    Raw8<T> rd[BN8_U], rv[BN8_U], ro[BN8_U]; unsigned mb[BN8_U];
-#pragma unroll
-    for (int u = 0; u < BN8_U; ++u) { const unsigned j = i + u * stride; if (j < n8) { const long long off = (long long)j * 8; rd[u].load(dout + off); rv[u].load(y + off);
-      if (mask) mb[u] = mask[j]; else if (act == 2 && out) ro[u].load(out + off); } }
-#pragma unroll
-    for (int u = 0; u < BN8_U; ++u) {
-      const unsigned j = i + u * stride; if (j >= n8) break;
-      const long long off = (long long)j * 8;
-      float d[8], v[8], o[8]; rd[u].get(d); rv[u].get(v);
-      if (mask) {
-#pragma unroll
-        for (int e = 0; e < 8; ++e) d[e] = (mb[u] >> e) & 1u ? d[e] : 0.f;
-      } else if (act == 2 && out) { float q[8]; ro[u].get(q);
-#pragma unroll
-        for (int e = 0; e < 8; ++e) d[e] = q[e] > 0.f ? d[e] : 0.f;
-      } else if (act != 0) {
-#pragma unroll
-        for (int e = 0; e < 8; ++e) { const float pre = v[e] * sc[e] + sh[e]; d[e] = act == 1 ? d[e] * dswishf_(pre) : (pre > 0.f ? d[e] : 0.f); }
-      }
-#pragma unroll
-      for (int e = 0; e < 8; ++e) o[e] = A[e] * (d[e] - m1[e] - (v[e] - mu[e]) * rs[e] * m2[e]);
-      st8<T>(dy + off, o);
-      if (dres) st8<T>(dres + off, d);
-    }
-  }
+  if constexpr (bn_src_needs_ss(SRC)) { ld8<float>(ss + c, sc); ld8<float>(ss + C + c, sh); }
+  auto emit = [&](const BnBwdIn<T, SRC>& in, unsigned j) {
+    const long long off = (long long)j * 8;
+    float d[8], v[8], o[8]; in.get(d, v, sc, sh);
+#pragma unroll
+    for (int e = 0; e < 8; ++e) o[e] = A[e] * fmaf(-((v[e] - mu[e]) * rs[e]), m2[e], d[e] - m1[e]);
+    st8<T>(dy + off, o);
+    if constexpr (DRES) st8<T>(dres + off, d);
+  };
+  bn8_stream<BN8_U, BnBwdIn<T, SRC>, unsigned>(i0, stride, n8, [&](BnBwdIn<T, SRC>& in, unsigned j) { in.load(dout, y, out, mask, j); }, emit);
+}
+template <typename T, bool DRES>
+static void bn_bwd_apply8_launch(int src, const void* dout, const void* y, const void* out, const float* ss, const float* gamma, const float* dstats, const float* count_ptr, float count,
+                                 void* dy, void* dres, float* dgamma, float* dbeta, long long n8, int C, const unsigned char* mask, hipStream_t st) {
+#define BN_APP8(SRC) hipLaunchKernelGGL((bn_bwd_apply8_kernel<T, SRC, DRES>), dim3(bn8_blocks(n8, C, BN8_CAP_BWD)), dim3(256), 0, st, (const T*)dout, (const T*)y, (const T*)out, ss, gamma, \
+                                        dstats, count_ptr, count, (T*)dy, (T*)dres, dgamma, dbeta, (unsigned)n8, C, mask)
+  switch (src) {
+    case BN_SRC_SWISH: BN_APP8(BN_SRC_SWISH); break;
+    case BN_SRC_RECOMP: BN_APP8(BN_SRC_RECOMP); break;
+    case BN_SRC_OUT: BN_APP8(BN_SRC_OUT); break;
+    case BN_SRC_BITS: BN_APP8(BN_SRC_BITS); break;
+    default: BN_APP8(BN_SRC_NONE); break;
+  }
+#undef BN_APP8
 }
 extern "C" int avec_bn_bwd_apply_mask(int dtype, const void* dout, const void* y, const unsigned char* mask, const float* ss, const float* gamma, const float* dstats,
                                       const float* count_ptr, float count, void* dy, void* dres, float* dgamma, float* dbeta, long long M, int C, hipStream_t st) {
   AVEC_CHECK_ARG(dout && y && mask && ss && gamma && dstats && dy && M > 0 && C % 8 == 0 && M * C / 8 < (1ll << 31), "bn_bwd_apply_mask: bad arguments");
-  const long long n8 = M * C / 8; const unsigned nb8 = bn8_blocks(n8, C, BN8_CAP_BWD);
-  DISPATCH_T(dtype, hipLaunchKernelGGL(bn_bwd_apply8_kernel<T>, dim3((unsigned)nb8), dim3(256), 0, st, (const T*)dout, (const T*)y, (const T*)nullptr, ss, gamma, dstats,
-                                       count_ptr, count, 2, (T*)dy, (T*)dres, dgamma, dbeta, (unsigned)n8, C, mask));
+  const long long n8 = M * C / 8;
+  if (dres) DISPATCH_T(dtype, bn_bwd_apply8_launch<T, true>(BN_SRC_BITS, dout, y, nullptr, ss, gamma, dstats, count_ptr, count, dy, dres, dgamma, dbeta, n8, C, mask, st));
+  else DISPATCH_T(dtype, bn_bwd_apply8_launch<T, false>(BN_SRC_BITS, dout, y, nullptr, ss, gamma, dstats, count_ptr, count, dy, nullptr, dgamma, dbeta, n8, C, mask, st));
   AVEC_LAUNCH_CHECK(); return 0;
 }
 extern "C" int avec_bn_bwd_apply(int dtype, const void* dout, const void* y, const void* out, const float* ss, const float* gamma, const float* dstats,
                                  const float* count_ptr, float count, int act, void* dy, void* dres, float* dgamma, float* dbeta, long long M, int C, hipStream_t st) {
   AVEC_CHECK_ARG(dout && y && ss && gamma && dstats && dy && M > 0 && C % 4 == 0, "bn_bwd_apply: bad arguments");
   if (C % 8 == 0 && M * C / 8 < (1ll << 31)) {
-    const long long n8 = M * C / 8; const unsigned nb8 = bn8_blocks(n8, C, BN8_CAP_BWD);
-    DISPATCH_T(dtype, hipLaunchKernelGGL(bn_bwd_apply8_kernel<T>, dim3((unsigned)nb8), dim3(256), 0, st, (const T*)dout, (const T*)y, (const T*)out, ss, gamma, dstats,
-                                         count_ptr, count, act, (T*)dy, (T*)dres, dgamma, dbeta, (unsigned)n8, C));
+    const long long n8 = M * C / 8; const int src = bn_src_apply(act, out);
+    if (dres) DISPATCH_T(dtype, bn_bwd_apply8_launch<T, true>(src, dout, y, out, ss, gamma, dstats, count_ptr, count, dy, dres, dgamma, dbeta, n8, C, nullptr, st));
+    else DISPATCH_T(dtype, bn_bwd_apply8_launch<T, false>(src, dout, y, out, ss, gamma, dstats, count_ptr, count, dy, nullptr, dgamma, dbeta, n8, C, nullptr, st));
     AVEC_LAUNCH_CHECK(); return 0;
   }
   long long n4 = M * C / 4; long long nb = (n4 + 255) / 256; if (nb > 4096) nb = 4096;
   DISPATCH_T(dtype, hipLaunchKernelGGL(bn_bwd_apply_kernel<T>, dim3((unsigned)nb), dim3(256), 0, st, (const T*)dout, (const T*)y, (const T*)out, ss, gamma, dstats,
                                        count_ptr, count, act, (T*)dy, (T*)dres, dgamma, dbeta, n4, C));
   AVEC_LAUNCH_CHECK(); return 0;
+}
+template <typename T> struct BnPairIn {
+  Raw8<T> d, v2, vr; unsigned char mb;
+  __device__ __forceinline__ void load(const T* __restrict__ dout, const T* __restrict__ y2, const T* __restrict__ yr, const unsigned char* __restrict__ mask, long long j) {
+    d.load(dout + j * 8); v2.load(y2 + j * 8); vr.load(yr + j * 8); mb = mask[j]; }
+  __device__ __forceinline__ void get(float (&dd)[8], float (&a)[8], float (&b)[8]) const {
+    d.get(dd); v2.get(a); vr.get(b);
+#pragma unroll
+    for (int e = 0; e < 8; ++e) dd[e] = (mb >> e) & 1 ? dd[e] : 0.f;
+  }
+};
+template <typename T>
+__global__ __launch_bounds__(256, 4) void bn_bwd_reduce8_pair_kernel(const T* __restrict__ dout, const T* __restrict__ y2, const T* __restrict__ yr, const float* __restrict__ ss2,
+                                                                  const float* __restrict__ ssr, float* dstats2, float* dstatsr, long long M, int C, ColWs ws,
+                                                                  const unsigned char* __restrict__ mask) {
+  const Col8 m = col8_map(C);
+  float part[4][8];
+#pragma unroll
+  for (int e = 0; e < 8; ++e) part[0][e] = part[1][e] = part[2][e] = part[3][e] = 0.f;
+  const long long row = (long long)blockIdx.x * m.R + m.r;
+  if (m.active && row < M) {
+    const int c = m.l * 8;
+    float mu2[8], rs2[8], mur[8], rsr[8]; ld8<float>(ss2 + 2 * C + c, mu2); ld8<float>(ss2 + 3 * C + c, rs2); ld8<float>(ssr + 2 * C + c, mur); ld8<float>(ssr + 3 * C + c, rsr);
+    auto acc = [&](const BnPairIn<T>& in, long long) {
+      float d[8], a[8], b[8]; in.get(d, a, b);
+#pragma unroll
+      for (int e = 0; e < 8; ++e) { part[0][e] += d[e]; part[1][e] += d[e] * (a[e] - mu2[e]) * rs2[e]; part[3][e] += d[e] * (b[e] - mur[e]) * rsr[e]; }
+    };
+    const long long L = m.L, l = m.l;
+    for (long long r = row; r < M; r += (long long)gridDim.x * m.R) { BnPairIn<T> in; in.load(dout, y2, yr, mask, r * L + l); acc(in, r); }
+#pragma unroll
+    for (int e = 0; e < 8; ++e) part[2][e] = part[0][e];
+  }
+  float* const dst[4] = {dstats2, dstats2 + C, dstatsr, dstatsr + C};
+  colreduce8_atomic<4>(part, dst, m, ws);
+}
+extern "C" int avec_bn_bwd_reduce_mask2(int dtype, const void* dout, const unsigned char* mask, const void* y2, const float* ss2, const void* yr, const float* ssr,
+                                        float* dstats2, float* dstatsr, long long M, int C, hipStream_t st) {
+  AVEC_CHECK_ARG(dout && mask && y2 && ss2 && yr && ssr && dstats2 && dstatsr && dstats2 != dstatsr && M > 0 && col8_ok(C), "bn_bwd_reduce_mask2: bad arguments");
+  ColWs ws; const unsigned nb = col8_cfg(M, C, 4, &ws, st);
+  DISPATCH_T(dtype, hipLaunchKernelGGL(bn_bwd_reduce8_pair_kernel<T>, dim3(nb), dim3(256), 0, st, (const T*)dout, (const T*)y2, (const T*)yr, ss2, ssr, dstats2, dstatsr, M, C, ws, mask));
+  AVEC_LAUNCH_CHECK();
+  if (ws.partial) { float* const dst[4] = {dstats2, dstats2 + C, dstatsr, dstatsr + C}; return col_finalize(ws, 1, nb, 4, C, dst, C, st); }
+  return 0;
+}
+struct BnPairSide { const float* ss; const float* gamma; const float* dstats; float* dgamma; float* dbeta; };
+template <typename T>
+__global__ __launch_bounds__(256) void bn_bwd_apply8_pair_kernel(const T* __restrict__ dout, const T* __restrict__ y2, const T* __restrict__ yr, const unsigned char* __restrict__ mask,
+                                                                 BnPairSide s2, BnPairSide sr, const float* count_ptr, float count, T* __restrict__ dy2, T* __restrict__ dyr,
+                                                                 unsigned n8, int C) {
+  const float inv_n = 1.f / (count_ptr ? *count_ptr : count);
+  if (blockIdx.x == 0) for (int c = threadIdx.x; c < C; c += 256) {
+    if (s2.dgamma) { atomicAdd(s2.dgamma + c, s2.dstats[C + c]); atomicAdd(s2.dbeta + c, s2.dstats[c]); }
+    if (sr.dgamma) { atomicAdd(sr.dgamma + c, sr.dstats[C + c]); atomicAdd(sr.dbeta + c, sr.dstats[c]); } }
+  const unsigned C8 = (unsigned)C >> 3, stride = gridDim.x * 256, i0 = blockIdx.x * 256 + threadIdx.x;
+  if (i0 >= n8) return;
+  const int c = (int)(i0 % C8) * 8;
+  float mu2[8], rs2[8], A2[8], p2[8], q2[8], mur[8], rsr[8], Ar[8], pr[8], qr[8];
+  auto coef = [&](const BnPairSide& s, float (&mu)[8], float (&rs)[8], float (&A)[8], float (&m1)[8], float (&m2)[8]) {
+    float g[8], s1[8], t2[8]; ld8<float>(s.ss + 2 * C + c, mu); ld8<float>(s.ss + 3 * C + c, rs); ld8<float>(s.gamma + c, g); ld8<float>(s.dstats + c, s1); ld8<float>(s.dstats + C + c, t2);
+#pragma unroll
+    for (int e = 0; e < 8; ++e) { A[e] = g[e] * rs[e]; m1[e] = s1[e] * inv_n; m2[e] = t2[e] * inv_n; }
+  };
+  coef(s2, mu2, rs2, A2, p2, q2); coef(sr, mur, rsr, Ar, pr, qr);
+  auto emit = [&](const BnPairIn<T>& in, unsigned j) {
+    const long long off = (long long)j * 8;
+    float d[8], a[8], b[8], o[8]; in.get(d, a, b);
+#pragma unroll
+    for (int e = 0; e < 8; ++e) o[e] = A2[e] * fmaf(-((a[e] - mu2[e]) * rs2[e]), q2[e], d[e] - p2[e]);
+    st8<T>(dy2 + off, o);
+#pragma unroll
+    for (int e = 0; e < 8; ++e) o[e] = Ar[e] * fmaf(-((b[e] - mur[e]) * rsr[e]), qr[e], d[e] - pr[e]);
+    st8<T>(dyr + off, o);
+  };
+  bn8_stream<BN8_U, BnPairIn<T>, unsigned>(i0, stride, n8, [&](BnPairIn<T>& in, unsigned j) { in.load(dout, y2, yr, mask, j); }, emit);
+}
+extern "C" int avec_bn_bwd_apply_mask2(int dtype, const void* dout, const unsigned char* mask, const void* y2, const float* ss2, const float* gamma2, const float* dstats2,
+                                       const void* yr, const float* ssr, const float* gammar, const float* dstatsr, const float* count_ptr, float count,
+                                       void* dy2, void* dyr, float* dgamma2, float* dbeta2, float* dgammar, float* dbetar, long long M, int C, hipStream_t st) {
+  AVEC_CHECK_ARG(dout && mask && y2 && ss2 && gamma2 && dstats2 && yr && ssr && gammar && dstatsr && dy2 && dyr && dy2 != dyr && M > 0 && C % 8 == 0 && M * C / 8 < (1ll << 31) &&
+                 !dgamma2 == !dbeta2 && !dgammar == !dbetar, "bn_bwd_apply_mask2: bad arguments");
+  const long long n8 = M * C / 8;
+  const BnPairSide s2{ss2, gamma2, dstats2, dgamma2, dbeta2}, sr{ssr, gammar, dstatsr, dgammar, dbetar};
+  DISPATCH_T(dtype, hipLaunchKernelGGL(bn_bwd_apply8_pair_kernel<T>, dim3(bn8_blocks(n8, C, BN8_CAP_BWD)), dim3(256), 0, st, (const T*)dout, (const T*)y2, (const T*)yr, mask, s2, sr,
+                                       count_ptr, count, (T*)dy2, (T*)dyr, (unsigned)n8, C));
+  AVEC_LAUNCH_CHECK(); return 0;
+}
+extern "C" int avec_bn8_geometry(int pass, long long M, int C, unsigned* blocks, unsigned* chunks_per_thread_per_trip) {
+  AVEC_CHECK_ARG(pass >= 0 && pass <= 2 && blocks && chunks_per_thread_per_trip && M > 0 && C > 0 && C % 8 == 0 && M * C / 8 < (1ll << 31) && (pass != 1 || col8_ok(C)),
+                 "bn8_geometry: bad arguments (the 8-wide passes need C %% 8 == 0, M*C < 2^34, C <= 2048 for the reduction)");
+  if (pass == 1) { *blocks = col8_blocks(M, C); *chunks_per_thread_per_trip = BN8_UR; }
+  else { *blocks = bn8_blocks(M * C / 8, C, pass == 0 ? BN8_CAP_FWD : BN8_CAP_BWD); *chunks_per_thread_per_trip = BN8_U; }
+  return 0;
 }
 
 template <typename T>
diff --git a/avec_amd/ops.py b/avec_amd/ops.py
--- a/avec_amd/ops.py
+++ b/avec_amd/ops.py
@@ -1020,6 +1020,19 @@
     return dy, (dout if pre is not None else dres)
 
 
+def bn_backward_pair(bn2, st2, bnr, str_, count, dout, y2, yr, mask, M):
+    C = st2.C
+    dstats = rt.zeros_scratch(4 * C, dout.device)
+    d2, dr = dstats[:2 * C], dstats[2 * C:]
+    lib.bn_bwd_reduce_mask2(rt.dt(), dout.data_ptr(), mask.data_ptr(), y2.data_ptr(), st2.ss.data_ptr(), yr.data_ptr(), str_.ss.data_ptr(), d2.data_ptr(), dr.data_ptr(),
+                            M, C, rt.stream())
+    dy2, dyr = empty((M, C), rt.act_dtype(), dout), empty((M, C), rt.act_dtype(), dout)
+    lib.bn_bwd_apply_mask2(rt.dt(), dout.data_ptr(), mask.data_ptr(), y2.data_ptr(), st2.ss.data_ptr(), bn2.weight.data_ptr(), d2.data_ptr(),
+                           yr.data_ptr(), str_.ss.data_ptr(), bnr.weight.data_ptr(), dr.data_ptr(), None, float(count), dy2.data_ptr(), dyr.data_ptr(),
+                           _p(grad_of(bn2.weight)), _p(grad_of(bn2.bias)), _p(grad_of(bnr.weight)), _p(grad_of(bnr.bias)), M, C, rt.stream())
+    return dy2, dyr
+
+
 def _add_local_affine_grads(dstats, gw, gb, C, key):
     if not rt.sync_batchnorm():
         return dstats, False
@@ -1426,6 +1439,7 @@
     return dx
 
 
+BN_PAIR = False
 RES_MASK = True
 
 
@@ -1498,7 +1512,11 @@
             raise RuntimeError("ResNetBlock backward: a fused BatchNorm-backward request does not belong to this block (the block output has another consumer?)")
         lazy_dres = (RES_MASK and not BNB_FUSE and ctx.relu_mask is not None and pre2 is None and
                      (has_proj or (conv1.weight.shape[2] == 3 and res_mask_ok(H, W, Cin, Cout, stride) and not KERNEL_TIMER.enabled)))
-        dy2, dres = bn_backward(bn2, st2, c2, Mo, dout, y2, out, ACT_RELU, Mo, want_dres=not lazy_dres, pre=pre2, mask=ctx.relu_mask)
+        pair = BN_PAIR and has_proj and lazy_dres and not rt.sync_batchnorm()
+        if pair:
+            dy2, dyr = bn_backward_pair(bn2, st2, blk.residual[1], str_, Mo, dout, y2, yr, ctx.relu_mask, Mo)
+        else:
+            dy2, dres = bn_backward(bn2, st2, c2, Mo, dout, y2, out, ACT_RELU, Mo, want_dres=not lazy_dres, pre=pre2, mask=ctx.relu_mask)
         f1 = BnbFuse(y1, st1.ss, None, Cout)
         da1 = conv2d_bwd(dy2, a1, conv2.weight, N, OH, OW, Cout, 1, OH, OW, bnb=f1)
         dy1, _ = bn_backward(bn1, st1, c1, Mo, da1, y1, None, ACT_RELU, Mo, pre=f1 if f1.done else None)
@@ -1507,7 +1525,9 @@
         fx = BnbFuse(prev[0], prev[2].ss, prev[1], prev[3]) if prev is not None else None
         if has_proj:
             convr, bnr = blk.residual[0], blk.residual[1]
-            if lazy_dres:
+            if pair:
+                pass
+            elif lazy_dres:
                 dyr, _ = bn_backward(bnr, str_, cr, Mo, dout, yr, None, ACT_NONE, Mo, mask=ctx.relu_mask)
             else:
                 dyr, _ = bn_backward(bnr, str_, cr, Mo, dres, yr, None, ACT_NONE, Mo)
diff --git a/include/avec_hip.h b/include/avec_hip.h
--- a/include/avec_hip.h
+++ b/include/avec_hip.h
@@ -133,6 +133,12 @@
 int avec_bn_bwd_reduce_mask(int dtype, const void* dout, const void* y, const unsigned char* mask, const float* ss, float* dstats, long long M, int C, hipStream_t stream);
 int avec_bn_bwd_apply_mask(int dtype, const void* dout, const void* y, const unsigned char* mask, const float* ss, const float* gamma, const float* dstats,
                            const float* count_ptr, float count, void* dy, void* dres, float* dgamma, float* dbeta, long long M, int C, hipStream_t stream);
+int avec_bn_bwd_reduce_mask2(int dtype, const void* dout, const unsigned char* mask, const void* y2, const float* ss2, const void* yr, const float* ssr,
+                             float* dstats2, float* dstatsr, long long M, int C, hipStream_t stream);
+int avec_bn_bwd_apply_mask2(int dtype, const void* dout, const unsigned char* mask, const void* y2, const float* ss2, const float* gamma2, const float* dstats2,
+                            const void* yr, const float* ssr, const float* gammar, const float* dstatsr, const float* count_ptr, float count,
+                            void* dy2, void* dyr, float* dgamma2, float* dbeta2, float* dgammar, float* dbetar, long long M, int C, hipStream_t stream);
+int avec_bn8_geometry(int pass, long long M, int C, unsigned* blocks, unsigned* chunks_per_thread_per_trip);
 int avec_softmax_fwd(int dtype, const float* logits, void* probs, long long M, int V, hipStream_t stream);
 int avec_softmax_bwd(int dtype, const void* dprobs, const float* logits, float* dlogits, const float* dadd, long long M, int V, hipStream_t stream);
 int avec_cast_rows(int dtype, const float* src, long long ld_src, void* dst, long long ld_dst, long long M, int N, hipStream_t stream);
```

After: 1917, median of 6. About the same (+0.7%).
